# j-min/HiREST

Hardware: AMD Instinct MI355X
Metric: encoded frames/sec (EVA-CLIP-g/14 224^2) (higher is better)
Workload: dtype bf16

## Files before the change

### hirest_amd/_lib.py

```python
from __future__ import annotations

import ctypes as C
import os

HERE = os.path.dirname(os.path.abspath(__file__))
LIB_PATH = os.path.join(HERE, "lib", "libhirest_hip.so")
if os.environ.get("HIREST_LIB_VARIANT"):
    LIB_PATH = os.path.join(HERE, "lib", f"libhirest_hip.{os.environ['HIREST_LIB_VARIANT']}.so")

(EPI_BIAS_BF16, EPI_BIAS_GELU_BF16, EPI_BIAS_QGELU_BF16, EPI_BIAS_RESID_F32, EPI_BIAS_F32, EPI_PATCH_POS_F32,
 EPI_BIAS_RESID_LNSTATS_F32, EPI_LNFOLD_BF16, EPI_LNFOLD_GELU_BF16, EPI_BIAS_GELU_SPLIT2, EPI_BIAS_RESID2_LNSTATS) = range(11)

TOWER_NO_LNFOLD = 1
TOWER_NO_PRUNE = 2
TOWER_F32_RESIDUAL = 4
GEMM_REVERSE = 1
GEMM_X3 = 2
GEMM_X3_T128 = 4
ABI_VERSION = 4

ERRORS = {-1: "HIREST_E_BADARG", -2: "HIREST_E_SHAPE (unsupported shape)", -3: "HIREST_E_WORKSPACE (workspace too small)"}


class GemmArgs(C.Structure):
    _fields_ = [("struct_size", C.c_uint64),
                ("A", C.c_void_p), ("lda", C.c_int64), ("W", C.c_void_p), ("ldw", C.c_int64),
                ("bias", C.c_void_p), ("out", C.c_void_p), ("ldo", C.c_int64),
                ("M", C.c_int32), ("N", C.c_int32), ("K", C.c_int32), ("epilogue", C.c_int32),
                ("pos", C.c_void_p), ("patches_per_frame", C.c_int32), ("aux0", C.c_void_p), ("aux1", C.c_void_p), ("flags", C.c_int32)]

    @classmethod
    def make(cls, *fields):
        return cls(C.sizeof(cls), *fields)


F32_ENTRY = {"gemm": 0, "ws": 1, "layouts": 2, "ln": 3, "ln_colmax": 4, "rows_colmax": 5}


class GemmF32Query(C.Structure):
    _fields_ = [("struct_size", C.c_uint32)] + \
               [(n, C.c_int32) for n in ("entry", "M", "N", "K", "has_resid", "has_periodic", "has_ids", "has_ln_out", "has_workspace",
                                         "a_kmajor", "w_kmajor", "select_kernel", "ring_mode", "rows_ln_mode", "cus")]

    @classmethod
    def make(cls, entry, M, N, K, **fields):
        q = cls(C.sizeof(cls), F32_ENTRY[entry], M, N, K, select_kernel=-1, ring_mode=-1, rows_ln_mode=-1)
        for k, v in fields.items():
            setattr(q, k, int(v))
        return q


class BlockWeights(C.Structure):
    _fields_ = [(n, C.c_void_p) for n in ("ln1_g", "ln1_b", "qkv_w", "qkv_b", "proj_w", "proj_b",
                                          "ln2_g", "ln2_b", "fc1_w", "fc1_b", "fc2_w", "fc2_b",
                                          "qkv_wf", "qkv_bf", "qkv_s", "fc1_wf", "fc1_bf", "fc1_s")]


class VisionTower(C.Structure):
    _fields_ = [(n, C.c_int32) for n in ("image_size", "patch", "width", "heads", "head_dim", "mlp_dim",
                                         "layers", "embed_dim", "kpad", "act")] + \
               [("ln_eps", C.c_float)] + \
               [("patch_w", C.c_void_p), ("patch_b", C.c_void_p), ("cls", C.c_void_p), ("pos", C.c_void_p),
                ("blocks", C.POINTER(BlockWeights)),
                ("norm_g", C.c_void_p), ("norm_b", C.c_void_p), ("head_w", C.c_void_p), ("head_b", C.c_void_p),
                ("image_mean", C.c_void_p), ("image_std", C.c_void_p),
                ("ln_pre_g", C.c_void_p), ("ln_pre_b", C.c_void_p), ("out_all_tokens", C.c_int32)]


class TextTower(C.Structure):
    _fields_ = [(n, C.c_int32) for n in ("context", "vocab", "width", "heads", "layers", "embed_dim", "act")] + \
               [("ln_eps", C.c_float)] + \
               [("tok_emb", C.c_void_p), ("pos", C.c_void_p), ("blocks", C.POINTER(BlockWeights)),
                ("lnf_g", C.c_void_p), ("lnf_b", C.c_void_p), ("proj_w", C.c_void_p)]


class BlockWeightsF32(C.Structure):
    _fields_ = [(n, C.c_void_p) for n in ("ln1_g", "ln1_b", "qkv_w", "qkv_b", "proj_w", "proj_b",
                                          "ln2_g", "ln2_b", "fc1_w", "fc1_b", "fc2_w", "fc2_b")]


class VisionTowerF32(C.Structure):
    _fields_ = [(n, t) if n != "blocks" else (n, C.POINTER(BlockWeightsF32)) for n, t in VisionTower._fields_]


class TextTowerF32(C.Structure):
    _fields_ = [(n, t) if n != "blocks" else (n, C.POINTER(BlockWeightsF32)) for n, t in TextTower._fields_]


class BlockWeightsX3(C.Structure):
    _fields_ = [(n, C.c_void_p) for n in ("qkv_w2", "proj_w2", "fc1_w2", "fc2_w2")]


class VisionTowerX3(C.Structure):
    _fields_ = [("base", C.POINTER(VisionTowerF32)), ("blocks", C.POINTER(BlockWeightsX3))]


class CaptionLayer(C.Structure):
    _fields_ = [(n, C.c_void_p) for n in ("qkv_w", "qkv_b", "so_w", "so_b", "so_ln_g", "so_ln_b", "cq_w", "cq_b",
                                          "co_w", "co_b", "co_ln_g", "co_ln_b", "ff1_w", "ff1_b", "ff2_w", "ff2_b", "ff_ln_g", "ff_ln_b")]


class CaptionDecoder(C.Structure):
    _fields_ = [(n, C.c_int32) for n in ("layers", "heads", "hidden", "inter", "vocab_padded", "max_pos")] + \
               [(n, C.c_void_p) for n in ("word_emb", "pos_emb", "emb_ln_g", "emb_ln_b")] + \
               [("layer", C.POINTER(CaptionLayer))] + \
               [(n, C.c_void_p) for n in ("tr_w", "tr_b", "tr_ln_g", "tr_ln_b", "lm_w", "lm_b", "lm_w2")]


class WhisperLayer(C.Structure):
    _fields_ = [(n, C.c_void_p) for n in ("attn_ln_g", "attn_ln_b", "qkv_w", "qkv_b", "so_w", "so_b", "cross_ln_g", "cross_ln_b", "cq_w", "cq_b",
                                          "co_w", "co_b", "mlp_ln_g", "mlp_ln_b", "fc1_w", "fc1_b", "fc2_w", "fc2_b")]


class WhisperDecoder(C.Structure):
    _fields_ = [(n, C.c_int32) for n in ("layers", "heads", "hidden", "inter", "vocab_padded", "max_pos")] + \
               [(n, C.c_void_p) for n in ("tok_emb", "pos_emb")] + [("layer", C.POINTER(WhisperLayer))] + \
               [(n, C.c_void_p) for n in ("ln_g", "ln_b", "lm_b")]


class WhisperTailParams(C.Structure):
    _fields_ = [(n, C.c_int32) for n in ("n_vocab", "eot", "no_speech", "no_timestamps", "timestamp_begin", "max_initial_timestamp_index",
                                         "sample_begin", "blank", "suppress_blank", "timestamp_rules", "monotonic")] + \
               [("temperature", C.c_float), ("seed", C.c_uint32), ("serial", C.c_uint32), ("suppress_mask", C.c_void_p)]


class DtwProblem(C.Structure):
    _fields_ = [("x", C.c_void_p), ("ldx", C.c_int64), ("N", C.c_int32), ("M", C.c_int32), ("negate", C.c_int32), ("reserved", C.c_int32),
                ("path", C.c_void_p), ("path_len", C.c_void_p), ("cost", C.c_void_p), ("ldc", C.c_int64)]


class WhisperPrefillSeq(C.Structure):
    _fields_ = [(n, C.c_int32) for n in ("offset", "length", "window", "first_row", "n_rows", "sot_index")] + [("reserved", C.c_int32 * 2)]


DTW_MAX_N, DTW_MAX_M = 256, 4096

WHISPER_ROW_STATE_WORDS = 8
WHISPER_ROW_CTL_WORDS = 8


class JointLayerX3(C.Structure):
    _fields_ = [(n, C.c_void_p) for n in ("qkv_w2", "qkv_b", "ao_w2", "ao_b", "ln1_g", "ln1_b", "fc1_w2", "fc1_b", "fc2_w2", "fc2_b", "ln2_g", "ln2_b")]


class JointEncoderX3(C.Structure):
    _fields_ = [("struct_size", C.c_uint64)] + [(n, C.c_int32) for n in ("layers", "heads", "width", "mlp_dim", "in_dim", "max_pos")] + \
               [("ln_eps", C.c_float), ("attn_shift", C.c_float)] + \
               [(n, C.c_void_p) for n in ("emb_w2", "emb_b", "pos", "emb_ln_g", "emb_ln_b")] + [("layer", C.POINTER(JointLayerX3))]


class ColsumItem(C.Structure):
    _fields_ = [("x", C.c_void_p), ("row_weight", C.c_void_p), ("row_select", C.c_void_p), ("out", C.c_void_p), ("ldx", C.c_int64),
                ("R", C.c_int32), ("C", C.c_int32), ("select_value", C.c_int32), ("reserved", C.c_int32)]


COLSUM_GROUP_MAX = 40


class SplitItem(C.Structure):
    _fields_ = [("x", C.c_void_p), ("out", C.c_void_p), ("ldx", C.c_int64), ("ldo", C.c_int64), ("rows", C.c_int32), ("cols", C.c_int32),
                ("transposed", C.c_int32), ("reserved", C.c_int32)]


class OptimItem(C.Structure):
    _fields_ = [("p", C.c_void_p), ("g", C.c_void_p), ("m", C.c_void_p), ("v", C.c_void_p), ("n", C.c_int64)]


OPTIM_GROUP_MAX = 64
OPTIM_CHUNK = 8192


class TrainBlock(C.Structure):
    _fields_ = [("struct_size", C.c_uint64)] + [(n, C.c_int32) for n in ("B", "T", "heads", "width", "mlp", "precision")] + \
               [("ln_eps", C.c_float), ("drop", C.c_float)] + [(n, C.c_uint32) for n in ("seed_attn", "seed_ao", "seed_out", "reserved")] + \
               [(n, C.c_void_p) for n in ("wqkv", "bqkv", "wo", "bo", "ln1_g", "ln1_b", "w1", "b1", "w2", "b2", "ln2_g", "ln2_b", "x",
                                          "qkv", "P", "cx", "a_pre", "aa", "hpre", "hh", "x_pre", "out", "x2", "out2",
                                          "wqkv2", "wo2", "w12", "w22", "wqkvT2", "woT2", "w1T2", "w2T2", "ws")] + [("ws_bytes", C.c_size_t)]


class TrainFusionBwd(C.Structure):
    _fields_ = [("struct_size", C.c_uint64)] + \
               [(n, C.c_int32) for n in ("B", "T", "E", "W", "vis_dim", "text_dim", "asr_dim", "boundary", "max_pos", "reserved")] + \
               [("drop", C.c_float), ("seed_emb", C.c_uint32)] + \
               [(n, C.c_void_p) for n in ("w_emb", "emb_ln_g", "t2_w", "asr1_w", "asr0_g", "norm_g",
                                          "x0", "f", "v", "tn", "tin", "a0", "asr2", "v0", "vis2", "t", "text", "mm32", "bm32", "n_valid", "dx",
                                          "g_emb_ln_g", "g_emb_ln_b", "g_pos", "g_w_emb", "g_b_emb", "g_mask", "g_bound", "g_t2_w", "g_t2_b", "g_t0_w", "g_t0_b",
                                          "g_asr1_w", "g_asr1_b", "g_asr0_g", "g_asr0_b", "g_norm_g", "g_norm_b", "g_vis_w", "g_vis_b", "g_text_w", "g_text_b")] + \
               [("items", C.POINTER(ColsumItem)), ("n_items", C.POINTER(C.c_int32)), ("max_items", C.c_int32), ("reserved2", C.c_int32),
                ("ws", C.c_void_p), ("ws_bytes", C.c_size_t), ("side_stream", C.c_void_p), ("side_ws", C.c_void_p), ("side_ws_bytes", C.c_size_t),
                ("scratch", C.c_void_p), ("scratch_bytes", C.c_size_t)]


class TrainBlockGrads(C.Structure):
    _fields_ = [("struct_size", C.c_uint64)] + \
               [(n, C.c_void_p) for n in ("dout", "dx", "g_wqkv", "g_wo", "g_w1", "g_w2", "g_bqkv", "g_bo", "g_b1", "g_b2", "g_ln1_g", "g_ln1_b",
                                          "g_ln2_g", "g_ln2_b")] + \
               [("items", C.POINTER(ColsumItem)), ("n_items", C.POINTER(C.c_int32)), ("max_items", C.c_int32), ("reserved", C.c_int32),
                ("side_stream", C.c_void_p), ("side_ws", C.c_void_p), ("side_ws_bytes", C.c_size_t), ("scratch", C.c_void_p),
                ("scratch_bytes", C.c_size_t)]


class JpegImage(C.Structure):
    _fields_ = [(n, C.c_int32) for n in ("width", "height", "ncomp", "hs", "vs", "restart_interval", "mcux", "mcuy", "supported",
                                         "reason")] + \
               [("scan_begin", C.c_int64), ("scan_end", C.c_int64), ("table_set", C.c_int32), ("reserved", C.c_int32),
                ("data_offset", C.c_int64), ("out_offset", C.c_int64), ("ws_offset", C.c_int64),
                ("plane_offset", C.c_int64)]


class JpegTables(C.Structure):
    _fields_ = [("qt", (C.c_uint16 * 64) * 3), ("huff_bits", (C.c_uint8 * 16) * 6), ("huff_vals", (C.c_uint8 * 256) * 6)]


JPEG_REASONS = {0: "ok", 1: "not a JPEG / malformed markers", 2: "progressive", 3: "arithmetic coding", 4: "lossless / hierarchical",
                5: "not 8-bit", 6: "colour space (CMYK / YCCK / RGB / component count)", 7: "sampling factors", 8: "multi-scan",
                9: "truncated (no EOI after the scan)", 10: "bad or missing tables", 11: "image size"}
JPEG_STATUS = {1: "bad Huffman code", 2: "more than 64 coefficients in a block", 4: "out of data", 8: "RSTn out of sequence",
               16: "unsupported"}


BATCH_GATHER_MAX = 8


class BatchGather(C.Structure):
    _fields_ = [("src", C.c_void_p), ("dst", C.c_void_p), ("row_of_example", C.c_void_p), ("words", C.c_int32), ("reserved", C.c_int32)]


class BatchArgs(C.Structure):
    _fields_ = [("struct_size", C.c_uint64), ("index", C.c_void_p)] + \
               [(n, C.c_int32) for n in ("B", "T", "D", "Da", "n_examples", "n_model_frames", "n_gather", "reserved")] + \
               [(n, C.c_void_p) for n in ("frames", "frame_off", "asr_rows", "sub_off", "sub_span", "ex_video", "ex_len", "ex_range",
                                          "bound_off", "bound_val", "vis", "asr", "vis_mask", "moment_mask", "prev_boundary_mask")] + \
               [("gather", BatchGather * BATCH_GATHER_MAX)]


class ProfRecord(C.Structure):
    _fields_ = [("kind", C.c_int32), ("tag", C.c_int32), ("d0", C.c_int64), ("d1", C.c_int64), ("d2", C.c_int64),
                ("ms", C.c_float)]


_SIGNATURES = {
    "hirest_profile_enable": (C.c_int, [C.c_int32]),
    "hirest_attention_debug_mode": (C.c_int, [C.c_int32]),
    "hirest_profile_collect": (C.c_int, [C.POINTER(ProfRecord), C.c_int32]),
    "hirest_abi_version": (C.c_int, []),
    "hirest_build_info": (C.c_char_p, []),
    "hirest_gemm_bf16": (C.c_int, [C.POINTER(GemmArgs), C.c_void_p]),
    "hirest_gemm_select_kernel": (C.c_int, [C.c_int32]),
    "hirest_gemm_debug_mode": (C.c_int, [C.c_int32]),
    "hirest_gemm_dispatch_name": (C.c_int, [C.POINTER(GemmArgs), C.c_char_p, C.c_int32]),
    "hirest_attention_select_kernel": (C.c_int, [C.c_int32]),
    "hirest_attention_set_skew": (C.c_int, [C.c_int32]),
    "hirest_attention_set_mapping": (C.c_int, [C.c_int32]),
    "hirest_attention_set_pace": (C.c_int, [C.c_int32]),
    "hirest_attention_x3_select_waves": (C.c_int, [C.c_int32]),
    "hirest_attention_x3_debug_trace": (C.c_int, [C.c_void_p]),
    "hirest_attention_set_stagger": (C.c_int, [C.c_int32]),
    "hirest_attention_debug_trace_read": (C.c_int, [C.c_void_p, C.c_int32]),
    "hirest_layernorm": (C.c_int, [C.c_void_p, C.c_int64, C.c_void_p, C.c_void_p, C.c_void_p, C.c_float,
                                   C.c_void_p, C.c_int64, C.c_int32, C.c_int32, C.c_int32, C.c_void_p]),
    "hirest_attention_bf16": (C.c_int, [C.c_void_p, C.c_void_p, C.c_int32, C.c_int32, C.c_int32, C.c_int32,
                                        C.c_float, C.c_int32, C.c_void_p]),
    "hirest_attention_bf16_rows": (C.c_int, [C.c_void_p, C.c_void_p, C.c_int32, C.c_int32, C.c_int32, C.c_int32,
                                             C.c_float, C.c_int32, C.c_int32, C.c_void_p]),
    "hirest_fold_layernorm": (C.c_int, [C.c_void_p, C.c_void_p, C.c_void_p, C.c_void_p, C.c_void_p, C.c_void_p, C.c_void_p, C.c_int32,
                                        C.c_int32, C.c_void_p]),
    "hirest_patchify": (C.c_int, [C.c_void_p, C.c_int32, C.c_int32, C.c_int32, C.c_int32, C.c_void_p, C.c_void_p,
                                  C.c_void_p, C.c_int32, C.c_void_p]),
    "hirest_rowstats_bf16": (C.c_int, [C.c_void_p, C.c_int64, C.c_void_p, C.c_void_p, C.c_float, C.c_int32, C.c_int32, C.c_void_p, C.c_void_p]),
    "hirest_rowstats_split_bf16": (C.c_int, [C.c_void_p, C.c_int64, C.c_void_p, C.c_void_p, C.c_void_p, C.c_float, C.c_int32, C.c_int32, C.c_void_p,
                                             C.c_void_p]),
    "hirest_combine_hi_lo_f32": (C.c_int, [C.c_void_p, C.c_void_p, C.c_int64, C.c_void_p, C.c_int64, C.c_int32, C.c_int32, C.c_void_p]),
    "hirest_ln_stats_finalize": (C.c_int, [C.c_void_p, C.c_int32, C.c_void_p, C.c_float, C.c_int32, C.c_int32, C.c_void_p, C.c_void_p]),
    "hirest_write_cls_rows": (C.c_int, [C.c_void_p, C.c_int64, C.c_void_p, C.c_void_p, C.c_int32, C.c_int32,
                                        C.c_int32, C.c_void_p]),
    "hirest_embed_tokens": (C.c_int, [C.c_void_p, C.c_void_p, C.c_void_p, C.c_void_p, C.c_void_p, C.c_int32,
                                      C.c_int32, C.c_int32, C.c_int32, C.c_void_p]),
    "hirest_f32_to_bf16": (C.c_int, [C.c_void_p, C.c_void_p, C.c_int64, C.c_void_p]),
    "hirest_pool_l2norm": (C.c_int, [C.c_void_p, C.c_void_p, C.c_int32, C.c_int32, C.c_int32, C.c_int32, C.c_void_p]),
    "hirest_pool_l2norm_varlen": (C.c_int, [C.c_void_p, C.c_void_p, C.c_void_p, C.c_int32, C.c_int32, C.c_void_p]),
    "hirest_similarity_f32": (C.c_int, [C.c_void_p, C.c_void_p, C.c_void_p, C.c_int32, C.c_int32, C.c_int32, C.c_void_p]),
    "hirest_topk_workspace_bytes": (C.c_int64, [C.c_int32, C.c_int32, C.c_int32]),
    "hirest_topk_f32_ws": (C.c_int, [C.c_void_p, C.c_void_p, C.c_int32, C.c_int32, C.c_int32, C.c_void_p, C.c_void_p, C.c_void_p,
                                     C.c_int64, C.c_void_p]),
    "hirest_topk_f32": (C.c_int, [C.c_void_p, C.c_void_p, C.c_int32, C.c_int32, C.c_int32, C.c_void_p, C.c_void_p,
                                  C.c_void_p]),
    "hirest_clip_score": (C.c_int, [C.c_void_p, C.c_int32, C.c_int32, C.c_void_p, C.c_int32, C.c_void_p, C.c_int32, C.c_int32,
                                    C.c_int32, C.c_void_p, C.c_void_p]),
    "hirest_bertscore_greedy": (C.c_int, [C.c_void_p, C.c_int64, C.c_int32, C.c_void_p, C.c_int32, C.c_void_p, C.c_void_p, C.c_void_p,
                                          C.c_int32, C.c_void_p, C.c_void_p]),
    "hirest_gemm_f32": (C.c_int, [C.c_void_p, C.c_int64, C.c_void_p, C.c_int64, C.c_void_p, C.c_void_p, C.c_int64, C.c_void_p,
                                  C.c_int32, C.c_void_p, C.c_int64, C.c_int32, C.c_int32, C.c_int32, C.c_int32, C.c_void_p]),
    "hirest_attention_f32": (C.c_int, [C.c_void_p, C.c_void_p, C.c_int32, C.c_int32, C.c_int32, C.c_int32, C.c_float,
                                       C.c_float, C.c_void_p]),
    "hirest_attention_f32_qkv": (C.c_int, [C.c_void_p, C.c_int64, C.c_void_p, C.c_void_p, C.c_int64, C.c_void_p, C.c_int32, C.c_int32,
                                           C.c_int32, C.c_int32, C.c_int32, C.c_float, C.c_float, C.c_float, C.c_void_p]),
    "hirest_gemm_f32_select_kernel": (C.c_int, [C.c_int32]),
    "hirest_gemm_f32_workspace_bytes": (C.c_size_t, [C.c_int32, C.c_int32, C.c_int32]),
    "hirest_gemm_f32_layouts_workspace_bytes": (C.c_size_t, [C.c_int32, C.c_int32, C.c_int32]),
    "hirest_gemm_f32_layouts": (C.c_int, [C.c_void_p, C.c_int64, C.c_int32, C.c_void_p, C.c_int64, C.c_int32, C.c_void_p, C.c_void_p, C.c_int64,
                                          C.c_void_p, C.c_int64, C.c_int32, C.c_int32, C.c_int32, C.c_int32, C.c_void_p, C.c_size_t, C.c_void_p]),
    "hirest_gemm_f32_ws": (C.c_int, [C.c_void_p, C.c_int64, C.c_void_p, C.c_int64, C.c_void_p, C.c_void_p, C.c_int64, C.c_void_p,
                                     C.c_int32, C.c_void_p, C.c_int64, C.c_int32, C.c_int32, C.c_int32, C.c_int32, C.c_void_p, C.c_size_t,
                                     C.c_void_p]),
    "hirest_attention_f32_decode": (C.c_int, [C.c_void_p, C.c_int64, C.c_void_p, C.c_void_p, C.c_int64, C.c_void_p, C.c_int32, C.c_void_p,
                                              C.c_void_p, C.c_int64, C.c_void_p, C.c_void_p, C.c_void_p, C.c_int32, C.c_int32, C.c_float,
                                              C.c_float, C.c_float, C.c_void_p]),
    "hirest_gemm_f32_ln": (C.c_int, [C.c_void_p, C.c_int64, C.c_void_p, C.c_void_p, C.c_void_p, C.c_void_p, C.c_void_p, C.c_float,
                                     C.c_void_p, C.c_int64, C.c_void_p, C.c_int64, C.c_void_p, C.c_void_p, C.c_int64, C.c_void_p,
                                     C.c_int64, C.c_int32, C.c_int32, C.c_int32, C.c_int32, C.c_void_p]),
    "hirest_caption_step_workspace_bytes": (C.c_size_t, [C.POINTER(CaptionDecoder), C.c_int32]),
    "hirest_beam_backtrack": (C.c_int, [C.c_void_p, C.c_void_p, C.c_void_p, C.c_void_p, C.c_int32, C.c_int32, C.c_int32, C.c_void_p, C.c_void_p]),
    "hirest_beam_advance": (C.c_int, [C.c_void_p, C.c_void_p, C.c_int32, C.c_int32, C.c_int32, C.c_int32, C.c_int32, C.c_int32,
                                      C.c_void_p, C.c_void_p, C.c_void_p, C.c_void_p, C.c_void_p, C.c_void_p, C.c_void_p, C.c_void_p,
                                      C.c_void_p]),
    "hirest_caption_decode_step": (C.c_int, [C.POINTER(CaptionDecoder), C.c_int32, C.c_int32, C.c_void_p, C.c_void_p,
                                             C.POINTER(C.c_void_p), C.POINTER(C.c_void_p), C.POINTER(C.c_void_p), C.c_int32,
                                             C.c_void_p, C.c_void_p, C.c_void_p, C.c_size_t, C.c_void_p]),
    "hirest_caption_decode_logits": (C.c_int, [C.POINTER(CaptionDecoder), C.c_int32, C.c_int32, C.c_void_p, C.c_void_p,
                                               C.POINTER(C.c_void_p), C.POINTER(C.c_void_p), C.POINTER(C.c_void_p), C.c_int32,
                                               C.c_void_p, C.c_void_p, C.c_size_t, C.c_void_p]),
    "hirest_caption_select": (C.c_int, [C.c_int32]),
    "hirest_gemm_f32_ln_colmax": (C.c_int, [C.c_void_p, C.c_int64, C.c_void_p, C.c_void_p, C.c_float, C.c_void_p, C.c_int64, C.c_void_p,
                                            C.c_void_p, C.c_int64, C.c_void_p, C.c_int32, C.c_int32, C.c_int32, C.c_void_p]),
    "hirest_gemm_f32_dispatch_name": (C.c_int, [C.POINTER(GemmF32Query), C.c_char_p, C.c_int32]),
    "hirest_gemm_f32_rows_ln_mode": (C.c_int, [C.c_int32]),
    "hirest_gemm_f32_ring_mode": (C.c_int, [C.c_int32]),
    "hirest_gemm_f32_rows_preferred": (C.c_int, [C.c_int32]),
    "hirest_gemm_f32_rows_colmax": (C.c_int, [C.c_void_p, C.c_int64, C.c_void_p, C.c_int64, C.c_void_p, C.c_void_p, C.c_int64, C.c_void_p,
                                              C.c_int32, C.c_int32, C.c_int32, C.c_void_p]),
    "hirest_caption_beam_step": (C.c_int, [C.POINTER(CaptionDecoder), C.c_int32, C.c_int32, C.c_int32, C.c_void_p, C.c_void_p,
                                           C.POINTER(C.c_void_p), C.POINTER(C.c_void_p), C.POINTER(C.c_void_p), C.c_int32, C.c_void_p,
                                           C.c_void_p, C.c_int32, C.c_int32, C.c_void_p, C.c_void_p, C.c_void_p, C.c_void_p, C.c_void_p,
                                           C.c_void_p, C.c_void_p, C.c_size_t, C.c_void_p, C.c_size_t, C.c_void_p]),
    "hirest_caption_beam_tail_workspace_bytes": (C.c_size_t, [C.c_int32, C.c_int32, C.c_int32]),
    "hirest_caption_beam_tail": (C.c_int, [C.c_void_p, C.c_int64, C.c_void_p, C.c_int32, C.c_int32, C.c_int32, C.c_int32, C.c_int32,
                                           C.c_int32, C.c_void_p, C.c_void_p, C.c_void_p, C.c_void_p, C.c_void_p, C.c_void_p,
                                           C.c_void_p, C.c_void_p, C.c_void_p, C.c_void_p, C.c_size_t, C.c_void_p]),
    "hirest_attention_f32_varlen": (C.c_int, [C.c_void_p, C.c_void_p, C.c_void_p, C.c_int32, C.c_int32, C.c_int32, C.c_int32, C.c_float,
                                              C.c_float, C.c_void_p]),
    "hirest_log_softmax_f32": (C.c_int, [C.c_void_p, C.c_int64, C.c_void_p, C.c_void_p, C.c_int64, C.c_int32, C.c_int32, C.c_void_p]),
    "hirest_joint_time_grid_f32": (C.c_int, [C.c_void_p, C.c_int32, C.c_int32, C.c_void_p, C.c_void_p]),
    "hirest_joint_time_features": (C.c_int, [C.c_void_p, C.c_void_p, C.c_void_p, C.c_void_p, C.c_int32, C.c_int32, C.c_int32,
                                             C.c_void_p]),
    "hirest_joint_base": (C.c_int, [C.c_void_p, C.c_void_p, C.c_void_p, C.c_void_p, C.c_void_p, C.c_int32, C.c_int32, C.c_int32,
                                    C.c_void_p]),
    "hirest_joint_mask_add": (C.c_int, [C.c_void_p, C.c_void_p, C.c_void_p, C.c_void_p, C.c_void_p, C.c_void_p, C.c_int64,
                                        C.c_int32, C.c_void_p]),
    "hirest_transpose_pad_f32": (C.c_int, [C.c_void_p, C.c_int64, C.c_int32, C.c_int32, C.c_void_p, C.c_int32, C.c_void_p]),
    "hirest_weighted_colsum_grouped_f32": (C.c_int, [C.c_void_p, C.c_int32, C.c_void_p]),
    "hirest_train_fusion_backward_scratch_bytes": (C.c_size_t, [C.POINTER(TrainFusionBwd)]),
    "hirest_train_fusion_backward": (C.c_int, [C.POINTER(TrainFusionBwd), C.c_void_p]),
    "hirest_train_block_forward_scratch_bytes": (C.c_size_t, [C.POINTER(TrainBlock)]),
    "hirest_train_block_forward": (C.c_int, [C.POINTER(TrainBlock), C.c_void_p, C.c_size_t, C.c_void_p]),
    "hirest_train_block_backward_scratch_bytes": (C.c_size_t, [C.POINTER(TrainBlock)]),
    "hirest_train_block_backward": (C.c_int, [C.POINTER(TrainBlock), C.POINTER(TrainBlockGrads), C.c_void_p]),
    "hirest_optim_partials_count": (C.c_int64, [C.c_void_p, C.c_int32]),
    "hirest_grad_sqnorm_grouped_f32": (C.c_int, [C.c_void_p, C.c_int32, C.c_void_p, C.c_void_p]),
    "hirest_clip_coef_f32": (C.c_int, [C.c_void_p, C.c_int64, C.c_float, C.c_void_p, C.c_void_p]),
    "hirest_adamw_grouped_f32": (C.c_int, [C.c_void_p, C.c_int32, C.c_void_p, C.c_float, C.c_float, C.c_float, C.c_float, C.c_float,
                                           C.c_float, C.c_float, C.c_void_p]),
    "hirest_grad_sqnorm_scaled_grouped_f32": (C.c_int, [C.c_void_p, C.c_int32, C.c_void_p, C.c_void_p, C.c_void_p]),
    "hirest_clip_coef_dev_f32": (C.c_int, [C.c_void_p, C.c_int64, C.c_void_p, C.c_void_p, C.c_void_p]),
    "hirest_optim_step_advance_f32": (C.c_int, [C.c_void_p, C.c_int32, C.c_void_p, C.c_void_p]),
    "hirest_adamw_capturable_grouped_f32": (C.c_int, [C.c_void_p, C.c_void_p, C.c_int32, C.c_void_p, C.c_void_p, C.c_double, C.c_void_p,
                                                      C.c_void_p, C.c_double, C.c_double, C.c_float, C.c_double, C.c_void_p]),
    "hirest_weighted_colsum_f32": (C.c_int, [C.c_void_p, C.c_int64, C.c_void_p, C.c_void_p, C.c_int32, C.c_int32, C.c_int32, C.c_void_p, C.c_void_p]),
    "hirest_scale_by_device_scalar_f32": (C.c_int, [C.c_void_p, C.c_void_p, C.c_int64, C.c_void_p]),
    "hirest_act_f32": (C.c_int, [C.c_void_p, C.c_void_p, C.c_int64, C.c_int32, C.c_void_p]),
    "hirest_act_bwd_f32": (C.c_int, [C.c_void_p, C.c_void_p, C.c_void_p, C.c_int64, C.c_int32, C.c_void_p]),
    "hirest_dropout_add_f32": (C.c_int, [C.c_void_p, C.c_void_p, C.c_void_p, C.c_int64, C.c_float, C.c_uint32, C.c_void_p]),
    "hirest_layernorm_bwd_f32": (C.c_int, [C.c_void_p, C.c_void_p, C.c_void_p, C.c_float, C.c_void_p, C.c_void_p, C.c_int32, C.c_int32, C.c_void_p]),
    "hirest_attention_train_select": (C.c_int, [C.c_int32]),
    "hirest_gemm_f32_strided": (C.c_int, [C.c_void_p, C.c_int64, C.c_int64, C.c_void_p, C.c_int64, C.c_int64, C.c_void_p, C.c_int64,
                                          C.c_int32, C.c_int32, C.c_int32, C.c_float, C.c_void_p]),
    "hirest_attention_train_fwd_f32": (C.c_int, [C.c_void_p, C.c_void_p, C.c_void_p, C.c_int32, C.c_int32, C.c_int32, C.c_int32, C.c_float,
                                                 C.c_float, C.c_float, C.c_uint32, C.c_void_p]),
    "hirest_attention_train_bwd_f32": (C.c_int, [C.c_void_p, C.c_void_p, C.c_void_p, C.c_void_p, C.c_void_p, C.c_int32, C.c_int32, C.c_int32,
                                                 C.c_int32, C.c_float, C.c_float, C.c_uint32, C.c_void_p]),
    "hirest_attention_train_fwd_qkv_f32": (C.c_int, [C.c_void_p, C.c_int64, C.c_void_p, C.c_void_p, C.c_int64, C.c_void_p, C.c_void_p, C.c_void_p,
                                                     C.c_int64, C.c_int32, C.c_int32, C.c_int32, C.c_int32, C.c_int32, C.c_float, C.c_float,
                                                     C.c_float, C.c_uint32, C.c_void_p]),
    "hirest_attention_train_bwd_qkv_f32": (C.c_int, [C.c_void_p, C.c_int64, C.c_void_p, C.c_void_p, C.c_int64, C.c_void_p, C.c_void_p, C.c_int64,
                                                     C.c_void_p, C.c_void_p, C.c_int64, C.c_void_p, C.c_void_p, C.c_int64, C.c_int32, C.c_int32,
                                                     C.c_int32, C.c_int32, C.c_int32, C.c_float, C.c_float, C.c_uint32, C.c_void_p]),
    "hirest_embedding_fwd_f32": (C.c_int, [C.c_void_p, C.c_void_p, C.c_void_p, C.c_void_p, C.c_int64, C.c_int32, C.c_int32, C.c_void_p]),
    "hirest_embedding_pos_fwd_f32": (C.c_int, [C.c_void_p, C.c_void_p, C.c_void_p, C.c_void_p, C.c_void_p, C.c_int64, C.c_int32, C.c_void_p]),
    "hirest_embedding_bwd_f32": (C.c_int, [C.c_void_p, C.c_void_p, C.c_void_p, C.c_int64, C.c_int32, C.c_void_p]),
    "hirest_ce_rows_f32": (C.c_int, [C.c_void_p, C.c_int64, C.c_void_p, C.c_int32, C.c_int32, C.c_float, C.c_int32, C.c_void_p, C.c_void_p, C.c_void_p]),
    "hirest_bce_masked_f32": (C.c_int, [C.c_void_p, C.c_void_p, C.c_void_p, C.c_int32, C.c_int32, C.c_float, C.c_void_p, C.c_void_p, C.c_void_p]),
    "hirest_joint_base_bwd_f32": (C.c_int, [C.c_void_p, C.c_void_p, C.c_void_p, C.c_void_p, C.c_void_p, C.c_int32, C.c_int32, C.c_int32, C.c_void_p]),
    "hirest_l2norm_bwd_f32": (C.c_int, [C.c_void_p, C.c_void_p, C.c_void_p, C.c_int32, C.c_int32, C.c_void_p]),
    "hirest_ce_masked_f32": (C.c_int, [C.c_void_p, C.c_void_p, C.c_void_p, C.c_int32, C.c_int32, C.c_float, C.c_void_p, C.c_void_p, C.c_void_p]),
    "hirest_heads_bwd_f32": (C.c_int, [C.c_void_p, C.c_int64, C.c_int32, C.c_int32, C.c_void_p, C.c_void_p, C.c_void_p, C.c_void_p, C.c_void_p]),
    "hirest_linear_heads": (C.c_int, [C.c_void_p, C.c_int64, C.c_int32, C.c_int32, C.c_void_p, C.c_void_p, C.c_void_p, C.c_void_p,
                                      C.c_void_p, C.c_void_p]),
    "hirest_masked_argmax": (C.c_int, [C.c_void_p, C.c_void_p, C.c_float, C.c_int32, C.c_int32, C.c_void_p, C.c_void_p]),
    "hirest_moment_valid_f32": (C.c_int, [C.c_void_p, C.c_void_p, C.c_void_p, C.c_void_p, C.c_void_p, C.c_int32, C.c_int32, C.c_float,
                                          C.c_void_p, C.c_void_p, C.c_void_p]),
    "hirest_lm_head_ce_workspace_bytes": (C.c_size_t, [C.c_int32, C.c_int32]),
    "hirest_lm_head_ce_f32": (C.c_int, [C.c_void_p, C.c_int64, C.c_void_p, C.c_int64, C.c_void_p, C.c_void_p, C.c_int32, C.c_int32,
                                        C.c_int32, C.c_int32, C.c_void_p, C.c_void_p, C.c_void_p, C.c_size_t, C.c_void_p]),
    "hirest_segmentation_step": (C.c_int, [C.c_void_p, C.c_void_p, C.c_void_p, C.c_int32, C.c_int32, C.c_double, C.c_void_p,
                                           C.c_void_p, C.c_int32, C.c_void_p, C.c_void_p]),
    "hirest_preprocess_plan_bytes": (C.c_int64, [C.c_int32, C.c_int32, C.c_int32]),
    "hirest_preprocess_plan": (C.c_int, [C.c_int32, C.c_int32, C.c_int32, C.c_void_p, C.c_int64]),
    "hirest_preprocess_workspace_bytes": (C.c_int64, [C.c_int32, C.c_int32, C.c_int32, C.c_int32]),
    "hirest_preprocess_u8": (C.c_int, [C.c_void_p, C.c_int32, C.c_int32, C.c_int32, C.c_int32, C.c_void_p, C.c_void_p,
                                       C.c_int32, C.c_void_p, C.c_void_p, C.c_void_p, C.c_int64, C.c_void_p]),
    "hirest_jpeg_parse": (C.c_int, [C.c_void_p, C.c_int64, C.POINTER(JpegImage), C.POINTER(JpegTables)]),
    "hirest_jpeg_workspace_bytes": (C.c_int64, [C.POINTER(JpegImage), C.c_int32]),
    "hirest_jpeg_decode": (C.c_int, [C.c_void_p, C.c_void_p, C.c_int32, C.c_void_p, C.c_void_p, C.c_void_p, C.c_void_p, C.c_void_p,
                                     C.c_int64, C.c_void_p]),
    "hirest_jpeg_decode_host": (C.c_int, [C.POINTER(JpegImage), C.POINTER(JpegTables), C.c_void_p, C.c_void_p, C.POINTER(C.c_int32)]),
    "hirest_jpeg_chunked_workspace_bytes": (C.c_int64, [C.c_int32]),
    "hirest_jpeg_decode_chunked": (C.c_int, [C.c_void_p, C.c_void_p, C.c_int32, C.c_void_p, C.c_void_p, C.c_void_p, C.c_void_p, C.c_void_p,
                                             C.c_int64, C.c_int64, C.c_void_p, C.c_int64, C.c_void_p]),
# ... 130 lines not shown
```

### hirest_amd/clip.py

```python
from __future__ import annotations

import ctypes as C
import os
from typing import Dict, List, Union

import torch
from torch import nn

from . import _lib, ops
from .eva_clip import (OPENAI_DATASET_MEAN, OPENAI_DATASET_STD, _NO_FOLD, _RESBLOCK, TextTower, _Leaf, _Tower, _linear, _norm,
                       _precision_scope, image_transform)
from .tokenizer import tokenize

__all__ = ["available_models", "load", "tokenize", "build_model", "CLIP"]


def available_models() -> List[str]:
    return []


class OpenAIVisionTower(_Tower):
    _what = "CLIP vision tower"
    _FIELDS = (("patch_w", "patch", "conv1.weight"), ("patch_b", None, None),
               ("cls", "f32", "class_embedding"), ("pos", "f32", "positional_embedding"),
               ("norm_g", "f32", "ln_post.weight"), ("norm_b", "f32", "ln_post.bias"), ("head_w", "wT", "proj"), ("head_b", None, None),
               ("image_mean", "const", "image_mean"), ("image_std", "const", "image_std"),
               ("ln_pre_g", "f32", "ln_pre.weight"), ("ln_pre_b", "f32", "ln_pre.bias"))
    _TABLES = {"bf16": (_lib.VisionTower, _FIELDS, _lib.BlockWeights, _RESBLOCK + _NO_FOLD),
               "fp32": (_lib.VisionTowerF32, _FIELDS, _lib.BlockWeightsF32, _RESBLOCK)}
    image_mean, image_std = OPENAI_DATASET_MEAN, OPENAI_DATASET_STD

    def __init__(self, input_resolution: int, patch_size: int, width: int, layers: int, heads: int, output_dim: int):
        super().__init__()
        self.input_resolution, self.patch_size, self.width, self.layers, self.heads = input_resolution, patch_size, width, layers, heads
        self.output_dim = output_dim
        self.grid = input_resolution // patch_size
        self.num_tokens = self.grid ** 2 + 1
        D = width
        self.conv1 = _Leaf(weight=(D, 3, patch_size, patch_size))
        self.class_embedding = nn.Parameter(torch.zeros(D))
        self.positional_embedding = nn.Parameter(torch.zeros(self.num_tokens, D))
        self.ln_pre = _norm(D)
        self.transformer = nn.Module()
        blocks = []
        for _ in range(layers):
            b = nn.Module()
            b.attn = _Leaf(in_proj_weight=(3 * D, D), in_proj_bias=(3 * D,))
            b.attn.out_proj = _linear(D, D)
            b.ln_1, b.ln_2 = _norm(D), _norm(D)
            b.mlp = nn.Module()
            b.mlp.c_fc, b.mlp.c_proj = _linear(4 * D, D), _linear(D, 4 * D)
            blocks.append(b)
        self.transformer.resblocks = nn.ModuleList(blocks)
        self.precision = "bf16"
        self.pip_head = False
        self.ln_post = _norm(D)
        self.proj = nn.Parameter(torch.zeros(D, output_dim))
        self.max_frames_per_call = 2048

    def _blocks(self):
        return self.transformer.resblocks

    def _scalars(self):
        D, P = self.width, self.patch_size
        return dict(image_size=self.input_resolution, patch=P, width=D, heads=self.heads, head_dim=D // self.heads, mlp_dim=4 * D,
                    layers=self.layers, embed_dim=self.output_dim, kpad=(3 * P * P + 63) // 64 * 64,
                    act=1, ln_eps=1e-5,
                    out_all_tokens=1)

    @torch.no_grad()
    def forward(self, x: torch.Tensor) -> torch.Tensor:
        if x.dtype not in (torch.float32, torch.bfloat16, torch.uint8):
            x = x.float()
        f32 = self.precision != "bf16"
        desc = C.byref(self._prepared_for("fp32" if f32 else "bf16", x.device)["desc"])
        lib = _lib.load()
        x = x.contiguous()
        B, T, E = x.shape[0], self.num_tokens, self.output_dim
        out = torch.empty((B, T, E), dtype=torch.float32, device=x.device)
        if B == 0:
            return out[:, 0, :] if self.pip_head else out[:, 1:, :]
        code = ops._IN_DTYPES[x.dtype]

        def call(s, n, ws):
            if f32:
                _lib.check(lib.hirest_vision_forward_f32(desc, x[s:s + n].data_ptr(), code, n, out[s:s + n].data_ptr(), ws.data_ptr(),
                                                         ws.numel(), ops.stream_ptr()), "hirest_vision_forward_f32")
            else:
                _lib.check(lib.hirest_vision_forward(desc, x[s:s + n].data_ptr(), code, n, out[s:s + n].data_ptr(), ws.data_ptr(),
                                                     ws.numel(), 0, ops.stream_ptr()), "hirest_vision_forward")
        wsb = lib.hirest_vision_workspace_bytes_f32 if f32 else lib.hirest_vision_workspace_bytes
        self._run_calls(B, self.max_frames_per_call, False, lambda n: wsb(desc, n), call, x.device)
        if self.pip_head:
            return out[:, 0, :]
        return out[:, 1:, :]


class CLIP(nn.Module):

    def __init__(self, embed_dim, image_resolution, vision_layers, vision_width, vision_patch_size,
                 context_length, vocab_size, transformer_width, transformer_heads, transformer_layers):
        super().__init__()
        if isinstance(vision_layers, (tuple, list)):
            raise NotImplementedError("ModifiedResNet visual towers are not used by HiREST and not implemented")
        self.context_length = context_length
        self.visual = OpenAIVisionTower(image_resolution, vision_patch_size, vision_width, vision_layers,
                                        vision_width // 64, embed_dim)
        t = TextTower(vocab_size, transformer_width, transformer_layers, transformer_heads, context_length, embed_dim,
                      quick_gelu=True)
        object.__setattr__(self, "_text", t)
        self.transformer = t.transformer
        self.token_embedding = t.token_embedding
        self.positional_embedding = t.positional_embedding
        self.ln_final = t.ln_final
        self.text_projection = t.text_projection
        self.logit_scale = t.logit_scale
        self.vocab_size = vocab_size

    def _apply(self, fn, *a, **k):
        r = super()._apply(fn, *a, **k)
        self._text.invalidate()
        self._text._workspace = None
        return r

    def _load_from_state_dict(self, *a, **k):
        self._text.invalidate()
        return super()._load_from_state_dict(*a, **k)

    def set_precision(self, precision: str):
        if precision not in ("bf16", "fp32", "bf16x3"):
            raise ValueError(f"precision must be one of ('bf16', 'fp32', 'bf16x3'), got {precision!r}")
        p = "bf16" if precision == "bf16" else "fp32"
        self.visual.precision = p
        self._text.precision = p
        return self

    def precision_scope(self, visual: str = None, text: str = None):
        for precision in (visual, text):
            if precision not in (None, "bf16", "fp32", "bf16x3"):
                raise ValueError(f"precision must be one of ('bf16', 'fp32', 'bf16x3'), got {precision!r}")
        to = {None: None, "bf16": "bf16", "fp32": "fp32", "bf16x3": "fp32"}
        return _precision_scope(((self.visual, to[visual]), (self._text, to[text])))

    @property
    def dtype(self):
        return self.visual.conv1.weight.dtype

    def encode_image(self, image):
        return self.visual(image)

    def encode_text(self, text):
        return self._text(text)

    def forward(self, image, text):
        img = self.encode_image(image)
        txt = self.encode_text(text)
        img = ops.pool_l2norm(img.float().unsqueeze(1).contiguous())
        txt = ops.pool_l2norm(txt.float().unsqueeze(1).contiguous())
        logits_per_image = ops.gemm_f32_strided(img, txt, float(torch.exp(self.logit_scale.detach().float().cpu())))
        return logits_per_image, logits_per_image.transpose(-1, -2)


def build_model(state_dict: Dict[str, torch.Tensor]) -> CLIP:
    if "visual.proj" not in state_dict:
        raise NotImplementedError("only ViT CLIP checkpoints are supported (ModifiedResNet is unused by HiREST)")
    vision_width = state_dict["visual.conv1.weight"].shape[0]
    vision_layers = len([k for k in state_dict if k.startswith("visual.") and k.endswith(".attn.in_proj_weight")])
    vision_patch_size = state_dict["visual.conv1.weight"].shape[-1]
    grid_size = round((state_dict["visual.positional_embedding"].shape[0] - 1) ** 0.5)
    image_resolution = vision_patch_size * grid_size
    embed_dim = state_dict["text_projection"].shape[1]
    context_length = state_dict["positional_embedding"].shape[0]
    vocab_size = state_dict["token_embedding.weight"].shape[0]
    transformer_width = state_dict["ln_final.weight"].shape[0]
    transformer_heads = transformer_width // 64
    transformer_layers = len(set(k.split(".")[2] for k in state_dict if k.startswith("transformer.resblocks")))
    model = CLIP(embed_dim, image_resolution, vision_layers, vision_width, vision_patch_size, context_length, vocab_size,
                 transformer_width, transformer_heads, transformer_layers)
    sd = {k: v for k, v in state_dict.items() if k not in ("input_resolution", "context_length", "vocab_size")}
    model.load_state_dict({k: v.float() for k, v in sd.items()}, strict=True)
    return model.eval()


def load(name: str, device: Union[str, torch.device] = "cuda", jit: bool = False, download_root: str = None, pip_head: bool = False,
         precision: str = "bf16"):
    if not os.path.isfile(name):
        raise RuntimeError(f"Model {name} not found; available models = {available_models()}")
    try:
        state_dict = torch.jit.load(name, map_location="cpu").eval().state_dict()
    except RuntimeError:
        state_dict = torch.load(name, map_location="cpu")
    model = build_model(state_dict).to(device)
    env = os.environ.get("HIREST_PRECISION", "").strip().lower()
    model.set_precision(env or precision)
    model.visual.pip_head = bool(pip_head)
    return model, image_transform(model.visual.input_resolution)
```

### hirest_amd/csrc/attention.hip

```cpp
#include "common.h"
#include <atomic>
#include "profile.h"

namespace {

template <int DH, int DP, int NT>
struct AttnCfg {
    static constexpr int NPAD = 16 * NT;
    static constexpr int KS = (NT + 1) / 2;
    static constexpr int KP = 32 * KS;
    static constexpr int KRS = DP * 2 + 16;
    static constexpr int VRS = KP * 2 + 16;
    static constexpr int LDS_BYTES = NPAD * KRS + DP * VRS;
};

template <int DH, int DP, int NT>
__global__ __launch_bounds__(512) void attention_kernel(const bf16_t* __restrict__ qkv, bf16_t* __restrict__ out,
                                                       int N, int H, float scale_log2e, int causal, int nq) {
    using C = AttnCfg<DH, DP, NT>;
    extern __shared__ __attribute__((aligned(16))) char smem[];
    char* Ks = smem;
    char* Vt = smem + C::NPAD * C::KRS;
    const int tid = threadIdx.x, lane = tid & 63, wave = tid >> 6;
    const int b = blockIdx.x / H, h = blockIdx.x - b * H;
    const int D = H * DH;
    const int64_t ld = 3 * (int64_t)D;
    const bf16_t* base = qkv + (int64_t)b * N * ld + h * DH;

    constexpr int KCH = DP / 8;
    for (int idx = tid; idx < C::NPAD * KCH; idx += 512) {
        const int key = idx / KCH, ch = idx - key * KCH;
        bf16x8 v = {0, 0, 0, 0, 0, 0, 0, 0};
        if (key < N && ch * 8 < DH) v = *reinterpret_cast<const bf16x8*>(base + (int64_t)key * ld + D + ch * 8);
        *reinterpret_cast<bf16x8*>(Ks + key * C::KRS + ch * 16) = v;
    }
    constexpr int VCH = DH / 8;
    for (int idx = tid; idx < C::KP * VCH; idx += 512) {
        const int ch = idx / C::KP, key = idx - ch * C::KP;
        bf16x8 v = {0, 0, 0, 0, 0, 0, 0, 0};
        if (key < N) v = *reinterpret_cast<const bf16x8*>(base + (int64_t)key * ld + 2 * D + ch * 8);
#pragma unroll
        for (int e = 0; e < 8; ++e) *reinterpret_cast<bf16_t*>(Vt + (ch * 8 + e) * C::VRS + key * 2) = v[e];
    }
    __syncthreads();

    const int g = lane >> 4, c16 = lane & 15;
    const int nqt = (nq + 15) >> 4;
    for (int qt = wave; qt < nqt; qt += 8) {
        const int q = qt * 16 + c16;
        const bool qvalid = q < N;
        bf16x8 qf[DP / 32];
#pragma unroll
        for (int kk = 0; kk < DP / 32; ++kk) {
            const int d = (kk * 4 + g) * 8;
            bf16x8 v = {0, 0, 0, 0, 0, 0, 0, 0};
            if (qvalid && d < DH) v = *reinterpret_cast<const bf16x8*>(base + (int64_t)q * ld + d);
            qf[kk] = v;
        }
        f32x4 st[NT];
#pragma unroll
        for (int t = 0; t < NT; ++t) {
            f32x4 acc = {0.f, 0.f, 0.f, 0.f};
#pragma unroll
            for (int kk = 0; kk < DP / 32; ++kk) {
                const bf16x8 kf = *reinterpret_cast<const bf16x8*>(Ks + (t * 16 + c16) * C::KRS + (kk * 4 + g) * 16);
                acc = __builtin_amdgcn_mfma_f32_16x16x32_bf16(kf, qf[kk], acc, 0, 0, 0);
            }
            st[t] = acc;
            if ((t & 1) == 1) __builtin_amdgcn_sched_barrier(0);
        }
        const int klimit = causal ? (q < N - 1 ? q : N - 1) : N - 1;
        float mx = -3.0e38f;
#pragma unroll
        for (int t = 0; t < NT; ++t)
#pragma unroll
            for (int i = 0; i < 4; ++i) {
                const int key = t * 16 + 4 * g + i;
                const float s = key <= klimit ? st[t][i] : -3.0e38f;
                st[t][i] = s;
                mx = fmaxf(mx, s);
            }
        mx = fmaxf(mx, __shfl_xor(mx, 16, 64));
        mx = fmaxf(mx, __shfl_xor(mx, 32, 64));
        float sum = 0.f;
#pragma unroll
        for (int t = 0; t < NT; ++t)
#pragma unroll
            for (int i = 0; i < 4; ++i) {
                const float pz = exp2f((st[t][i] - mx) * scale_log2e);
                st[t][i] = pz;
                sum += pz;
            }
        sum += __shfl_xor(sum, 16, 64);
        sum += __shfl_xor(sum, 32, 64);
        const float inv = 1.0f / sum;
        bf16x8 pf[C::KS];
#pragma unroll
        for (int s = 0; s < C::KS; ++s) {
#pragma unroll
            for (int i = 0; i < 4; ++i) {
                pf[s][i] = (bf16_t)st[2 * s][i];
                if (2 * s + 1 < NT) pf[s][4 + i] = (bf16_t)st[2 * s + 1][i];
                else pf[s][4 + i] = (bf16_t)0.f;
            }
        }
#pragma unroll 1
        for (int dt = 0; dt < DP / 16; ++dt) {
            f32x4 acc = {0.f, 0.f, 0.f, 0.f};
            const char* vrow = Vt + (dt * 16 + c16) * C::VRS + 8 * g;
#pragma unroll
            for (int s = 0; s < C::KS; ++s) {
                const bf16x4 lo = *reinterpret_cast<const bf16x4*>(vrow + s * 64);
                const bf16x4 hi = *reinterpret_cast<const bf16x4*>(vrow + s * 64 + 32);
                const bf16x8 vf = {lo[0], lo[1], lo[2], lo[3], hi[0], hi[1], hi[2], hi[3]};
                acc = __builtin_amdgcn_mfma_f32_16x16x32_bf16(vf, pf[s], acc, 0, 0, 0);
            }
            const int d = dt * 16 + 4 * g;
            if (q < nq && d < DH) {
                bf16x4 o;
#pragma unroll
                for (int i = 0; i < 4; ++i) o[i] = (bf16_t)(acc[i] * inv);
                *reinterpret_cast<bf16x4*>(out + ((int64_t)b * N + q) * D + h * DH + d) = o;
            }
        }
    }
}

template <int DH, int DP, int NT>
int launch(const bf16_t* qkv, bf16_t* out, int B, int N, int H, float scale, int causal, int nq, hipStream_t s) {
    using C = AttnCfg<DH, DP, NT>;
    static HirestDevCfg cfg;
    auto kern = attention_kernel<DH, DP, NT>;
    if (int e = hirest_configure(kern, C::LDS_BYTES, cfg)) return e;
    hipLaunchKernelGGL(kern, dim3(B * H), dim3(512), C::LDS_BYTES, s, qkv, out, N, H, scale * 1.44269504088896340736f, causal, nq);
    return hirest_launch_status();
}


template <int DH, int DP, int NT>
struct AttnCfg2 {
    static constexpr int NPAD = 16 * NT;
    static constexpr int KS = (NT + 1) / 2;
    static constexpr int KP = 32 * KS;
    static constexpr int RS = DP * 2;
    static constexpr int CPR = DP / 8;
    static constexpr int NK_INSTR = NPAD * CPR / 64;
    static constexpr int NV_INSTR = KP * CPR / 64;
    static constexpr int LDS_BYTES = (NPAD + KP) * RS;
};

__device__ __forceinline__ void wait_vm_le(int n) {
    switch (n) {
        case 0: asm volatile("s_waitcnt vmcnt(0)" ::: "memory"); break;
        case 1: asm volatile("s_waitcnt vmcnt(1)" ::: "memory"); break;
        case 2: asm volatile("s_waitcnt vmcnt(2)" ::: "memory"); break;
        case 3: asm volatile("s_waitcnt vmcnt(3)" ::: "memory"); break;
        case 4: asm volatile("s_waitcnt vmcnt(4)" ::: "memory"); break;
        case 5: asm volatile("s_waitcnt vmcnt(5)" ::: "memory"); break;
        case 6: asm volatile("s_waitcnt vmcnt(6)" ::: "memory"); break;
        case 7: asm volatile("s_waitcnt vmcnt(7)" ::: "memory"); break;
        default: asm volatile("s_waitcnt vmcnt(8)" ::: "memory"); break;
    }
}

template <int DH, int DP, int NT>
__global__ __launch_bounds__(512) void attention_kernel_v2(const bf16_t* __restrict__ qkv, bf16_t* __restrict__ out,
                                                          int N, int H, float scale_log2e, int causal, int nq) {
    using C = AttnCfg2<DH, DP, NT>;
    extern __shared__ __attribute__((aligned(16))) char smem[];
    char* Ks = smem;
    char* Vs = smem + C::NPAD * C::RS;
    const int tid = threadIdx.x, lane = tid & 63;
    const int wave = __builtin_amdgcn_readfirstlane(tid >> 6);
    const int b = blockIdx.x / H, h = blockIdx.x - b * H;
    const int D = H * DH;
    const int64_t ld = 3 * (int64_t)D;
    const bf16_t* base = qkv + (int64_t)b * N * ld + h * DH;

    int nv_mine = 0;
    for (int i = wave; i < C::NK_INSTR; i += 8) {
        const int ci = i * 64 + lane;
        int row = ci / C::CPR, c = ci - row * C::CPR;
        c = (c & ~3) | ((c & 3) ^ ((-(row >> 2)) & 3));
        row = row < N ? row : N - 1;
        c = c * 8 < DH ? c : DH / 8 - 1;
        glds16(base + (int64_t)row * ld + D + c * 8, Ks + i * 1024);
    }
    for (int i = wave; i < C::NV_INSTR; i += 8) {
        const int ci = i * 64 + lane;
        int row = ci / C::CPR, c = ci - row * C::CPR;
        row = row < N ? row : N - 1;
        c = c * 8 < DH ? c : DH / 8 - 1;
        glds16(base + (int64_t)row * ld + 2 * D + c * 8, Vs + i * 1024);
        ++nv_mine;
    }
    wait_vm_le(nv_mine);
    __builtin_amdgcn_s_barrier();

    const int g = lane >> 4, c16 = lane & 15;
    const int gk = g ^ ((-(c16 >> 2)) & 3);
    const int nqt = (nq + 15) >> 4;
    bool v_ready = false;
    for (int qt = wave; qt < nqt; qt += 8) {
        const int q = qt * 16 + c16;
        const bool qvalid = q < N;
        bf16x8 qf[DP / 32];
#pragma unroll
        for (int kk = 0; kk < DP / 32; ++kk) {
            const int d = (kk * 4 + g) * 8;
            bf16x8 v = {0, 0, 0, 0, 0, 0, 0, 0};
            if (qvalid && d < DH) v = *reinterpret_cast<const bf16x8*>(base + (int64_t)q * ld + d);
            qf[kk] = v;
        }
        f32x4 st[NT];
#pragma unroll
        for (int t = 0; t < NT; ++t) {
            f32x4 acc = {0.f, 0.f, 0.f, 0.f};
#pragma unroll
            for (int kk = 0; kk < DP / 32; ++kk) {
                const bf16x8 kf = *reinterpret_cast<const bf16x8*>(Ks + (t * 16 + c16) * C::RS + (kk * 4 + gk) * 16);
                acc = __builtin_amdgcn_mfma_f32_16x16x32_bf16(kf, qf[kk], acc, 0, 0, 0);
            }
            st[t] = acc;
            if ((t & 1) == 1) __builtin_amdgcn_sched_barrier(0);
        }
        const int klimit = causal ? (q < N - 1 ? q : N - 1) : N - 1;
        float mx = -3.0e38f;
#pragma unroll
        for (int t = 0; t < NT; ++t)
#pragma unroll
            for (int i = 0; i < 4; ++i) {
                const int key = t * 16 + 4 * g + i;
                const float sv = key <= klimit ? st[t][i] : -3.0e38f;
                st[t][i] = sv;
                mx = fmaxf(mx, sv);
            }
        mx = fmaxf(mx, __shfl_xor(mx, 16, 64));
        mx = fmaxf(mx, __shfl_xor(mx, 32, 64));
        float sum = 0.f;
#pragma unroll
        for (int t = 0; t < NT; ++t)
#pragma unroll
            for (int i = 0; i < 4; ++i) {
                const float pz = exp2f((st[t][i] - mx) * scale_log2e);
                st[t][i] = pz;
                sum += pz;
            }
        sum += __shfl_xor(sum, 16, 64);
        sum += __shfl_xor(sum, 32, 64);
        const float inv = 1.0f / sum;
        bf16x8 pf[C::KS];
#pragma unroll
        for (int s = 0; s < C::KS; ++s) {
#pragma unroll
            for (int i = 0; i < 4; ++i) {
                pf[s][i] = (bf16_t)st[2 * s][i];
                if (2 * s + 1 < NT) pf[s][4 + i] = (bf16_t)st[2 * s + 1][i];
                else pf[s][4 + i] = (bf16_t)0.f;
            }
        }
        if (!v_ready) {
            asm volatile("s_waitcnt vmcnt(0)" ::: "memory");
            __builtin_amdgcn_s_barrier();
            v_ready = true;
        }
        const char* vlane = Vs + (4 * g + (c16 >> 2)) * C::RS + (c16 & 3) * 8;
#pragma unroll 1
        for (int dt = 0; dt < DP / 16; ++dt) {
            f32x4 acc = {0.f, 0.f, 0.f, 0.f};
            const char* vrow = vlane + dt * 32;
#pragma unroll
            for (int s = 0; s < C::KS; ++s) {
                const bf16x4 lo = __builtin_amdgcn_ds_read_tr16_b64_v4bf16(
                    (__attribute__((address_space(3))) bf16x4*)(vrow + s * 32 * C::RS));
                const bf16x4 hi = __builtin_amdgcn_ds_read_tr16_b64_v4bf16(
                    (__attribute__((address_space(3))) bf16x4*)(vrow + (s * 32 + 16) * C::RS));
                const bf16x8 vf = {lo[0], lo[1], lo[2], lo[3], hi[0], hi[1], hi[2], hi[3]};
                acc = __builtin_amdgcn_mfma_f32_16x16x32_bf16(vf, pf[s], acc, 0, 0, 0);
            }
            const int d = dt * 16 + 4 * g;
            if (q < nq && d < DH) {
                bf16x4 o;
#pragma unroll
                for (int i = 0; i < 4; ++i) o[i] = (bf16_t)(acc[i] * inv);
                *reinterpret_cast<bf16x4*>(out + ((int64_t)b * N + q) * D + h * DH + d) = o;
            }
        }
    }
    if (!v_ready) {
        asm volatile("s_waitcnt vmcnt(0)" ::: "memory");
        __builtin_amdgcn_s_barrier();
    }
}


__device__ __forceinline__ void sleep_n(int n) {
    for (int i = 0; i < n; ++i) __builtin_amdgcn_s_sleep(1);
}
template <int NW, int CPR> struct ROWS_PER_PIECE_OK { static constexpr bool value = (NW * 64 % CPR == 0) && ((NW * 64 / CPR) % 8 == 0); };
__device__ __attribute__((aligned(16))) const unsigned short g_attn_ones[8] = {0x3F80, 0x3F80, 0x3F80, 0x3F80, 0x3F80, 0x3F80, 0x3F80, 0x3F80};
__device__ __attribute__((aligned(16))) const unsigned short g_attn_zeros[8] = {0, 0, 0, 0, 0, 0, 0, 0};
constexpr int ATTN_TRACE_STEPS = 64, ATTN_TRACE_WAVES = 12, ATTN_TRACE_SLOTS = 12;
__device__ long long g_attn_trace[ATTN_TRACE_STEPS * ATTN_TRACE_WAVES * ATTN_TRACE_SLOTS];
__device__ __forceinline__ float max3_raw(float a, float b, float c) {
    float r;
    asm("v_max3_f32 %0, %1, %2, %3" : "=v"(r) : "v"(a), "v"(b), "v"(c));
    return r;
}
typedef float f32x2_t __attribute__((ext_vector_type(2)));
template <int DH, int DP, int NT, bool FAST, bool DBG, int NW = 9, bool LEAN = false, bool PROD = false>
__global__ __launch_bounds__((NW + (PROD ? 1 : 0)) * 64) void attention_kernel_v3(const bf16_t* __restrict__ qkv, bf16_t* __restrict__ out,
                                                          int N, int H, float scale_log2e, int causal, int dbg_bits, int nq, int skew,
                                                          int B, int map, int pace, int stagger) {
    const int dbg = DBG ? dbg_bits : 0;
    using C = AttnCfg2<DH, DP, NT>;
    extern __shared__ __attribute__((aligned(16))) char smem[];
    char* Vs = smem + 2 * C::NPAD * C::RS;
    const int tid = threadIdx.x, lane = tid & 63;
    const int wave = __builtin_amdgcn_readfirstlane(tid >> 6);
    const int D = H * DH;
    const int64_t ld = 3 * (int64_t)D;
    int b0, bstep, h0, hstep, nsteps;
    if (map == 0) { b0 = blockIdx.x; bstep = 0; h0 = 0; hstep = 1; nsteps = H; }
    else {
        const int xcd = blockIdx.x & 7, slot = blockIdx.x >> 3, FL = (gridDim.x >> 3) / H;
        h0 = slot % H; hstep = 0; b0 = xcd * FL + slot / H; bstep = 8 * FL;
        nsteps = b0 < B ? (B - b0 + bstep - 1) / bstep : 0;
    }
    if (nsteps == 0) return;
    if (stagger > 0 && blockIdx.x < 256) sleep_n(((blockIdx.x >> 3) & 15) * stagger);
    auto sbase = [&](int st) { return qkv + (int64_t)(b0 + st * bstep) * N * ld + (h0 + st * hstep) * DH; };
    const int g = lane >> 4, c16 = lane & 15;
    const int gk = g ^ ((-(c16 >> 2)) & 3);
    const int nqt = (nq + 15) >> 4;

    const int ci0 = wave * 64 + lane;
    const int row0 = ci0 / C::CPR, col0 = ci0 - row0 * C::CPR;
    constexpr bool VSWAP = C::RS == 192;
    const int vlog = VSWAP ? ((((col0 >> 1) ^ ((row0 >> 2) & 1)) << 1) | (col0 & 1)) : col0;
    const int vc = vlog * 8 < DH ? vlog : DH / 8 - 1;
    static_assert(ROWS_PER_PIECE_OK<NW, C::CPR>::value, "a lane's rows must keep (row >> 2) & 1 from piece to piece");
    static_assert((NW * 64) % C::CPR == 0, "piece stride must be whole rows");
    constexpr int ROWS_PER_PIECE = NW * 64 / C::CPR;
    auto dma_k = [&](int h, char* dst) -> int {
        int n = 0;
        const bf16_t* src = sbase(h) + D;
        for (int i = wave, row = row0; i < C::NK_INSTR; i += NW, row += ROWS_PER_PIECE) {
            int kc = (col0 & ~3) | ((col0 & 3) ^ ((-(row >> 2)) & 3));
            const bool kpad = kc * 8 >= DH;
            kc = kpad ? DH / 8 - 1 : kc;
            const int r = row < N ? row : N - 1;
            const void* from = src + (int64_t)r * ld + kc * 8;
            if (LEAN && DP > DH) from = kpad ? (const void*)g_attn_zeros : from;
            glds16(from, dst + i * 1024);
            ++n;
        }
        return n;
    };
    constexpr bool SUM_IN_MFMA = LEAN && DP > DH;
    const bool vpad = SUM_IN_MFMA && vlog * 8 >= DH;
    auto dma_v = [&](int h) {
        const bf16_t* src = sbase(h) + 2 * D + vc * 8;
        for (int i = wave, row = row0; i < C::NV_INSTR; i += NW, row += ROWS_PER_PIECE) {
            const int r = row < N ? row : N - 1;
            const void* from = src + (int64_t)r * ld;
            if (SUM_IN_MFMA) from = vpad ? (const void*)g_attn_ones : from;
            glds16(from, Vs + i * 1024);
        }
    };
    auto load_q = [&](int h, int qtile, bf16x8 (&dst)[DP / 32]) {
        const int q = qtile * 16 + c16;
        const bf16_t* base = sbase(h);
        if (LEAN && DP > DH) {
            const bf16_t* row = base + (int64_t)(q < N ? q : N - 1) * ld;
#pragma unroll
            for (int kk = 0; kk < DP / 32; ++kk) {
                const int d = (kk * 4 + g) * 8;
                dst[kk] = *reinterpret_cast<const bf16x8*>(row + (d < DH ? d : DH - 8));
            }
            return;
        }
#pragma unroll
        for (int kk = 0; kk < DP / 32; ++kk) {
            const int d = (kk * 4 + g) * 8;
            bf16x8 v = {0, 0, 0, 0, 0, 0, 0, 0};
            if (qtile < nqt && q < N && d < DH) v = *reinterpret_cast<const bf16x8*>(base + (int64_t)q * ld + d);
            dst[kk] = v;
        }
    };

    if (PROD && wave == NW) {
        constexpr int PER = C::CPR / 4;
        static_assert(C::NK_INSTR % PER == 0 && C::NV_INSTR % PER == 0, "whole 16-row groups");
        int prow[PER], pkoff[PER], pvoff[PER];
        bool pkpad[PER], pvpad[PER];
#pragma unroll
        for (int j = 0; j < PER; ++j) {
            const int ci = j * 64 + lane, r = ci / C::CPR, c = ci - r * C::CPR;
            prow[j] = r;
            int kc = (c & ~3) | ((c & 3) ^ ((-(r >> 2)) & 3));
            pkpad[j] = kc * 8 >= DH;
            pkoff[j] = (pkpad[j] ? DH / 8 - 1 : kc) * 8;
            const int vl = VSWAP ? ((((c >> 1) ^ ((r >> 2) & 1)) << 1) | (c & 1)) : c;
            pvpad[j] = SUM_IN_MFMA && vl * 8 >= DH;
            pvoff[j] = (vl * 8 < DH ? vl : DH / 8 - 1) * 8;
        }
        auto issue_k = [&](int st, char* dst, int pace_units) {
            const bf16_t* src = sbase(st) + D;
            for (int it0 = 0; it0 < C::NK_INSTR / PER; ++it0) {
                const int it = map ? (it0 + h0) % (C::NK_INSTR / PER) : it0;
#pragma unroll
                for (int j = 0; j < PER; ++j) {
                    const int row = prow[j] + 16 * it, r = row < N ? row : N - 1;
                    const void* from = src + (int64_t)r * ld + pkoff[j];
                    if (LEAN && DP > DH) from = pkpad[j] ? (const void*)g_attn_zeros : from;
                    glds16(from, dst + (it * PER + j) * 1024);
                    if (pace_units > 0) sleep_n(pace_units);
                }
            }
        };
        auto issue_v = [&](int st) {
            const bf16_t* src = sbase(st) + 2 * D;
            for (int it0 = 0; it0 < C::NV_INSTR / PER; ++it0) {
                const int it = map ? (it0 + h0) % (C::NV_INSTR / PER) : it0;
#pragma unroll
                for (int j = 0; j < PER; ++j) {
                    const int row = prow[j] + 16 * it, r = row < N ? row : N - 1;
                    const void* from = src + (int64_t)r * ld + pvoff[j];
                    if (SUM_IN_MFMA) from = pvpad[j] ? (const void*)g_attn_ones : from;
                    glds16(from, Vs + (it * PER + j) * 1024);
                }
            }
        };
        issue_k(0, smem, 0);
        for (int h = 0; h < nsteps; ++h) {
            asm volatile("s_waitcnt vmcnt(0)" ::: "memory");
            __builtin_amdgcn_s_barrier();
            issue_v(h);
            asm volatile("s_waitcnt vmcnt(0)" ::: "memory");
            __builtin_amdgcn_s_barrier();
            if (h + 1 < nsteps) issue_k(h + 1, smem + ((h + 1) & 1) * (C::NPAD * C::RS), pace);
        }
        asm volatile("s_waitcnt vmcnt(0)" ::: "memory");
        return;
    }

    bf16x8 qa[DP / 32], qb[DP / 32];
    load_q(0, wave, qa);
    load_q(0, wave + NW, qb);
    if (!(dbg & 8) && !PROD) dma_k(0, smem);
    for (int h = 0; h < nsteps; ++h) {
        const char* Ks = smem + (h & 1) * (C::NPAD * C::RS);
        auto stamp = [&](int slot) {
            if (DBG && (dbg & 256) && blockIdx.x == 0 && h < ATTN_TRACE_STEPS) {
                const long long t = __builtin_readcyclecounter();
                if (lane == 0) g_attn_trace[(h * ATTN_TRACE_WAVES + wave) * ATTN_TRACE_SLOTS + slot] = t;
            }
        };
        stamp(10);
        asm volatile("s_waitcnt vmcnt(0)" ::: "memory");
#pragma unroll
        for (int kk = 0; kk < DP / 32; ++kk) { asm volatile("" : "+v"(qa[kk])); asm volatile("" : "+v"(qb[kk])); }
        if (!(dbg & 128)) __builtin_amdgcn_s_barrier();
        stamp(0);
        if (!(dbg & 8) && !PROD) dma_v(h);
        const int nk_next = (h + 1 < nsteps && !(dbg & 8) && !PROD) ? dma_k(h + 1, smem + ((h + 1) & 1) * (C::NPAD * C::RS)) : 0;
        bool v_ready = false;
        auto tile = [&](int qt, bf16x8 (&qf)[DP / 32], int ord) {
            stamp(1 + 4 * ord);
            const int q = qt * 16 + c16;
            const bool qvalid = q < N;
            f32x4 st[NT];
#pragma unroll
            for (int t = 0; t < NT; t += 2) {
                f32x4 a0 = {0.f, 0.f, 0.f, 0.f}, a1 = {0.f, 0.f, 0.f, 0.f};
                if (!(dbg & 1))
#pragma unroll
                for (int kk = 0; kk < DP / 32; ++kk) {
                    const bf16x8 k0 = *reinterpret_cast<const bf16x8*>(Ks + (t * 16 + c16) * C::RS + (kk * 4 + gk) * 16);
                    a0 = __builtin_amdgcn_mfma_f32_16x16x32_bf16(k0, qf[kk], a0, 0, 0, 0);
                    if (t + 1 < NT) {
                        const bf16x8 k1 = *reinterpret_cast<const bf16x8*>(Ks + ((t + 1) * 16 + c16) * C::RS + (kk * 4 + gk) * 16);
                        a1 = __builtin_amdgcn_mfma_f32_16x16x32_bf16(k1, qf[kk], a1, 0, 0, 0);
                    }
                }
                st[t] = a0;
                if (t + 1 < NT) st[t + 1] = a1;
                if ((t & 2) || !FAST) __builtin_amdgcn_sched_barrier(0);
            }
            if (h + 1 < nsteps && !(dbg & 32)) load_q(h + 1, qt, qf);
            stamp(2 + 4 * ord);
            const int klimit = causal ? (q < N - 1 ? q : N - 1) : N - 1;
            float mx = -3.0e38f;
            float sum = 0.f;
            bf16x8 pf[C::KS];
            if (LEAN) {
                float mxb = -3.0e38f;
#pragma unroll
                for (int t = 0; t < NT; ++t) {
                    if (!FAST || t == NT - 1) {
#pragma unroll
                        for (int i = 0; i < 4; ++i) st[t][i] = (t * 16 + 4 * g + i) <= klimit ? st[t][i] : -3.0e38f;
                    }
                    if (t & 1) { mxb = max3_raw(mxb, st[t][0], st[t][1]); mxb = max3_raw(mxb, st[t][2], st[t][3]); }
                    else { mx = max3_raw(mx, st[t][0], st[t][1]); mx = max3_raw(mx, st[t][2], st[t][3]); }
                }
                float pa = max3_raw(mx, mxb, mxb), pb = pa;
                lane_swap16(pa, pb); pa = max3_raw(pa, pb, pb); pb = pa; lane_swap32(pa, pb); mx = max3_raw(pa, pb, pb);
                const float nmc = -mx * scale_log2e;
                const f32x2_t sc2 = {scale_log2e, scale_log2e}, nm2 = {nmc, nmc};
                f32x2_t sum2 = {0.f, 0.f};
#pragma unroll
                for (int s2 = 0; s2 < C::KS; ++s2) {
#pragma unroll
                    for (int u = 0; u < 2; ++u) {
                        if (2 * s2 + u < NT) {
#pragma unroll
                            for (int ip = 0; ip < 2; ++ip) {
                                const f32x2_t sv = {st[2 * s2 + u][2 * ip], st[2 * s2 + u][2 * ip + 1]};
                                const f32x2_t e = __builtin_elementwise_fma(sv, sc2, nm2);
                                const f32x2_t p2 = (dbg & 2) ? e : f32x2_t{__builtin_amdgcn_exp2f(e[0]), __builtin_amdgcn_exp2f(e[1])};
                                if (!SUM_IN_MFMA) sum2 += p2;
                                pf[s2][4 * u + 2 * ip] = (bf16_t)p2[0];
                                pf[s2][4 * u + 2 * ip + 1] = (bf16_t)p2[1];
                            }
                        } else {
#pragma unroll
                            for (int i = 0; i < 4; ++i) pf[s2][4 + i] = (bf16_t)0.f;
                        }
                    }
                }
                if (!SUM_IN_MFMA) {
                    sum = sum2[0] + sum2[1];
                    float sa = sum, sb = sum; lane_swap16(sa, sb); sum = sa + sb; sa = sum; sb = sum; lane_swap32(sa, sb); sum = sa + sb;
                }
            } else {
#pragma unroll
            for (int t = 0; t < NT; ++t) {
                if (!FAST || t == NT - 1) {
#pragma unroll
                    for (int i = 0; i < 4; ++i) st[t][i] = (t * 16 + 4 * g + i) <= klimit ? st[t][i] : -3.0e38f;
                }
                mx = fmaxf(fmaxf(mx, fmaxf(st[t][0], st[t][1])), fmaxf(st[t][2], st[t][3]));
            }
            { float pa = mx, pb = mx; lane_swap16(pa, pb); mx = fmaxf(pa, pb); pa = mx; pb = mx; lane_swap32(pa, pb); mx = fmaxf(pa, pb); }
            const float nmc = -mx * scale_log2e;
#pragma unroll
            for (int s2 = 0; s2 < C::KS; ++s2) {
#pragma unroll
                for (int i = 0; i < 4; ++i) {
                    const float e0 = fmaf(st[2 * s2][i], scale_log2e, nmc);
                    const float p0 = (dbg & 2) ? e0 : __builtin_amdgcn_exp2f(e0);
                    sum += p0;
                    pf[s2][i] = (bf16_t)p0;
                    if (2 * s2 + 1 < NT) {
                        const float e1 = fmaf(st[2 * s2 + 1][i], scale_log2e, nmc);
                        const float p1 = (dbg & 2) ? e1 : __builtin_amdgcn_exp2f(e1);
                        sum += p1;
                        pf[s2][4 + i] = (bf16_t)p1;
                    } else {
                        pf[s2][4 + i] = (bf16_t)0.f;
                    }
                }
            }
            { float pa = sum, pb = sum; lane_swap16(pa, pb); sum = pa + pb; pa = sum; pb = sum; lane_swap32(pa, pb); sum = pa + pb; }
            }
            stamp(3 + 4 * ord);
            if (!v_ready) {
                if (!PROD) wait_vm_le(nk_next);
                if (!(dbg & 64)) __builtin_amdgcn_s_barrier();
                v_ready = true;
            }
            stamp(4 + 4 * ord);
            const char* vlane = Vs + (4 * g + (c16 >> 2)) * C::RS + (c16 & 3) * 8;
            const char* vl_e = vlane + ((VSWAP && (g & 1)) ? 32 : 0);
            const char* vl_o = vlane - ((VSWAP && (g & 1)) ? 32 : 0);
            f32x4 oacc[DP / 16];
#pragma unroll
            for (int dt = 0; dt < DP / 16; ++dt) oacc[dt] = f32x4{0.f, 0.f, 0.f, 0.f};
            if (!(dbg & 4))
#pragma unroll
            for (int s2 = 0; s2 < C::KS; ++s2) {
#pragma unroll
                for (int dt = 0; dt < DP / 16; ++dt) {
                    const char* vrow = ((dt & 1) ? vl_o : vl_e) + dt * 32 + s2 * 32 * C::RS;
                    const bf16x4 lo = __builtin_amdgcn_ds_read_tr16_b64_v4bf16((__attribute__((address_space(3))) bf16x4*)(vrow));
                    const bf16x4 hi = __builtin_amdgcn_ds_read_tr16_b64_v4bf16((__attribute__((address_space(3))) bf16x4*)(vrow + 16 * C::RS));
                    const bf16x8 vf = {lo[0], lo[1], lo[2], lo[3], hi[0], hi[1], hi[2], hi[3]};
                    oacc[dt] = __builtin_amdgcn_mfma_f32_16x16x32_bf16(vf, pf[s2], oacc[dt], 0, 0, 0);
                }
                if ((s2 & 1) || !FAST) __builtin_amdgcn_sched_barrier(0);
            }
            if (SUM_IN_MFMA) {
                float sa = oacc[DP / 16 - 1][0], sb = sa;
                lane_swap32(sa, sb);
                sum = sb;
            }
            const float inv = 1.0f / sum;
            static_assert((DP / 16) % 2 == 0 && DH % 8 == 0, "paired d tiles");
#pragma unroll
            for (int dp = 0; dp < DP / 32; ++dp) {
                union { bf16x4 v; unsigned u[2]; } e, o;
#pragma unroll
                for (int i = 0; i < 4; ++i) { e.v[i] = (bf16_t)(oacc[2 * dp][i] * inv); o.v[i] = (bf16_t)(oacc[2 * dp + 1][i] * inv); }
                const auto s0 = __builtin_amdgcn_permlane16_swap(e.u[0], o.u[0], false, false);
                const auto s1 = __builtin_amdgcn_permlane16_swap(e.u[1], o.u[1], false, false);
                union { bf16x8 v; unsigned u[4]; } w;
                w.u[0] = s0[0]; w.u[1] = s1[0]; w.u[2] = s0[1]; w.u[3] = s1[1];
                const int d = (2 * dp + (g & 1)) * 16 + (g >> 1) * 8;
                if (qvalid && q < nq && d < DH && !(dbg & 16)) *reinterpret_cast<bf16x8*>(out + ((int64_t)(b0 + h * bstep) * N + q) * D + (h0 + h * hstep) * DH + d) = w.v;
            }
        };
        if (skew > 0 && wave >= 4 && wave < 8) sleep_n(skew);
        if (wave < nqt) tile(wave, qa, 0);
        if (wave + NW < nqt) tile(wave + NW, qb, 1);
        stamp(9);
        if (!v_ready) {
            if (!PROD) wait_vm_le(nk_next);
            __builtin_amdgcn_s_barrier();
        }
    }
    asm volatile("s_waitcnt vmcnt(0)" ::: "memory");
}

std::atomic<int> g_attn_dbg{0};
std::atomic<int> g_attn_skew{12};
std::atomic<int> g_attn_stagger{16};
std::atomic<int> g_attn_pace{0};
std::atomic<int> g_attn_map{2};
std::atomic<int> g_attn_variant{7};

template <int DH, int DP, int NT, bool FAST, bool DBG, int NW = 9, bool LEAN = false, bool PROD = false>
int launch3_impl(const bf16_t* qkv, bf16_t* out, int B, int N, int H, float scale, int causal, int nq, hipStream_t s) {
    using C = AttnCfg2<DH, DP, NT>;
    constexpr int LDS = (2 * C::NPAD + C::KP) * C::RS;
    static_assert(LDS <= 163840, "K x2 + V must fit the CU's LDS");
    static HirestDevCfg cfg;
    auto kern = attention_kernel_v3<DH, DP, NT, FAST, DBG, NW, LEAN, PROD>;
    if (int e = hirest_configure(kern, LDS, cfg)) return e;
    const bool by_head = (g_attn_map == 1 || (g_attn_map == 2 && B < 256)) && H <= 32 && 32 % H == 0 && B >= 8 * (32 / H) * 4;
    const int grid = by_head ? 256 : B;
    hipLaunchKernelGGL(kern, dim3(grid), dim3((NW + (PROD ? 1 : 0)) * 64), LDS, s, qkv, out, N, H, scale * 1.44269504088896340736f, causal, g_attn_dbg, nq,
                       g_attn_skew, B, by_head ? 1 : 0, g_attn_pace, g_attn_stagger);
    return hirest_launch_status();
}

template <int DH, int DP, int NT, bool FAST>
int launch3(const bf16_t* qkv, bf16_t* out, int B, int N, int H, float scale, int causal, int nq, hipStream_t s) {
    if (g_attn_dbg && FAST && g_attn_variant == 6) return launch3_impl<DH, DP, NT, FAST, true, 9, true, true>(qkv, out, B, N, H, scale, causal, nq, s);
    if (g_attn_variant == 6) return launch3_impl<DH, DP, NT, FAST, false, 9, true, true>(qkv, out, B, N, H, scale, causal, nq, s);
    if (g_attn_dbg && FAST && g_attn_variant == 7) return launch3_impl<DH, DP, NT, FAST, true, 9, false, true>(qkv, out, B, N, H, scale, causal, nq, s);
    if (g_attn_variant == 7) return launch3_impl<DH, DP, NT, FAST, false, 9, false, true>(qkv, out, B, N, H, scale, causal, nq, s);
    if (g_attn_dbg && FAST && g_attn_variant == 5) return launch3_impl<DH, DP, NT, FAST, true, 9, true>(qkv, out, B, N, H, scale, causal, nq, s);
    if (g_attn_dbg && FAST) return launch3_impl<DH, DP, NT, FAST, true>(qkv, out, B, N, H, scale, causal, nq, s);
    if (g_attn_variant == 4) return launch3_impl<DH, DP, NT, FAST, false, 12>(qkv, out, B, N, H, scale, causal, nq, s);
    if (g_attn_variant == 5) return launch3_impl<DH, DP, NT, FAST, false, 9, true>(qkv, out, B, N, H, scale, causal, nq, s);
    return launch3_impl<DH, DP, NT, FAST, false>(qkv, out, B, N, H, scale, causal, nq, s);
}


template <int DH, int DP, int NT>
int launch2(const bf16_t* qkv, bf16_t* out, int B, int N, int H, float scale, int causal, int nq, hipStream_t s) {
    using C = AttnCfg2<DH, DP, NT>;
    static HirestDevCfg cfg;
    auto kern = attention_kernel_v2<DH, DP, NT>;
    if (int e = hirest_configure(kern, C::LDS_BYTES, cfg)) return e;
    hipLaunchKernelGGL(kern, dim3(B * H), dim3(512), C::LDS_BYTES, s, qkv, out, N, H, scale * 1.44269504088896340736f, causal, nq);
    return hirest_launch_status();
}

}

extern "C" int hirest_attention_debug_mode(int32_t bits) { g_attn_dbg = bits; return 0; }

extern "C" int hirest_attention_set_skew(int32_t units) {
    if (units < 0 || units > 64) return HIREST_E_BADARG;
    g_attn_skew = units;
    return 0;
}

extern "C" int hirest_attention_debug_trace_read(int64_t* dst, int32_t n) {
    if (!dst || n <= 0 || n > ATTN_TRACE_STEPS * ATTN_TRACE_WAVES * ATTN_TRACE_SLOTS) return HIREST_E_BADARG;
    return (int)hipMemcpyFromSymbol(dst, HIP_SYMBOL(g_attn_trace), sizeof(long long) * n);
}

extern "C" int hirest_attention_set_stagger(int32_t units) {
    if (units < 0 || units > 64) return HIREST_E_BADARG;
    g_attn_stagger = units;
    return 0;
}

extern "C" int hirest_attention_set_pace(int32_t units) {
    if (units < 0 || units > 64) return HIREST_E_BADARG;
    g_attn_pace = units;
    return 0;
}

extern "C" int hirest_attention_set_mapping(int32_t by_head) {
    if (by_head < 0 || by_head > 2) return HIREST_E_BADARG;
    g_attn_map = by_head;
    return 0;
}

extern "C" int hirest_attention_select_kernel(int32_t which) {
    if (which < 1 || which > 7) return HIREST_E_BADARG;
    g_attn_variant = which;
    return 0;
}

extern "C" int hirest_attention_bf16(const hirest_bf16* qkv, hirest_bf16* out, int32_t B, int32_t N, int32_t H,
                                     int32_t dh, float scale, int32_t causal, void* stream) {
    return hirest_attention_bf16_rows(qkv, out, B, N, H, dh, scale, causal, N, stream);
}

extern "C" int hirest_attention_bf16_rows(const hirest_bf16* qkv, hirest_bf16* out, int32_t B, int32_t N, int32_t H,
                                          int32_t dh, float scale, int32_t causal, int32_t q_rows, void* stream) {
    if (!qkv || !out || B <= 0 || N <= 0 || H <= 0 || q_rows <= 0 || q_rows > N) return HIREST_E_BADARG;
    const int nq = q_rows;
    hipStream_t s = reinterpret_cast<hipStream_t>(stream);
    const bf16_t* q = reinterpret_cast<const bf16_t*>(qkv);
    bf16_t* o = reinterpret_cast<bf16_t*>(out);
    HirestProfScope prof(HIREST_PROF_ATTENTION, causal, (int64_t)B * H, N, dh, s);
    if (g_attn_variant >= 3 && N > 80 && N <= 272 && B >= 64) {
        const bool fast = !causal && N > 256;
        if (dh == 88) return fast ? launch3<88, 96, 17, true>(q, o, B, N, H, scale, causal, nq, s)
                                  : launch3<88, 96, 17, false>(q, o, B, N, H, scale, causal, nq, s);
        if (dh == 64) return fast ? launch3<64, 64, 17, true>(q, o, B, N, H, scale, causal, nq, s)
                                  : launch3<64, 64, 17, false>(q, o, B, N, H, scale, causal, nq, s);
    }
    if (g_attn_variant >= 2) {
        if (dh == 88) {
            if (N <= 80) return launch2<88, 96, 5>(q, o, B, N, H, scale, causal, nq, s);
            if (N <= 272) return launch2<88, 96, 17>(q, o, B, N, H, scale, causal, nq, s);
        } else if (dh == 64) {
            if (N <= 80) return launch2<64, 64, 5>(q, o, B, N, H, scale, causal, nq, s);
            if (N <= 272) return launch2<64, 64, 17>(q, o, B, N, H, scale, causal, nq, s);
        }
        return HIREST_E_SHAPE;
    }
    if (dh == 88) {
        if (N <= 80) return launch<88, 96, 5>(q, o, B, N, H, scale, causal, nq, s);
        if (N <= 272) return launch<88, 96, 17>(q, o, B, N, H, scale, causal, nq, s);
    } else if (dh == 64) {
        if (N <= 80) return launch<64, 64, 5>(q, o, B, N, H, scale, causal, nq, s);
        if (N <= 272) return launch<64, 64, 17>(q, o, B, N, H, scale, causal, nq, s);
    }
    return HIREST_E_SHAPE;
}
```

### hirest_amd/csrc/tower.hip

```cpp
#include "common.h"

namespace {

inline size_t align256(size_t v) { return (v + 255) & ~(size_t)255; }

struct Regions {
    size_t x, h, big, eot, xb, xl, cls, part, stats, guard, total;
};

Regions plan(int64_t M, int D, int wide, int B, bool lnfold = false) {
    Regions r;
    size_t off = 0;
    r.x = off; off += align256((size_t)M * D * 4);
    r.h = off; off += align256((size_t)M * D * 2);
    r.big = off; off += align256((size_t)M * wide * 2);
    r.eot = off; off += align256((size_t)B * 4);
    r.xb = r.xl = r.cls = r.part = r.stats = r.guard = off;
    if (lnfold) {
        r.xb = off; off += align256((size_t)M * D * 2);
        r.xl = off; off += align256((size_t)M * D * 2);
        r.cls = off; off += 2 * align256((size_t)B * D * 2);
        r.part = off; off += align256((size_t)M * ((D + 63) / 64) * 8);
        r.stats = off; off += align256((size_t)M * 8);
        r.guard = off; off += 256;
    }
    r.total = off;
    return r;
}

inline bool vision_lnfold(const hirest_vision_tower* t, int B) {
    if (!t->blocks || !t->blocks[0].qkv_wf || t->act != 0 || t->ln_pre_g || B < 64) return false;
    const int T = (t->image_size / t->patch) * (t->image_size / t->patch) + 1;
    const int64_t M = (int64_t)B * T;
    return t->width >= 256 && t->width <= 1536 && t->width % 8 == 0 && M * t->width >= (int64_t)2048 * 1024;
}

inline int vision_wide(const hirest_vision_tower* t) {
    int w = 3 * t->width;
    if (t->mlp_dim > w) w = t->mlp_dim;
    if (t->kpad > w) w = t->kpad;
    return w;
}

#define CHECK(expr) do { int _e = (expr); if (_e != 0) return _e; } while (0)

int gemm(const void* A, int64_t lda, const void* W, int64_t ldw, const float* bias, void* out, int64_t ldo, int M, int N,
         int K, int epi, void* stream, const float* pos = nullptr, int P = 0, void* aux0 = nullptr, void* aux1 = nullptr,
         int flags = 0) {
    hirest_gemm_args a;
    a.struct_size = sizeof(a);
    a.A = reinterpret_cast<const hirest_bf16*>(A); a.lda = lda;
    a.W = reinterpret_cast<const hirest_bf16*>(W); a.ldw = ldw;
    a.bias = bias; a.out = out; a.ldo = ldo; a.M = M; a.N = N; a.K = K; a.epilogue = epi;
    a.pos = pos; a.patches_per_frame = P; a.aux0 = aux0; a.aux1 = aux1; a.flags = flags;
    return hirest_gemm_bf16(&a, stream);
}

int run_block(const hirest_block_weights& w, float* x, hirest_bf16* h, hirest_bf16* big, int B, int T, int D, int heads,
              int dh, int Dm, float eps, int act, int causal, void* stream) {
    const int M = B * T;
    CHECK(hirest_layernorm(x, D, nullptr, w.ln1_g, w.ln1_b, eps, h, D, 0, M, D, stream));
    CHECK(gemm(h, D, w.qkv_w, D, w.qkv_b, big, 3 * D, M, 3 * D, D, HIREST_EPI_BIAS_BF16, stream));
    CHECK(hirest_attention_bf16(big, h, B, T, heads, dh, 1.0f / sqrtf((float)dh), causal, stream));
    CHECK(gemm(h, D, w.proj_w, D, w.proj_b, x, D, M, D, D, HIREST_EPI_BIAS_RESID_F32, stream));
    CHECK(hirest_layernorm(x, D, nullptr, w.ln2_g, w.ln2_b, eps, h, D, 0, M, D, stream));
    CHECK(gemm(h, D, w.fc1_w, D, w.fc1_b, big, Dm, M, Dm, D,
               act == 1 ? HIREST_EPI_BIAS_QGELU_BF16 : HIREST_EPI_BIAS_GELU_BF16, stream));
    CHECK(gemm(big, Dm, w.fc2_w, Dm, w.fc2_b, x, D, M, D, Dm, HIREST_EPI_BIAS_RESID_F32, stream));
    return 0;
}

int run_block_lnfold(const hirest_block_weights& w, float* x, hirest_bf16* h, hirest_bf16* big, hirest_bf16* xb, float* part,
                     float* stats, float* guard, int B, int T, int D, int heads, int dh, int Dm, float eps, void* stream,
                     hirest_bf16* xl = nullptr) {
    const int M = B * T, G = (D + 63) / 64;
    void* res = xl ? static_cast<void*>(xl) : static_cast<void*>(x);
    const int epi_res = xl ? HIREST_EPI_BIAS_RESID2_LNSTATS : HIREST_EPI_BIAS_RESID_LNSTATS_F32;
    CHECK(gemm(xb, D, w.qkv_wf, D, w.qkv_bf, big, 3 * D, M, 3 * D, D, HIREST_EPI_LNFOLD_BF16, stream, nullptr, 0, stats,
               const_cast<float*>(w.qkv_s)));
    CHECK(hirest_attention_bf16(big, h, B, T, heads, dh, 1.0f / sqrtf((float)dh), 0, stream));
    CHECK(gemm(h, D, w.proj_w, D, w.proj_b, res, D, M, D, D, epi_res, stream, nullptr, 0, xb, part));
    CHECK(hirest_ln_stats_finalize(part, G, stats, eps, M, D, guard, stream));
    CHECK(gemm(xb, D, w.fc1_wf, D, w.fc1_bf, big, Dm, M, Dm, D, HIREST_EPI_LNFOLD_GELU_BF16, stream, nullptr, 0, stats,
               const_cast<float*>(w.fc1_s)));
    CHECK(gemm(big, Dm, w.fc2_w, Dm, w.fc2_b, res, D, M, D, Dm, epi_res, stream, nullptr, 0, xb, part, HIREST_GEMM_REVERSE));
    CHECK(hirest_ln_stats_finalize(part, G, stats, eps, M, D, guard, stream));
    return 0;
}

int run_block_lnfold_cls(const hirest_block_weights& w, float* x, hirest_bf16* h, hirest_bf16* big, hirest_bf16* xb, float* part,
                         float* stats, float* guard, int B, int T, int D, int heads, int dh, int Dm, float eps, void* stream,
                         hirest_bf16* xl = nullptr, hirest_bf16* cls_hi = nullptr, hirest_bf16* cls_lo = nullptr) {
    const int M = B * T, G = (D + 63) / 64;
    const int64_t TD = (int64_t)T * D;
    CHECK(gemm(xb, D, w.qkv_wf, D, w.qkv_bf, big, 3 * D, M, 3 * D, D, HIREST_EPI_LNFOLD_BF16, stream, nullptr, 0, stats,
               const_cast<float*>(w.qkv_s)));
    CHECK(hirest_attention_bf16_rows(big, h, B, T, heads, dh, 1.0f / sqrtf((float)dh), 0, 1, stream));
    if (xl) {
        hipStream_t s = reinterpret_cast<hipStream_t>(stream);
        if (hipMemcpy2DAsync(cls_hi, (size_t)D * 2, xb, (size_t)TD * 2, (size_t)D * 2, B, hipMemcpyDeviceToDevice, s) != hipSuccess ||
            hipMemcpy2DAsync(cls_lo, (size_t)D * 2, xl, (size_t)TD * 2, (size_t)D * 2, B, hipMemcpyDeviceToDevice, s) != hipSuccess)
            return hirest_launch_status();
        CHECK(gemm(h, TD, w.proj_w, D, w.proj_b, cls_lo, D, B, D, D, HIREST_EPI_BIAS_RESID2_LNSTATS, stream, nullptr, 0, cls_hi, part));
        CHECK(hirest_ln_stats_finalize(part, G, stats, eps, B, D, guard, stream));
        CHECK(gemm(cls_hi, D, w.fc1_wf, D, w.fc1_bf, big, Dm, B, Dm, D, HIREST_EPI_LNFOLD_GELU_BF16, stream, nullptr, 0, stats,
                   const_cast<float*>(w.fc1_s)));
        CHECK(gemm(big, Dm, w.fc2_w, Dm, w.fc2_b, cls_lo, D, B, D, Dm, HIREST_EPI_BIAS_RESID2_LNSTATS, stream, nullptr, 0, cls_hi, part));
        return 0;
    }
    CHECK(gemm(h, TD, w.proj_w, D, w.proj_b, x, TD, B, D, D, HIREST_EPI_BIAS_RESID_LNSTATS_F32, stream, nullptr, 0, xb, part));
    CHECK(hirest_ln_stats_finalize(part, G, stats, eps, B, D, guard, stream));
    CHECK(gemm(xb, D, w.fc1_wf, D, w.fc1_bf, big, Dm, B, Dm, D, HIREST_EPI_LNFOLD_GELU_BF16, stream, nullptr, 0, stats,
               const_cast<float*>(w.fc1_s)));
    CHECK(gemm(big, Dm, w.fc2_w, Dm, w.fc2_b, x, TD, B, D, Dm, HIREST_EPI_BIAS_RESID_LNSTATS_F32, stream, nullptr, 0, xb, part));
    return 0;
}

}

extern "C" int hirest_abi_version(void) { return HIREST_ABI_VERSION; }

extern "C" const char* hirest_build_info(void) {
    return "hirest_hip gfx950 (CDNA4) | gemm pq256 (persistent ping-pong, 2 phases per K step, 16x16x32 bf16 MFMA) / p256 / t128 + LDS-DMA | "
           "bf16x3 split-operand GEMM + attention | attention 16x16x32 bf16 MFMA + tr16 reads | " __VERSION__;
}

extern "C" size_t hirest_vision_workspace_bytes(const hirest_vision_tower* t, int32_t B) {
    if (!t || B <= 0) return 0;
    const int T = (t->image_size / t->patch) * (t->image_size / t->patch) + 1;
    return plan((int64_t)B * T, t->width, vision_wide(t), B, vision_lnfold(t, B)).total;
}

extern "C" size_t hirest_vision_guard_offset(const hirest_vision_tower* t, int32_t B) {
    if (!t || B <= 0 || !vision_lnfold(t, B)) return (size_t)-1;
    const int T = (t->image_size / t->patch) * (t->image_size / t->patch) + 1;
    return plan((int64_t)B * T, t->width, vision_wide(t), B, true).guard;
}

extern "C" int hirest_vision_forward(const hirest_vision_tower* t, const void* frames, int32_t in_dtype, int32_t B,
                                     float* out, void* workspace, size_t workspace_bytes, int32_t flags, void* stream) {
    if (!t || !frames || !out || !workspace || B <= 0 || !t->blocks) return HIREST_E_BADARG;
    if (t->width != t->heads * t->head_dim || t->image_size % t->patch != 0) return HIREST_E_SHAPE;
    const int G = t->image_size / t->patch, P = G * G, T = P + 1, D = t->width;
    const bool can_fold = vision_lnfold(t, B), lnfold = can_fold && !(flags & HIREST_TOWER_NO_LNFOLD);
    const Regions r = plan((int64_t)B * T, D, vision_wide(t), B, can_fold);
    if (workspace_bytes < r.total) return HIREST_E_WORKSPACE;
    char* ws = reinterpret_cast<char*>(workspace);
    float* x = reinterpret_cast<float*>(ws + r.x);
    hirest_bf16* h = reinterpret_cast<hirest_bf16*>(ws + r.h);
    hirest_bf16* big = reinterpret_cast<hirest_bf16*>(ws + r.big);

    CHECK(hirest_patchify(frames, in_dtype, B, t->image_size, t->patch, t->image_mean, t->image_std, big, t->kpad, stream));
    CHECK(gemm(big, t->kpad, t->patch_w, t->kpad, t->patch_b, x, D, B * P, D, t->kpad, HIREST_EPI_PATCH_POS_F32, stream,
               t->pos, P));
    CHECK(hirest_write_cls_rows(x, D, t->cls, t->pos, B, T, D, stream));
    if (t->ln_pre_g)
        CHECK(hirest_layernorm(x, D, nullptr, t->ln_pre_g, t->ln_pre_b, t->ln_eps, x, D, 1, B * T, D, stream));
    int64_t cls_ldx = (int64_t)T * D;
    if (lnfold) {
        hirest_bf16* xb = reinterpret_cast<hirest_bf16*>(ws + r.xb);
        float* part = reinterpret_cast<float*>(ws + r.part);
        float* stats = reinterpret_cast<float*>(ws + r.stats);
        float* guard = reinterpret_cast<float*>(ws + r.guard);
        if (hipMemsetAsync(guard, 0, 256, reinterpret_cast<hipStream_t>(stream)) != hipSuccess) return hirest_launch_status();
        const bool prune = !t->out_all_tokens && !(flags & HIREST_TOWER_NO_PRUNE);
        hirest_bf16* xl = ((flags & HIREST_TOWER_F32_RESIDUAL) || (prune && t->layers == 1)) ? nullptr : reinterpret_cast<hirest_bf16*>(ws + r.xl);
        hirest_bf16* cls_hi = reinterpret_cast<hirest_bf16*>(ws + r.cls);
        hirest_bf16* cls_lo = reinterpret_cast<hirest_bf16*>(ws + r.cls + align256((size_t)B * D * 2));
        CHECK(hirest_rowstats_split_bf16(x, D, xb, xl, stats, t->ln_eps, B * T, D, guard, stream));
        for (int l = 0; l < t->layers; ++l) {
            if (prune && l == t->layers - 1) {
                CHECK(run_block_lnfold_cls(t->blocks[l], x, h, big, xb, part, stats, guard, B, T, D, t->heads, t->head_dim, t->mlp_dim,
                                           t->ln_eps, stream, xl, cls_hi, cls_lo));
            } else {
                CHECK(run_block_lnfold(t->blocks[l], x, h, big, xb, part, stats, guard, B, T, D, t->heads, t->head_dim, t->mlp_dim,
                                       t->ln_eps, stream, xl));
            }
        }
        if (xl && !prune) CHECK(hirest_combine_hi_lo_f32(xb, xl, D, x, D, B * T, D, stream));
        if (xl && prune) {
            CHECK(hirest_combine_hi_lo_f32(cls_hi, cls_lo, D, x, D, B, D, stream));
            cls_ldx = D;
        }
    } else {
        for (int l = 0; l < t->layers; ++l)
            CHECK(run_block(t->blocks[l], x, h, big, B, T, D, t->heads, t->head_dim, t->mlp_dim, t->ln_eps, t->act, 0, stream));
    }
    if (t->out_all_tokens) {
        CHECK(hirest_layernorm(x, D, nullptr, t->norm_g, t->norm_b, t->ln_eps, h, D, 0, B * T, D, stream));
        CHECK(gemm(h, D, t->head_w, D, t->head_b, out, t->embed_dim, B * T, t->embed_dim, D, HIREST_EPI_BIAS_F32, stream));
        return 0;
    }
    CHECK(hirest_layernorm(x, cls_ldx, nullptr, t->norm_g, t->norm_b, t->ln_eps, h, D, 0, B, D, stream));
    CHECK(gemm(h, D, t->head_w, D, t->head_b, out, t->embed_dim, B, t->embed_dim, D, HIREST_EPI_BIAS_F32, stream));
    return 0;
}

extern "C" size_t hirest_text_workspace_bytes(const hirest_text_tower* t, int32_t B) {
    if (!t || B <= 0) return 0;
    return plan((int64_t)B * t->context, t->width, 4 * t->width, B).total;
}

extern "C" int hirest_text_forward(const hirest_text_tower* t, const int64_t* tokens, int32_t B, float* out,
                                   void* workspace, size_t workspace_bytes, void* stream) {
    if (!t || !tokens || !out || !workspace || B <= 0 || !t->blocks) return HIREST_E_BADARG;
    if (t->width % t->heads != 0) return HIREST_E_SHAPE;
    const int L = t->context, D = t->width, dh = D / t->heads;
    const Regions r = plan((int64_t)B * L, D, 4 * D, B);
    if (workspace_bytes < r.total) return HIREST_E_WORKSPACE;
    char* ws = reinterpret_cast<char*>(workspace);
    float* x = reinterpret_cast<float*>(ws + r.x);
    hirest_bf16* h = reinterpret_cast<hirest_bf16*>(ws + r.h);
    hirest_bf16* big = reinterpret_cast<hirest_bf16*>(ws + r.big);
    int32_t* eot = reinterpret_cast<int32_t*>(ws + r.eot);

    CHECK(hirest_embed_tokens(tokens, t->tok_emb, t->pos, x, eot, B, L, D, t->vocab, stream));
    for (int l = 0; l < t->layers; ++l)
        CHECK(run_block(t->blocks[l], x, h, big, B, L, D, t->heads, dh, 4 * D, t->ln_eps, t->act, 1, stream));
    CHECK(hirest_layernorm(x, D, eot, t->lnf_g, t->lnf_b, t->ln_eps, h, D, 0, B, D, stream));
    CHECK(gemm(h, D, t->proj_w, D, nullptr, out, t->embed_dim, B, t->embed_dim, D, HIREST_EPI_BIAS_F32, stream));
    return 0;
}
```

### hirest_amd/eva_clip.py

```python
from __future__ import annotations

import ctypes as C
import json
import math
import os
from contextlib import contextmanager
from copy import deepcopy
from operator import attrgetter
from typing import Dict, Optional, Tuple

import numpy as np
import torch
from torch import nn

from . import _lib, ops, synth

OPENAI_DATASET_MEAN = (0.48145466, 0.4578275, 0.40821073)
OPENAI_DATASET_STD = (0.26862954, 0.26130258, 0.27577711)

TOWER_PRECISIONS = ("fp32", "bf16x3", "bf16")
_NO_GUARD = (1 << 64) - 1

_MODEL_CONFIGS: Dict[str, dict] = {"EVA_CLIP_g_14": synth.EVA_CLIP_G_14, "EVA_CLIP_tiny_test": synth.EVA_CLIP_TINY,
                                   "EVA_CLIP_tiny_e1024_test": dict(synth.EVA_CLIP_TINY, embed_dim=1024)}


def list_models():
    return list(_MODEL_CONFIGS.keys())


def add_model_config(path):
    paths = [os.path.join(path, f) for f in os.listdir(path)] if os.path.isdir(path) else [path]
    for p in paths:
        if p.endswith(".json"):
            cfg = json.load(open(p))
            if all(k in cfg for k in ("embed_dim", "vision_cfg", "text_cfg")):
                _MODEL_CONFIGS[os.path.splitext(os.path.basename(p))[0]] = cfg


def get_model_config(model_name):
    return deepcopy(_MODEL_CONFIGS[model_name]) if model_name in _MODEL_CONFIGS else None


class _Leaf(nn.Module):

    def __init__(self, **shapes):
        super().__init__()
        for name, shape in shapes.items():
            self.register_parameter(name, nn.Parameter(torch.zeros(shape), requires_grad=True))


def _linear(out_f, in_f, bias=True):
    return _Leaf(weight=(out_f, in_f), bias=(out_f,)) if bias else _Leaf(weight=(out_f, in_f))


def _norm(d):
    return _Leaf(weight=(d,), bias=(d,))


def _struct(struct, /, **fields):
    names = [n for n, _ in struct._fields_]
    if sorted(fields) != sorted(names):
        raise TypeError(f"{struct.__name__}: fields {sorted(set(fields) ^ set(names))} missing or unknown")
    return struct(**fields)


@contextmanager
def _precision_scope(towers):
    old = [t.precision for t, _ in towers]
    try:
        for t, p in towers:
            if p is not None:
                t.precision = p
        yield
    finally:
        for (t, _), p in zip(towers, old):
            t.precision = p


def _fold_rows(lin, weight, norm):
    return tuple((f"{lin}_{out}", f"fold{i}", (weight, f"{lin}_b", norm)) for i, out in enumerate(("wf", "bf", "s")))


_NO_FOLD = tuple((f, None, None) for f in ("qkv_wf", "qkv_bf", "qkv_s", "fc1_wf", "fc1_bf", "fc1_s"))
_RESBLOCK = (("ln1_g", "f32", "ln_1.weight"), ("ln1_b", "f32", "ln_1.bias"),
             ("qkv_w", "w", "attn.in_proj_weight"), ("qkv_b", "f32", "attn.in_proj_bias"),
             ("proj_w", "w", "attn.out_proj.weight"), ("proj_b", "f32", "attn.out_proj.bias"),
             ("ln2_g", "f32", "ln_2.weight"), ("ln2_b", "f32", "ln_2.bias"),
             ("fc1_w", "w", "mlp.c_fc.weight"), ("fc1_b", "f32", "mlp.c_fc.bias"),
             ("fc2_w", "w", "mlp.c_proj.weight"), ("fc2_b", "f32", "mlp.c_proj.bias"))


class _Tower(nn.Module):
    _TABLES: Dict[str, tuple] = {}
    _what = "tower"
    fold_layernorm = False

    def __init__(self):
        super().__init__()
        self._prepared = None
        self._workspace = None
        self.precision = "bf16"

    def _apply(self, fn, *a, **k):
        self._prepared = None
        self._workspace = None
        return super()._apply(fn, *a, **k)

    def _load_from_state_dict(self, *a, **k):
        self._prepared = None
        return super()._load_from_state_dict(*a, **k)

    def invalidate(self):
        self._prepared = None

    def _ws(self, nbytes: int, device) -> torch.Tensor:
        if self._workspace is None or self._workspace.numel() < nbytes or self._workspace.device != device:
            self._workspace = torch.empty(nbytes, dtype=torch.uint8, device=device)
        return self._workspace

    @staticmethod
    def _f32(p: torch.Tensor) -> torch.Tensor:
        return p.detach().float().contiguous()

    def _prepared_for(self, kind: str, device) -> dict:
        cache = self._prepared
        if cache is None or any(p["device"] != device for p in cache.values()):
            cache = self._prepared = {}
        if kind not in cache:
            if device.type != "cuda":
                raise RuntimeError(f"hirest_amd: the {self._what} runs on MI355X only (no CPU fallback); move the model to a GPU")
            desc_cls, rows, block_cls, block_rows = self._TABLES[kind]
            keep = []
            blocks = (block_cls * self.layers)()
            for i, b in enumerate(self._blocks()):
                blocks[i] = _struct(block_cls, **self._pointers(b, block_rows, kind, device, keep))
            if kind == "x3":
                base = self._prepared_for("fp32", device)
                keep.append(base)
                scalars = {"base": C.pointer(base["desc"])}
            else:
                scalars = self._scalars()
            desc = _struct(desc_cls, blocks=blocks, **scalars, **self._pointers(self, rows, kind, device, keep))
            cache[kind] = {"device": device, "desc": desc, "blocks": blocks, "keep": keep}
        return cache[kind]

    def _pointers(self, owner, rows, kind, device, keep) -> dict:
        cast = ops.to_bf16 if kind == "bf16" else (lambda t: t)
        fold = self.fold_layernorm and not self.quick_gelu
        done, folded = {}, {}
        for field, form, src in rows:
            if form is None or (form.startswith("fold") and not fold):
                t = None
            elif form == "const":
                t = torch.tensor(getattr(self, src), dtype=torch.float32, device=device)
            elif form.startswith("fold"):
                if src not in folded:
                    weight, bias, norm = src
                    folded[src] = self._fold(self._f32(attrgetter(weight)(owner)), done[bias], attrgetter(norm)(owner), device)
                t = folded[src][int(form[4:])]
            else:
                p = attrgetter(src)(owner)
                if form == "qkv_bias":
                    t = torch.cat([p.q_bias.detach().float(), torch.zeros(self.width, device=device), p.v_bias.detach().float()])
                elif form == "patch":
                    K = p[0].numel()
                    t = torch.zeros((self.width, self._scalars()["kpad"]), dtype=torch.float32, device=device)
                    t[:, :K] = p.detach().float().reshape(self.width, K)
                    t = cast(t)
                else:
                    t = self._f32(p.detach().float().t() if form == "wT" else p)
                    t = ops.split2(t) if form == "split" else t if form == "f32" else cast(t)
            done[field] = t
        keep.extend(t for t in done.values() if t is not None)
        return {f: None if t is None else t.data_ptr() for f, t in done.items()}

    def _fold(self, w32, bias, norm, device):
        N, K = w32.shape
        wf = torch.empty((N, K), dtype=torch.bfloat16, device=device)
        bf = torch.empty((N,), dtype=torch.float32, device=device)
        cs = torch.empty((N,), dtype=torch.float32, device=device)
        _lib.check(_lib.load().hirest_fold_layernorm(w32.data_ptr(), self._f32(norm.weight).data_ptr(), self._f32(norm.bias).data_ptr(),
                                                     bias.data_ptr(), wf.data_ptr(), bf.data_ptr(), cs.data_ptr(), N, K,
                                                     ops.stream_ptr()), "hirest_fold_layernorm")
        return wf, bf, cs

    @staticmethod
    def _call_size(B: int, limit, near_equal: bool) -> int:
        limit = max(1, int(limit))
        return -(-B // -(-B // limit)) if near_equal else min(B, limit)

    def _run_calls(self, B: int, limit, near_equal: bool, ws_bytes, call, device):
        if B <= 0:
            return []
        step = self._call_size(B, limit, near_equal)
        ws = self._ws(ws_bytes(step), device)
        spans = [(s, min(step, B - s)) for s in range(0, B, step)]
        for s, n in spans:
            call(s, n, ws)
        return spans


class VisionTower(_Tower):
    _what = "vision tower"
    _FIELDS = (("patch_w", "patch", "patch_embed.proj.weight"), ("patch_b", "f32", "patch_embed.proj.bias"),
               ("cls", "f32", "cls_token"), ("pos", "f32", "pos_embed"), ("norm_g", "f32", "norm.weight"), ("norm_b", "f32", "norm.bias"),
               ("head_w", "w", "head.weight"), ("head_b", "f32", "head.bias"),
               ("image_mean", "const", "image_mean"), ("image_std", "const", "image_std"), ("ln_pre_g", None, None), ("ln_pre_b", None, None))
    _BLOCK = (("ln1_g", "f32", "norm1.weight"), ("ln1_b", "f32", "norm1.bias"),
              ("qkv_w", "w", "attn.qkv.weight"), ("qkv_b", "qkv_bias", "attn"),
              ("proj_w", "w", "attn.proj.weight"), ("proj_b", "f32", "attn.proj.bias"),
              ("ln2_g", "f32", "norm2.weight"), ("ln2_b", "f32", "norm2.bias"),
              ("fc1_w", "w", "mlp.fc1.weight"), ("fc1_b", "f32", "mlp.fc1.bias"),
              ("fc2_w", "w", "mlp.fc2.weight"), ("fc2_b", "f32", "mlp.fc2.bias"))
    _TABLES = {"bf16": (_lib.VisionTower, _FIELDS, _lib.BlockWeights,
                        _BLOCK + _fold_rows("qkv", "attn.qkv.weight", "norm1") + _fold_rows("fc1", "mlp.fc1.weight", "norm2")),
               "fp32": (_lib.VisionTowerF32, _FIELDS, _lib.BlockWeightsF32, _BLOCK),
               "x3": (_lib.VisionTowerX3, (), _lib.BlockWeightsX3, tuple((f + "2", "split", src) for f, form, src in _BLOCK if form == "w"))}

    def __init__(self, image_size, patch_size, width, layers, heads, mlp_ratio, embed_dim, quick_gelu=False):
        super().__init__()
        self.image_size, self.patch_size, self.width, self.layers, self.heads = image_size, patch_size, width, layers, heads
        self.mlp_dim = int(width * mlp_ratio)
        self.embed_dim = self.num_classes = embed_dim
        self.quick_gelu = quick_gelu
        self.num_tokens = (image_size // patch_size) ** 2 + 1
        D, Dm = width, self.mlp_dim
        self.cls_token = nn.Parameter(torch.zeros(1, 1, D))
        self.pos_embed = nn.Parameter(torch.zeros(1, self.num_tokens, D))
        self.patch_embed = nn.Module()
        self.patch_embed.proj = _Leaf(weight=(D, 3, patch_size, patch_size), bias=(D,))
        blocks = []
        for _ in range(layers):
            b = nn.Module()
            b.norm1, b.norm2 = _norm(D), _norm(D)
            b.attn = _Leaf(q_bias=(D,), v_bias=(D,))
            b.attn.qkv = _linear(3 * D, D, bias=False)
            b.attn.proj = _linear(D, D)
            b.mlp = nn.Module()
            b.mlp.fc1, b.mlp.fc2 = _linear(Dm, D), _linear(D, Dm)
            blocks.append(b)
        self.blocks = nn.ModuleList(blocks)
        self.norm = _norm(D)
        self.head = _linear(embed_dim, D)
        self.image_mean, self.image_std = OPENAI_DATASET_MEAN, OPENAI_DATASET_STD
        self.max_frames_per_call = 1024
        self.max_frames_per_call_f32 = 256
        self.max_frames_per_call_x3 = 1024
        self.fold_layernorm = True
        self.fold_guard_ratio = 4.0
        self.last_fold_ratio = 0.0
        self.fold_fallbacks = 0
        self.prune_last_block = True
        self.f32_residual = os.environ.get("HIREST_F32_RESIDUAL", "0") == "1"

    def _blocks(self):
        return self.blocks

    def _scalars(self):
        P = self.patch_size
        return dict(image_size=self.image_size, patch=P, width=self.width, heads=self.heads, head_dim=self.width // self.heads,
                    mlp_dim=self.mlp_dim, layers=self.layers, embed_dim=self.embed_dim, kpad=(3 * P * P + 63) // 64 * 64,
                    act=1 if self.quick_gelu else 0, ln_eps=1e-6,
                    out_all_tokens=0)

    _EXACT = {"fp32": ("fp32", "hirest_vision_workspace_bytes_f32", "hirest_vision_forward_f32", "max_frames_per_call_f32", False),
              "bf16x3": ("x3", "hirest_vision_workspace_bytes_x3", "hirest_vision_forward_x3", "max_frames_per_call_x3", True)}

    def _forward_exact(self, image: torch.Tensor) -> torch.Tensor:
        kind, ws_bytes, fwd, limit, near_equal = self._EXACT[self.precision]
        desc = C.byref(self._prepared_for(kind, image.device)["desc"])
        lib = _lib.load()
        out = torch.empty((image.shape[0], self.embed_dim), dtype=torch.float32, device=image.device)
        code = ops._IN_DTYPES[image.dtype]

        def call(s, n, ws):
            _lib.check(getattr(lib, fwd)(desc, image[s:s + n].data_ptr(), code, n, out[s:s + n].data_ptr(), ws.data_ptr(), ws.numel(),
                                         ops.stream_ptr()), fwd)
        self._run_calls(image.shape[0], getattr(self, limit), near_equal, lambda n: getattr(lib, ws_bytes)(desc, n), call, image.device)
        return out

    @torch.no_grad()
    @ops.on_tensor_device
    def forward(self, image: torch.Tensor) -> torch.Tensor:
        if image.dtype == torch.uint8:
            H, W = image.shape[1], image.shape[2]
        else:
            H, W = image.shape[-2], image.shape[-1]
            if image.dtype not in (torch.float32, torch.bfloat16):
                image = image.float()
        assert H == self.image_size and W == self.image_size, \
            f"Input image size ({H}*{W}) doesn't match model ({self.image_size}*{self.image_size})."
        image = image.contiguous()
        if self.precision in self._EXACT:
            return self._forward_exact(image)
        desc = C.byref(self._prepared_for("bf16", image.device)["desc"])
        lib = _lib.load()
        B = image.shape[0]
        out = torch.empty((B, self.embed_dim), dtype=torch.float32, device=image.device)
        if B == 0:
            return out
        step = self._call_size(B, self.max_frames_per_call, True)
        code = ops._IN_DTYPES[image.dtype]
        self.last_fold_ratio = 0.0
        flags = (0 if self.prune_last_block else _lib.TOWER_NO_PRUNE) | (_lib.TOWER_F32_RESIDUAL if self.f32_residual else 0)
        goff = lib.hirest_vision_guard_offset(desc, step) if self.fold_guard_ratio is not None else _NO_GUARD
        guards = torch.zeros(-(-B // step), dtype=torch.float32, device=image.device) if goff != _NO_GUARD else None

        def call(s, n, ws, extra=0):
            _lib.check(lib.hirest_vision_forward(desc, image[s:s + n].data_ptr(), code, n, out[s:s + n].data_ptr(),
                                                 ws.data_ptr(), ws.numel(), flags | extra, ops.stream_ptr()), "hirest_vision_forward")

        def guarded(s, n, ws):
            call(s, n, ws)
            if guards is not None:
                g = lib.hirest_vision_guard_offset(desc, n)
                if g != _NO_GUARD:
                    guards[s // step:s // step + 1].copy_(ws[g:g + 4].view(torch.float32))
        spans = self._run_calls(B, self.max_frames_per_call, True, lambda n: lib.hirest_vision_workspace_bytes(desc, n), guarded, image.device)
        if guards is not None:
            ratios = guards.cpu().tolist()
            self.last_fold_ratio = max(ratios)
            for (s, n), ratio in zip(spans, ratios):
                if not ratio <= self.fold_guard_ratio:
                    self.fold_fallbacks += 1
                    call(s, n, self._workspace, _lib.TOWER_NO_LNFOLD)
        return out


class TextTower(_Tower):
    _what = "text tower"
    _FIELDS = (("tok_emb", "f32", "token_embedding.weight"), ("pos", "f32", "positional_embedding"),
               ("lnf_g", "f32", "ln_final.weight"), ("lnf_b", "f32", "ln_final.bias"), ("proj_w", "wT", "text_projection"))
    _TABLES = {"bf16": (_lib.TextTower, _FIELDS, _lib.BlockWeights, _RESBLOCK + _NO_FOLD),
               "fp32": (_lib.TextTowerF32, _FIELDS, _lib.BlockWeightsF32, _RESBLOCK)}

    def __init__(self, vocab_size, width, layers, heads, context_length, embed_dim, quick_gelu=False):
        super().__init__()
        self.vocab_size, self.width, self.layers, self.heads = vocab_size, width, layers, heads
        self.context_length, self.embed_dim, self.quick_gelu = context_length, embed_dim, quick_gelu
        D = width
        self.token_embedding = _Leaf(weight=(vocab_size, D))
        self.positional_embedding = nn.Parameter(torch.zeros(context_length, D))
        self.transformer = nn.Module()
        blocks = []
        for _ in range(layers):
            b = nn.Module()
            b.ln_1, b.ln_2 = _norm(D), _norm(D)
            b.attn = _Leaf(in_proj_weight=(3 * D, D), in_proj_bias=(3 * D,))
            b.attn.out_proj = _linear(D, D)
            b.mlp = nn.Module()
            b.mlp.c_fc, b.mlp.c_proj = _linear(4 * D, D), _linear(D, 4 * D)
            blocks.append(b)
        self.transformer.resblocks = nn.ModuleList(blocks)
        self.ln_final = _norm(D)
        self.text_projection = nn.Parameter(torch.zeros(D, embed_dim))
        self.logit_scale = nn.Parameter(torch.ones([]) * math.log(1 / 0.07))
        self.max_rows_per_call = 1024

    def _blocks(self):
        return self.transformer.resblocks

    def _scalars(self):
        return dict(context=self.context_length, vocab=self.vocab_size, width=self.width, heads=self.heads, layers=self.layers,
                    embed_dim=self.embed_dim, act=1 if self.quick_gelu else 0, ln_eps=1e-5)

    @torch.no_grad()
    @ops.on_tensor_device
    def forward(self, text: torch.Tensor) -> torch.Tensor:
        if text.dim() != 2 or text.shape[1] != self.context_length:
            raise RuntimeError(f"encode_text expects [B,{self.context_length}] token ids, got {tuple(text.shape)}")
        f32 = self.precision == "fp32"
        desc = C.byref(self._prepared_for("fp32" if f32 else "bf16", text.device)["desc"])
        lib = _lib.load()
        text = text.to(torch.int64).contiguous()
        out = torch.empty((text.shape[0], self.embed_dim), dtype=torch.float32, device=text.device)
        ws_bytes, fwd = (lib.hirest_text_workspace_bytes_f32, lib.hirest_text_forward_f32) if f32 else \
            (lib.hirest_text_workspace_bytes, lib.hirest_text_forward)

        def call(s, n, ws):
            _lib.check(fwd(desc, text[s:s + n].data_ptr(), n, out[s:s + n].data_ptr(), ws.data_ptr(), ws.numel(), ops.stream_ptr()),
                       "hirest_text_forward_f32" if f32 else "hirest_text_forward")
        self._run_calls(text.shape[0], self.max_rows_per_call, False, lambda n: ws_bytes(desc, n), call, text.device)
        return out


class EVA_CLIP(nn.Module):

    def __init__(self, embed_dim: int, vision_cfg: dict, text_cfg: dict, quick_gelu: bool = False):
        super().__init__()
        v, t = dict(vision_cfg), dict(text_cfg)
        self.visual = VisionTower(v.get("image_size", 224), v.get("patch_size", 16), v.get("width", 768),
                                  v.get("layers", 12), v.get("width", 768) // v.get("head_width", 64),
                                  v.get("mlp_ratio", 4.0), embed_dim)
        self.text = TextTower(t.get("vocab_size", 49408), t.get("width", 512), t.get("layers", 12), t.get("heads", 8),
                              t.get("context_length", 77), embed_dim, quick_gelu)
        self.output_dtype = torch.float32

    def set_precision(self, precision: str):
        if precision not in TOWER_PRECISIONS:
            raise ValueError(f"precision must be one of {TOWER_PRECISIONS}, got {precision!r}")
        self.visual.precision = precision
        self.text.precision = "fp32" if precision == "bf16x3" else precision
        return self

    def precision_scope(self, visual: Optional[str] = None, text: Optional[str] = None):
        for precision in (visual, text):
            if precision is not None and precision not in TOWER_PRECISIONS:
                raise ValueError(f"precision must be one of {TOWER_PRECISIONS}, got {precision!r}")
        return _precision_scope(((self.visual, visual), (self.text, "fp32" if text == "bf16x3" else text)))

    @torch.no_grad()
    def init_random_(self, seed: int = 0):
        gen = torch.Generator(device=next(self.parameters()).device)
        gen.manual_seed(seed)
        for name, p in self.named_parameters():
            std, mean = synth._init_rule(name, tuple(p.shape))
# ... 132 lines not shown
```

### hirest_amd/ops.py

```python
from __future__ import annotations

import ctypes as C
import functools
from typing import Optional

import torch

from . import _lib
from ._lib import (EPI_BIAS_BF16, EPI_BIAS_F32, EPI_BIAS_GELU_BF16, EPI_BIAS_QGELU_BF16, EPI_BIAS_RESID_F32,
                   EPI_PATCH_POS_F32)

__all__ = ["gemm", "layernorm", "attention", "patchify", "write_cls_rows", "embed_tokens", "to_bf16",
           "pool_l2norm", "similarity", "topk", "clip_score", "stream_ptr", "on_tensor_device"]


_raw_stream = getattr(torch._C, "_cuda_getCurrentRawStream", None)


def stream_ptr() -> int:
    if _raw_stream is not None:
        return _raw_stream(torch.cuda.current_device())
    return torch.cuda.current_stream().cuda_stream


def on_tensor_device(fn):
    @functools.wraps(fn)
    def wrapped(*args, **kw):
        for a in list(args) + list(kw.values()):
            if isinstance(a, torch.Tensor) and a.is_cuda:
                if a.device.index != torch.cuda.current_device():
                    with torch.cuda.device(a.device):
                        return fn(*args, **kw)
                break
        return fn(*args, **kw)
    return wrapped


def _dev(t: torch.Tensor, dtype, name: str) -> int:
    if not isinstance(t, torch.Tensor) or not t.is_cuda:
        raise RuntimeError(f"{name}: expected a GPU tensor (the HIP path has no CPU fallback)")
    if t.dtype != dtype:
        raise RuntimeError(f"{name}: expected dtype {dtype}, got {t.dtype}")
    if not t.is_contiguous():
        raise RuntimeError(f"{name}: expected a contiguous tensor")
    return t.data_ptr()


def _opt(t: Optional[torch.Tensor], dtype, name: str) -> Optional[int]:
    return None if t is None else _dev(t, dtype, name)


@on_tensor_device
def gemm(a: torch.Tensor, w: torch.Tensor, bias: Optional[torch.Tensor], out: torch.Tensor, epilogue: int,
         pos: Optional[torch.Tensor] = None, patches_per_frame: int = 0,
         aux0: Optional[torch.Tensor] = None, aux1: Optional[torch.Tensor] = None, flags: int = 0) -> torch.Tensor:
    lib = _lib.load()
    M, K = a.shape
    N = w.shape[0]
    if w.shape[1] != K:
        raise RuntimeError(f"gemm: K mismatch {a.shape} x {w.shape}")
    out_dtype = torch.bfloat16 if epilogue in (EPI_BIAS_BF16, EPI_BIAS_GELU_BF16, EPI_BIAS_QGELU_BF16, _lib.EPI_LNFOLD_BF16,
                                              _lib.EPI_LNFOLD_GELU_BF16, _lib.EPI_BIAS_RESID2_LNSTATS) else torch.float32
    args = _lib.GemmArgs.make(_dev(a, torch.bfloat16, "gemm.a"), K, _dev(w, torch.bfloat16, "gemm.w"), K,
                         _opt(bias, torch.float32, "gemm.bias"), _dev(out, out_dtype, "gemm.out"), out.shape[-1],
                         M, N, K, epilogue, _opt(pos, torch.float32, "gemm.pos"), patches_per_frame,
                         None if aux0 is None else _dev(aux0, aux0.dtype, "gemm.aux0"),
                         None if aux1 is None else _dev(aux1, aux1.dtype, "gemm.aux1"), int(flags))
    _lib.check(lib.hirest_gemm_bf16(C.byref(args), stream_ptr()), "hirest_gemm_bf16")
    return out


def gemm_select_kernel(which: int):
    _lib.check(_lib.load().hirest_gemm_select_kernel(int(which)), "hirest_gemm_select_kernel")


ATTENTION_DEFAULT_KERNEL = 7


def attention_select_kernel(which: int):
    _lib.check(_lib.load().hirest_attention_select_kernel(int(which)), "hirest_attention_select_kernel")


def attention_set_mapping(by_head: Optional[bool] = None):
    _lib.check(_lib.load().hirest_attention_set_mapping(2 if by_head is None else int(bool(by_head))), "hirest_attention_set_mapping")


@on_tensor_device
def layernorm(x: torch.Tensor, gamma: torch.Tensor, beta: torch.Tensor, eps: float, out: torch.Tensor,
              row_index: Optional[torch.Tensor] = None, ldx: Optional[int] = None, rows: Optional[int] = None):
    lib = _lib.load()
    D = gamma.numel()
    rows = rows if rows is not None else (row_index.numel() if row_index is not None else x.numel() // D)
    ldx = ldx if ldx is not None else D
    out_f32 = 1 if out.dtype == torch.float32 else 0
    _lib.check(lib.hirest_layernorm(_dev(x, torch.float32, "ln.x"), ldx, _opt(row_index, torch.int32, "ln.row_index"),
                                    _dev(gamma, torch.float32, "ln.gamma"), _dev(beta, torch.float32, "ln.beta"),
                                    float(eps), _dev(out, out.dtype, "ln.out"), D, out_f32, rows, D, stream_ptr()),
               "hirest_layernorm")
    return out


@on_tensor_device
def attention(qkv: torch.Tensor, out: torch.Tensor, B: int, N: int, H: int, dh: int, causal: bool,
              scale: Optional[float] = None):
    lib = _lib.load()
    scale = dh ** -0.5 if scale is None else scale
    _lib.check(lib.hirest_attention_bf16(_dev(qkv, torch.bfloat16, "attn.qkv"), _dev(out, torch.bfloat16, "attn.out"),
                                         B, N, H, dh, float(scale), int(bool(causal)), stream_ptr()),
               "hirest_attention_bf16")
    return out


_IN_DTYPES = {torch.float32: 0, torch.bfloat16: 1, torch.uint8: 2}


@on_tensor_device
def patchify(frames: torch.Tensor, patch: int, kpad: int, out: torch.Tensor, mean=None, std=None):
    lib = _lib.load()
    if frames.dtype not in _IN_DTYPES:
        raise RuntimeError(f"patchify: unsupported frame dtype {frames.dtype}")
    code = _IN_DTYPES[frames.dtype]
    B = frames.shape[0]
    S = frames.shape[-1] if code != 2 else frames.shape[1]
    _lib.check(lib.hirest_patchify(_dev(frames, frames.dtype, "patchify.frames"), code, B, S, patch,
                                   _opt(mean, torch.float32, "mean"), _opt(std, torch.float32, "std"),
                                   _dev(out, torch.bfloat16, "patchify.out"), kpad, stream_ptr()), "hirest_patchify")
    return out


@on_tensor_device
def write_cls_rows(x: torch.Tensor, cls: torch.Tensor, pos0: torch.Tensor, B: int, T: int, D: int):
    lib = _lib.load()
    _lib.check(lib.hirest_write_cls_rows(_dev(x, torch.float32, "x"), D, _dev(cls, torch.float32, "cls"),
                                         _dev(pos0, torch.float32, "pos"), B, T, D, stream_ptr()), "hirest_write_cls_rows")
    return x


@on_tensor_device
def embed_tokens(tokens: torch.Tensor, tok_emb: torch.Tensor, pos: torch.Tensor, x: torch.Tensor, eot_row: torch.Tensor):
    lib = _lib.load()
    B, L = tokens.shape
    V, D = tok_emb.shape
    _lib.check(lib.hirest_embed_tokens(_dev(tokens, torch.int64, "tokens"), _dev(tok_emb, torch.float32, "tok_emb"),
                                       _dev(pos, torch.float32, "pos"), _dev(x, torch.float32, "x"),
                                       _dev(eot_row, torch.int32, "eot_row"), B, L, D, V, stream_ptr()), "hirest_embed_tokens")
    return x


@on_tensor_device
def to_bf16(t: torch.Tensor) -> torch.Tensor:
    lib = _lib.load()
    t = t.contiguous()
    out = torch.empty(t.shape, dtype=torch.bfloat16, device=t.device)
    n = t.numel()
    if n % 4 != 0:
        raise RuntimeError("to_bf16: element count must be a multiple of 4")
    _lib.check(lib.hirest_f32_to_bf16(_dev(t, torch.float32, "to_bf16.in"), out.data_ptr(), n, stream_ptr()), "hirest_f32_to_bf16")
    return out


@on_tensor_device
def split2(x: torch.Tensor, gelu: bool = False) -> torch.Tensor:
    lib = _lib.load()
    rows, D = x.shape
    out = torch.empty((rows, 2 * D), dtype=torch.bfloat16, device=x.device)
    _lib.check(lib.hirest_split2_bf16(_dev(x, torch.float32, "split2.in"), D, out.data_ptr(), 2 * D, rows, D, int(bool(gelu)), stream_ptr()),
               "hirest_split2_bf16")
    return out


@on_tensor_device
def gemm_x3(a2: torch.Tensor, w2: torch.Tensor, bias: Optional[torch.Tensor] = None, resid_out: Optional[torch.Tensor] = None,
            gelu_split: bool = False, stream=None) -> torch.Tensor:
    lib = _lib.load()
    M, K2 = a2.shape
    N = w2.shape[0]
    if gelu_split:
        out = torch.empty((M, 2 * N), dtype=torch.bfloat16, device=a2.device)
        args = _lib.GemmArgs.make(_dev(a2, torch.bfloat16, "gemm_x3.a"), K2, _dev(w2, torch.bfloat16, "gemm_x3.w"), K2,
                                  _opt(bias, torch.float32, "gemm_x3.bias"), out.data_ptr(), 2 * N, M, N, K2, _lib.EPI_BIAS_GELU_SPLIT2, None, 0,
                                  None, None, _lib.GEMM_X3)
        _lib.check(lib.hirest_gemm_bf16(C.byref(args), stream_ptr()), "hirest_gemm_bf16 (x3, gelu + split)")
        return out
    out = resid_out if resid_out is not None else torch.empty((M, N), dtype=torch.float32, device=a2.device)
    epi = _lib.EPI_BIAS_RESID_F32 if resid_out is not None else _lib.EPI_BIAS_F32
    args = _lib.GemmArgs.make(_dev(a2, torch.bfloat16, "gemm_x3.a"), K2, _dev(w2, torch.bfloat16, "gemm_x3.w"), K2,
                              _opt(bias, torch.float32, "gemm_x3.bias"), out.data_ptr(), N, M, N, K2, epi, None, 0, None, None, _lib.GEMM_X3)
    _lib.check(lib.hirest_gemm_bf16(C.byref(args), stream_ptr() if stream is None else stream), "hirest_gemm_bf16 (x3)")
    return out


@on_tensor_device
def pool_l2norm(frame_embeds: torch.Tensor, normalize_frames_first: bool = False) -> torch.Tensor:
    lib = _lib.load()
    V, F, E = frame_embeds.shape
    out = torch.empty((V, E), dtype=torch.float32, device=frame_embeds.device)
    _lib.check(lib.hirest_pool_l2norm(_dev(frame_embeds, torch.float32, "pool.in"), out.data_ptr(), V, F, E,
                                      int(bool(normalize_frames_first)), stream_ptr()), "hirest_pool_l2norm")
    return out


@on_tensor_device
def similarity(text_n: torch.Tensor, video_n: torch.Tensor) -> torch.Tensor:
    lib = _lib.load()
    Q, E = text_n.shape
    V = video_n.shape[0]
    out = torch.empty((Q, V), dtype=torch.float32, device=text_n.device)
    _lib.check(lib.hirest_similarity_f32(_dev(text_n, torch.float32, "sim.text"), _dev(video_n, torch.float32, "sim.video"),
                                         out.data_ptr(), Q, V, E, stream_ptr()), "hirest_similarity_f32")
    return out


def gemm_f32_strided(a: torch.Tensor, b: torch.Tensor, alpha: float = 1.0) -> torch.Tensor:
    lib = _lib.load()
    M, K = a.shape
    N = b.shape[0]
    out = torch.empty((M, N), dtype=torch.float32, device=a.device)
    _lib.check(lib.hirest_gemm_f32_strided(_dev(a, torch.float32, "gemm.a"), a.stride(0), 1, _dev(b, torch.float32, "gemm.b"), b.stride(0), 1,
                                           out.data_ptr(), N, M, N, K, float(alpha), stream_ptr()), "hirest_gemm_f32_strided")
    return out


@on_tensor_device
def topk(scores: torch.Tensor, k: int, tie_rank: Optional[torch.Tensor] = None):
    lib = _lib.load()
    Q, V = scores.shape
    idx = torch.empty((Q, k), dtype=torch.int32, device=scores.device)
    val = torch.empty((Q, k), dtype=torch.float32, device=scores.device)
    if V >= 16384:
        need = lib.hirest_topk_workspace_bytes(Q, V, k)
        ws = torch.empty(need, dtype=torch.uint8, device=scores.device)
        _lib.check(lib.hirest_topk_f32_ws(_dev(scores, torch.float32, "topk.scores"), _opt(tie_rank, torch.int32, "topk.tie_rank"),
                                          Q, V, k, idx.data_ptr(), val.data_ptr(), ws.data_ptr(), need, stream_ptr()),
                   "hirest_topk_f32_ws")
        return val, idx
    _lib.check(lib.hirest_topk_f32(_dev(scores, torch.float32, "topk.scores"), _opt(tie_rank, torch.int32, "topk.tie_rank"),
                                   Q, V, k, idx.data_ptr(), val.data_ptr(), stream_ptr()), "hirest_topk_f32")
    return val, idx



@on_tensor_device
def clip_score(img_rows: torch.Tensor, txt_rows: torch.Tensor, sel) -> torch.Tensor:
    lib = _lib.load()
    if img_rows.dim() != 2 or txt_rows.dim() != 2 or img_rows.shape[1] != txt_rows.shape[1]:
        raise RuntimeError(f"clip_score: expected [U, E] and [C, E] rows, got {tuple(img_rows.shape)} and {tuple(txt_rows.shape)}")
    sel = torch.as_tensor(sel)
    U, E = img_rows.shape
    C = txt_rows.shape[0]
    if sel.dim() != 2 or sel.shape[0] != C or sel.shape[1] < 1:
        raise RuntimeError(f"clip_score: sel must be [C={C}, K>=1], got {tuple(sel.shape)}")
    if sel.numel() and (int(sel.min()) < 0 or int(sel.max()) >= U):
        raise RuntimeError(f"clip_score: row ids must lie in [0, {U})")
    for t, name in ((img_rows, "clip_score.img"), (txt_rows, "clip_score.txt")):
        if t.dtype not in (torch.float32, torch.bfloat16):
            raise RuntimeError(f"{name}: expected fp32 or bf16 rows, got {t.dtype}")
    out = torch.empty(C, dtype=torch.float32, device=img_rows.device)
    sel = sel.to(device=img_rows.device, dtype=torch.int32).contiguous()
    _lib.check(lib.hirest_clip_score(_dev(img_rows, img_rows.dtype, "clip_score.img"), _IN_DTYPES[img_rows.dtype], U,
# ... 101 lines not shown
```

### include/hirest_hip.h

```cpp
#ifndef HIREST_HIP_H
#define HIREST_HIP_H

#include <stddef.h>
#include <stdint.h>

#ifdef __cplusplus
extern "C" {
#endif

#define HIREST_ABI_VERSION 4

#define HIREST_E_BADARG   (-1)
#define HIREST_E_SHAPE    (-2)
#define HIREST_E_WORKSPACE (-3)

typedef uint16_t hirest_bf16;

int hirest_abi_version(void);
const char* hirest_build_info(void);

enum hirest_epilogue {
    HIREST_EPI_BIAS_BF16 = 0,
    HIREST_EPI_BIAS_GELU_BF16 = 1,
    HIREST_EPI_BIAS_QGELU_BF16 = 2,
    HIREST_EPI_BIAS_RESID_F32 = 3,
    HIREST_EPI_BIAS_F32 = 4,
    HIREST_EPI_PATCH_POS_F32 = 5,
    HIREST_EPI_BIAS_RESID_LNSTATS_F32 = 6,
    HIREST_EPI_LNFOLD_BF16 = 7,
    HIREST_EPI_LNFOLD_GELU_BF16 = 8,
    HIREST_EPI_BIAS_GELU_SPLIT2 = 9,
    HIREST_EPI_BIAS_RESID2_LNSTATS = 10
};

typedef struct hirest_gemm_args {
    uint64_t struct_size;
    const hirest_bf16* A;  int64_t lda;
    const hirest_bf16* W;  int64_t ldw;
    const float* bias;
    void* out;             int64_t ldo;
    int32_t M, N, K;
    int32_t epilogue;
    const float* pos;
    int32_t patches_per_frame;
    void* aux0;
    void* aux1;
    int32_t flags;
} hirest_gemm_args;
enum { HIREST_GEMM_REVERSE = 1,
       HIREST_GEMM_X3 = 2,
       HIREST_GEMM_X3_T128 = 4
     };

int hirest_gemm_bf16(const hirest_gemm_args* args, void* stream);
int hirest_gemm_select_kernel(int32_t which);
int hirest_gemm_debug_mode(int32_t bits);
int hirest_gemm_dispatch_name(const hirest_gemm_args* args, char* out, int32_t out_len);

int hirest_layernorm(const float* x, int64_t ldx, const int32_t* row_index,
                     const float* gamma, const float* beta, float eps,
                     void* out, int64_t ldo, int32_t out_is_f32,
                     int32_t rows, int32_t D, void* stream);

int hirest_attention_bf16(const hirest_bf16* qkv, hirest_bf16* out,
                          int32_t B, int32_t N, int32_t H, int32_t dh,
                          float scale, int32_t causal, void* stream);
int hirest_attention_bf16_rows(const hirest_bf16* qkv, hirest_bf16* out,
                               int32_t B, int32_t N, int32_t H, int32_t dh,
                               float scale, int32_t causal, int32_t q_rows, void* stream);
int hirest_attention_select_kernel(int32_t which);
int hirest_attention_set_mapping(int32_t by_head);
int hirest_attention_set_pace(int32_t units);
int hirest_attention_set_stagger(int32_t units);
int hirest_attention_set_skew(int32_t units);
int hirest_attention_debug_mode(int32_t bits);
int hirest_attention_debug_trace_read(int64_t* dst, int32_t n);

int hirest_patchify(const void* frames, int32_t in_dtype, int32_t B, int32_t S, int32_t P,
                    const float* mean3, const float* std3,
                    hirest_bf16* patches, int32_t Kpad, void* stream);

int hirest_fold_layernorm(const float* W, const float* gamma, const float* beta, const float* bias, hirest_bf16* Wf,
                          float* bias_out, float* colsum_out, int32_t N, int32_t K, void* stream);
int hirest_write_cls_rows(float* x, int64_t ldx, const float* cls, const float* pos0,
                          int32_t B, int32_t tokens_per_frame, int32_t D, void* stream);

int hirest_rowstats_bf16(const float* x, int64_t ldx, hirest_bf16* xb, float* stats, float eps, int32_t rows, int32_t D,
                         float* guard, void* stream);
int hirest_rowstats_split_bf16(const float* x, int64_t ldx, hirest_bf16* xb, hirest_bf16* xlo, float* stats, float eps, int32_t rows,
                               int32_t D, float* guard, void* stream);
int hirest_combine_hi_lo_f32(const hirest_bf16* hi, const hirest_bf16* lo, int64_t ld_in, float* out, int64_t ldo, int32_t rows,
                             int32_t D, void* stream);
int hirest_ln_stats_finalize(const float* partials, int32_t groups, float* stats, float eps, int32_t rows, int32_t D,
                             float* guard, void* stream);

int hirest_embed_tokens(const int64_t* tokens, const float* tok_emb, const float* pos,
                        float* x, int32_t* eot_row, int32_t B, int32_t L, int32_t D,
                        int32_t vocab, void* stream);

int hirest_f32_to_bf16(const float* in, hirest_bf16* out, int64_t n, void* stream);

int hirest_pool_l2norm(const float* frame_embeds, float* out, int32_t V, int32_t F, int32_t E,
                       int32_t normalize_frames_first, void* stream);
int hirest_pool_l2norm_varlen(const float* rows, const int32_t* seg_off, float* out, int32_t V, int32_t E, void* stream);

int hirest_similarity_f32(const float* text_n, const float* video_n, float* scores,
                          int32_t Q, int32_t V, int32_t E, void* stream);

int hirest_topk_f32(const float* scores, const int32_t* tie_rank, int32_t Q, int32_t V, int32_t k,
                    int32_t* out_index, float* out_score, void* stream);
int64_t hirest_topk_workspace_bytes(int32_t Q, int32_t V, int32_t k);
int hirest_topk_f32_ws(const float* scores, const int32_t* tie_rank, int32_t Q, int32_t V, int32_t k,
                       int32_t* out_index, float* out_score, void* workspace, int64_t workspace_bytes, void* stream);
int hirest_clip_score(const void* img_rows, int32_t img_dtype, int32_t U, const void* txt_rows, int32_t txt_dtype,
                      const int32_t* sel, int32_t C, int32_t K, int32_t E, float* out, void* stream);

#define HIREST_BERTSCORE_MAX_TOKENS 1024
int hirest_bertscore_greedy(const float* states, int64_t ld, int32_t D, const int32_t* seq_off, int32_t n_seq,
                            const float* tok_weight, const int32_t* cand_seq, const int32_t* ref_seq, int32_t n_pairs,
                            float* out , void* stream);

typedef struct hirest_block_weights {
    const float* ln1_g; const float* ln1_b;
    const hirest_bf16* qkv_w; const float* qkv_b;
    const hirest_bf16* proj_w; const float* proj_b;
    const float* ln2_g; const float* ln2_b;
    const hirest_bf16* fc1_w; const float* fc1_b;
    const hirest_bf16* fc2_w; const float* fc2_b;
    const hirest_bf16* qkv_wf; const float* qkv_bf; const float* qkv_s;
    const hirest_bf16* fc1_wf; const float* fc1_bf; const float* fc1_s;
} hirest_block_weights;

typedef struct hirest_vision_tower {
    int32_t image_size, patch, width, heads, head_dim, mlp_dim, layers, embed_dim;
    int32_t kpad;
    int32_t act;
    float ln_eps;
    const hirest_bf16* patch_w;
    const float* patch_b;
    const float* cls;
    const float* pos;
    const hirest_block_weights* blocks;
    const float* norm_g; const float* norm_b;
    const hirest_bf16* head_w;
    const float* head_b;
    const float* image_mean; const float* image_std;
    const float* ln_pre_g; const float* ln_pre_b;
    int32_t out_all_tokens;
} hirest_vision_tower;

size_t hirest_vision_workspace_bytes(const hirest_vision_tower* t, int32_t B);
enum { HIREST_TOWER_NO_LNFOLD = 1,
       HIREST_TOWER_NO_PRUNE = 2,
       HIREST_TOWER_F32_RESIDUAL = 4 };
int hirest_vision_forward(const hirest_vision_tower* t, const void* frames, int32_t in_dtype,
                          int32_t B, float* out, void* workspace, size_t workspace_bytes,
                          int32_t flags, void* stream);
size_t hirest_vision_guard_offset(const hirest_vision_tower* t, int32_t B);

typedef struct hirest_text_tower {
    int32_t context, vocab, width, heads, layers, embed_dim;
    int32_t act;
    float ln_eps;
    const float* tok_emb;
    const float* pos;
    const hirest_block_weights* blocks;
    const float* lnf_g; const float* lnf_b;
    const hirest_bf16* proj_w;
} hirest_text_tower;

size_t hirest_text_workspace_bytes(const hirest_text_tower* t, int32_t B);
int hirest_text_forward(const hirest_text_tower* t, const int64_t* tokens, int32_t B, float* out,
                        void* workspace, size_t workspace_bytes, void* stream);

typedef struct hirest_block_weights_f32 {
    const float* ln1_g; const float* ln1_b;
    const float* qkv_w; const float* qkv_b;
    const float* proj_w; const float* proj_b;
    const float* ln2_g; const float* ln2_b;
    const float* fc1_w; const float* fc1_b;
    const float* fc2_w; const float* fc2_b;
} hirest_block_weights_f32;

typedef struct hirest_vision_tower_f32 {
    int32_t image_size, patch, width, heads, head_dim, mlp_dim, layers, embed_dim;
    int32_t kpad;
    int32_t act;
    float ln_eps;
    const float* patch_w;
    const float* patch_b; const float* cls; const float* pos;
    const hirest_block_weights_f32* blocks;
    const float* norm_g; const float* norm_b;
    const float* head_w; const float* head_b;
    const float* image_mean; const float* image_std;
    const float* ln_pre_g; const float* ln_pre_b;
    int32_t out_all_tokens;
} hirest_vision_tower_f32;

typedef struct hirest_text_tower_f32 {
    int32_t context, vocab, width, heads, layers, embed_dim;
    int32_t act;
    float ln_eps;
    const float* tok_emb; const float* pos;
    const hirest_block_weights_f32* blocks;
    const float* lnf_g; const float* lnf_b;
    const float* proj_w;
} hirest_text_tower_f32;

size_t hirest_vision_workspace_bytes_f32(const hirest_vision_tower_f32* t, int32_t B);
int hirest_vision_forward_f32(const hirest_vision_tower_f32* t, const void* frames, int32_t in_dtype, int32_t B, float* out,
                              void* workspace, size_t workspace_bytes, void* stream);
int hirest_vision_embed_f32(const hirest_vision_tower_f32* t, const void* frames, int32_t in_dtype, int32_t B, float* x, float* rows,
                            void* stream);
size_t hirest_text_workspace_bytes_f32(const hirest_text_tower_f32* t, int32_t B);
int hirest_text_forward_f32(const hirest_text_tower_f32* t, const int64_t* tokens, int32_t B, float* out,
                            void* workspace, size_t workspace_bytes, void* stream);

typedef struct hirest_block_weights_x3 {
    const hirest_bf16* qkv_w2;
    const hirest_bf16* proj_w2;
    const hirest_bf16* fc1_w2;
    const hirest_bf16* fc2_w2;
} hirest_block_weights_x3;

typedef struct hirest_vision_tower_x3 {
    const hirest_vision_tower_f32* base;
    const hirest_block_weights_x3* blocks;
} hirest_vision_tower_x3;

int hirest_split2_bf16(const float* x, int64_t ldx, hirest_bf16* out, int64_t ldo, int64_t rows, int32_t D, int32_t act, void* stream);
int hirest_split2_transposed_bf16(const float* x, int64_t ldx, hirest_bf16* out, int64_t ldo, int32_t rows, int32_t cols, void* stream);
#define HIREST_SPLIT_GROUP_MAX 16
typedef struct hirest_split_item {
    const float* x; hirest_bf16* out;
    int64_t ldx, ldo;
    int32_t rows, cols, transposed, reserved;
} hirest_split_item;
int hirest_split2_grouped_bf16(const hirest_split_item* items, int32_t count, void* stream);
int hirest_layernorm_split2(const float* x, int64_t ldx, const float* gamma, const float* beta, float eps, hirest_bf16* out, int64_t ldo,
                            int32_t rows, int32_t D, void* stream);
int hirest_attention_x3_qkv(const float* q, int64_t ldq, const float* k, const float* v, int64_t ldkv, float* out, int32_t B, int32_t Tq,
                            int32_t Tk, int32_t H, int32_t dh, float scale, void* stream);
int hirest_attention_x3_qkv_split2(const float* q, int64_t ldq, const float* k, const float* v, int64_t ldkv, hirest_bf16* out2, int32_t B,
                                   int32_t Tq, int32_t Tk, int32_t H, int32_t dh, float scale, void* stream);
int hirest_attention_x3_select_waves(int32_t waves);
int hirest_attention_x3_debug_trace(int64_t* device_buffer);
int hirest_vision_x3_select_attention(int32_t which);
size_t hirest_vision_workspace_bytes_x3(const hirest_vision_tower_x3* t, int32_t B);
int hirest_vision_forward_x3(const hirest_vision_tower_x3* t, const void* frames, int32_t in_dtype, int32_t B, float* out,
                             void* workspace, size_t workspace_bytes, void* stream);

int hirest_gemm_f32(const float* A, int64_t lda, const float* W, int64_t ldw, const float* bias,
                    const float* resid, int64_t ldr, const float* periodic, int32_t period,
                    float* out, int64_t ldo, int32_t M, int32_t N, int32_t K, int32_t act, void* stream);
size_t hirest_gemm_f32_workspace_bytes(int32_t M, int32_t N, int32_t K);
int hirest_gemm_f32_ws(const float* A, int64_t lda, const float* W, int64_t ldw, const float* bias, const float* resid, int64_t ldr,
                       const float* periodic, int32_t period, float* out, int64_t ldo, int32_t M, int32_t N, int32_t K, int32_t act,
                       void* workspace, size_t workspace_bytes, void* stream);
size_t hirest_gemm_f32_layouts_workspace_bytes(int32_t M, int32_t N, int32_t K);
int hirest_gemm_f32_layouts(const float* A, int64_t lda, int32_t a_kmajor, const float* W, int64_t ldw, int32_t w_kmajor,
                            const float* bias, const float* resid, int64_t ldr, float* out, int64_t ldo, int32_t M, int32_t N,
                            int32_t K, int32_t act, void* workspace, size_t workspace_bytes, void* stream);
int hirest_gemm_f32_select_kernel(int32_t which);
int hirest_gemm_f32_ring_mode(int32_t mode);
int hirest_gemm_f32_ln(const float* X, int64_t ldx, const int32_t* ids, const float* table, const float* pos_row,
                       const float* gamma, const float* beta, float eps, float* ln_out, int64_t ldl, const float* W, int64_t ldw,
                       const float* bias, const float* resid, int64_t ldr, float* out, int64_t ldo, int32_t M, int32_t N, int32_t K,
                       int32_t act, void* stream);
int hirest_gemm_f32_ln_colmax(const float* X, int64_t ldx, const float* gamma, const float* beta, float eps, const float* W, int64_t ldw,
                              const float* bias, float* out, int64_t ldo, float* colmax, int32_t M, int32_t N, int32_t K, void* stream);
int hirest_gemm_f32_rows_ln_mode(int32_t mode);
int hirest_gemm_f32_rows_preferred(int32_t M);
int hirest_gemm_f32_rows_colmax(const float* A, int64_t lda, const float* W, int64_t ldw, const float* bias, float* out, int64_t ldo,
                                float* colmax, int32_t M, int32_t N, int32_t K, void* stream);
#define HIREST_F32_ENTRY_GEMM 0
#define HIREST_F32_ENTRY_WS 1
#define HIREST_F32_ENTRY_LAYOUTS 2
#define HIREST_F32_ENTRY_LN 3
#define HIREST_F32_ENTRY_LN_COLMAX 4
#define HIREST_F32_ENTRY_ROWS_COLMAX 5
typedef struct hirest_gemm_f32_query {
    uint32_t struct_size;
    int32_t entry;
    int32_t M, N, K;
    int32_t has_resid, has_periodic;
    int32_t has_ids, has_ln_out;
    int32_t has_workspace;
    int32_t a_kmajor, w_kmajor;
    int32_t select_kernel, ring_mode, rows_ln_mode;
    int32_t cus;
} hirest_gemm_f32_query;
int hirest_gemm_f32_dispatch_name(const hirest_gemm_f32_query* query, char* out, int32_t out_len);
int hirest_attention_f32(const float* qkv, float* out, int32_t B, int32_t T, int32_t H, int32_t dh,
                         float scale, float add_const, void* stream);
int hirest_attention_f32_qkv(const float* q, int64_t ldq, const float* k, const float* v, int64_t ldkv, float* out,
                             int32_t B, int32_t Tq, int32_t Tk, int32_t H, int32_t dh, float scale, float add_const,
                             float causal_penalty, void* stream);
int hirest_attention_f32_varlen(const float* qkv, float* out, const int32_t* seq_off, int32_t B, int32_t max_len, int32_t H,
                                int32_t dh, float scale, float add_const, void* stream);
int hirest_log_softmax_f32(const float* x, int64_t ldx, const float* row_add, float* out, int64_t ldo, int32_t rows,
                           int32_t V, void* stream);
int hirest_joint_time_features(const int32_t* n_valid, const float* w1, const float* b1, float* tin,
                               int32_t B, int32_t T, int32_t E, void* stream);
int hirest_joint_time_grid_f32(const int32_t* n_valid, int32_t B, int32_t T, float* grid, void* stream);
int hirest_joint_base(const float* v, const float* text_proj, const float* asr, const float* temporal, float* base,
                      int32_t B, int32_t T, int32_t E, void* stream);
int hirest_joint_mask_add(const float* base, const int32_t* moment_mask, const int32_t* boundary_mask,
                          const float* mask_embed, const float* boundary_embed, float* f, int64_t rows, int32_t E,
                          void* stream);
int hirest_linear_heads(const float* x, int64_t rows, int32_t D, int32_t nheads, const float* w0, const float* w1,
                        const float* w2, const float* bias3, float* logits, void* stream);
typedef struct hirest_caption_layer {
    const float* qkv_w; const float* qkv_b;
    const float* so_w; const float* so_b; const float* so_ln_g; const float* so_ln_b;
    const float* cq_w; const float* cq_b;
    const float* co_w; const float* co_b; const float* co_ln_g; const float* co_ln_b;
    const float* ff1_w; const float* ff1_b;
    const float* ff2_w; const float* ff2_b; const float* ff_ln_g; const float* ff_ln_b;
} hirest_caption_layer;
typedef struct hirest_caption_decoder {
    int32_t layers, heads, hidden, inter, vocab_padded, max_pos;
    const float* word_emb; const float* pos_emb; const float* emb_ln_g; const float* emb_ln_b;
    const hirest_caption_layer* layer;
    const float* tr_w; const float* tr_b; const float* tr_ln_g; const float* tr_ln_b;
    const float* lm_w; const float* lm_b;
    const hirest_bf16* lm_w2;
} hirest_caption_decoder;
size_t hirest_caption_step_workspace_bytes(const hirest_caption_decoder* d, int32_t R);
int hirest_caption_decode_step(const hirest_caption_decoder* d, int32_t R, int32_t position, const int32_t* last_ids,
                               const int32_t* parent_rows, const float* const* kv_in, float* const* kv_out,
                               const float* const* enc_kv, int32_t F, const float* row_add, float* logp,
                               void* workspace, size_t workspace_bytes, void* stream);

int hirest_attention_f32_decode(const float* q, int64_t ldq, const float* k_hist, const float* v_hist, int64_t ld_hist,
                                const int32_t* parent, int32_t t_hist, const float* k_new, const float* v_new, int64_t ld_new,
                                float* k_out, float* v_out, float* out, int32_t R, int32_t H, float scale, float add_const,
                                float causal_penalty, void* stream);
int hirest_caption_select(int32_t mode);
int hirest_caption_decode_logits(const hirest_caption_decoder* d, int32_t R, int32_t position, const int32_t* last_ids,
                                 const int32_t* parent_rows, const float* const* kv_in, float* const* kv_out,
                                 const float* const* enc_kv, int32_t F, float* logits, void* workspace, size_t workspace_bytes,
                                 void* stream);
size_t hirest_caption_beam_tail_workspace_bytes(int32_t B, int32_t beam, int32_t vocab);
int hirest_caption_beam_tail(const float* logits, int64_t ldx, const float* row_add, int32_t B, int32_t beam, int32_t vocab,
                             int32_t step, int32_t max_steps, int32_t eos_id, float* scores, int32_t* tokens, int32_t* backptr,
                             int32_t* n_steps, int32_t* done, int32_t* next_ids, int32_t* next_parents, float* next_add,
                             int32_t* done_host, void* workspace, size_t workspace_bytes, void* stream);

int hirest_caption_beam_step(const hirest_caption_decoder* d, int32_t B, int32_t beam, int32_t position, int32_t* ids, int32_t* parent_rows,
// ... 408 lines not shown
```

Baseline: 2198.

## Permute folded QKV weight columns per head and pass layout to attention

Adds a QKV column layout descriptor so the folded QKV weights can be reordered at load time (q0 k0 | v0 k1 q1 | ... ordering), placing each head's q, k, v columns near each other. The attention kernels now compute per-head q/k/v base offsets from the layout instead of assuming contiguous Q|K|V blocks. The intent is better memory locality when attention reads each head's q/k/v slices from the QKV GEMM output. It costs a small amount of index arithmetic in the kernels, adds a field to the tower structs, and is enabled by default for EVA vision towers that use layernorm folding.

Result: no change. 2202 (median of 6 runs) (+0.2%).

```diff
diff --git a/hirest_amd/_lib.py b/hirest_amd/_lib.py
--- a/hirest_amd/_lib.py
+++ b/hirest_amd/_lib.py
@@ -64,7 +64,27 @@
                 ("blocks", C.POINTER(BlockWeights)),
                 ("norm_g", C.c_void_p), ("norm_b", C.c_void_p), ("head_w", C.c_void_p), ("head_b", C.c_void_p),
                 ("image_mean", C.c_void_p), ("image_std", C.c_void_p),
-                ("ln_pre_g", C.c_void_p), ("ln_pre_b", C.c_void_p), ("out_all_tokens", C.c_int32)]
+                ("ln_pre_g", C.c_void_p), ("ln_pre_b", C.c_void_p), ("out_all_tokens", C.c_int32),
+                ("qkv_fold_order", C.c_int32)]
+
+
+class QkvLayout(C.Structure):
+    _fields_ = [("first", C.c_int32 * 3), ("base", C.c_int32 * 3), ("step", C.c_int32 * 3)]
+
+    @classmethod
+    def make(cls, order: int, H: int, dh: int):
+        D, i3 = H * dh, C.c_int32 * 3
+        if order == 1:
+            return cls(i3(0, dh, 2 * dh), i3(dh, 0, 2 * dh), i3(3 * dh, 3 * dh, 3 * dh))
+        return cls(i3(0, D, 2 * D), i3(0, D, 2 * D), i3(dh, dh, dh))
+
+    def columns(self, H: int, dh: int):
+        perm = [0] * (3 * H * dh)
+        for x in range(3):
+            for h in range(H):
+                c = self.first[x] if h == 0 else self.base[x] + h * self.step[x]
+                perm[c:c + dh] = range(x * H * dh + h * dh, x * H * dh + (h + 1) * dh)
+        return perm
 
 
 class TextTower(C.Structure):
@@ -263,6 +283,8 @@
                                         C.c_float, C.c_int32, C.c_void_p]),
     "hirest_attention_bf16_rows": (C.c_int, [C.c_void_p, C.c_void_p, C.c_int32, C.c_int32, C.c_int32, C.c_int32,
                                              C.c_float, C.c_int32, C.c_int32, C.c_void_p]),
+    "hirest_attention_bf16_layout": (C.c_int, [C.c_void_p, C.c_void_p, C.c_int32, C.c_int32, C.c_int32, C.c_int32,
+                                               C.c_float, C.c_int32, C.c_int32, C.c_void_p, C.c_void_p]),
     "hirest_fold_layernorm": (C.c_int, [C.c_void_p, C.c_void_p, C.c_void_p, C.c_void_p, C.c_void_p, C.c_void_p, C.c_void_p, C.c_int32,
                                         C.c_int32, C.c_void_p]),
     "hirest_patchify": (C.c_int, [C.c_void_p, C.c_int32, C.c_int32, C.c_int32, C.c_int32, C.c_void_p, C.c_void_p,
diff --git a/hirest_amd/clip.py b/hirest_amd/clip.py
--- a/hirest_amd/clip.py
+++ b/hirest_amd/clip.py
@@ -66,7 +66,8 @@
         return dict(image_size=self.input_resolution, patch=P, width=D, heads=self.heads, head_dim=D // self.heads, mlp_dim=4 * D,
                     layers=self.layers, embed_dim=self.output_dim, kpad=(3 * P * P + 63) // 64 * 64,
                     act=1, ln_eps=1e-5,
-                    out_all_tokens=1)
+                    out_all_tokens=1,
+                    qkv_fold_order=0)
 
     @torch.no_grad()
     def forward(self, x: torch.Tensor) -> torch.Tensor:
diff --git a/hirest_amd/csrc/attention.hip b/hirest_amd/csrc/attention.hip
--- a/hirest_amd/csrc/attention.hip
+++ b/hirest_amd/csrc/attention.hip
@@ -3,6 +3,8 @@
 #include "profile.h"
 
 namespace {
+
+__device__ __forceinline__ int qkv_col(const hirest_qkv_layout& L, int x, int h) { return h == 0 ? L.first[x] : L.base[x] + h * L.step[x]; }
 
 template <int DH, int DP, int NT>
 struct AttnCfg {
@@ -16,7 +18,7 @@
 
 template <int DH, int DP, int NT>
 __global__ __launch_bounds__(512) void attention_kernel(const bf16_t* __restrict__ qkv, bf16_t* __restrict__ out,
-                                                       int N, int H, float scale_log2e, int causal, int nq) {
+                                                       int N, int H, float scale_log2e, int causal, int nq, hirest_qkv_layout L) {
     using C = AttnCfg<DH, DP, NT>;
     extern __shared__ __attribute__((aligned(16))) char smem[];
     char* Ks = smem;
@@ -25,20 +27,21 @@
     const int b = blockIdx.x / H, h = blockIdx.x - b * H;
     const int D = H * DH;
     const int64_t ld = 3 * (int64_t)D;
-    const bf16_t* base = qkv + (int64_t)b * N * ld + h * DH;
+    const bf16_t* frame = qkv + (int64_t)b * N * ld;
+    const bf16_t *qs = frame + qkv_col(L, 0, h), *ks = frame + qkv_col(L, 1, h), *vs = frame + qkv_col(L, 2, h);
 
     constexpr int KCH = DP / 8;
     for (int idx = tid; idx < C::NPAD * KCH; idx += 512) {
         const int key = idx / KCH, ch = idx - key * KCH;
         bf16x8 v = {0, 0, 0, 0, 0, 0, 0, 0};
-        if (key < N && ch * 8 < DH) v = *reinterpret_cast<const bf16x8*>(base + (int64_t)key * ld + D + ch * 8);
+        if (key < N && ch * 8 < DH) v = *reinterpret_cast<const bf16x8*>(ks + (int64_t)key * ld + ch * 8);
         *reinterpret_cast<bf16x8*>(Ks + key * C::KRS + ch * 16) = v;
     }
     constexpr int VCH = DH / 8;
     for (int idx = tid; idx < C::KP * VCH; idx += 512) {
         const int ch = idx / C::KP, key = idx - ch * C::KP;
         bf16x8 v = {0, 0, 0, 0, 0, 0, 0, 0};
-        if (key < N) v = *reinterpret_cast<const bf16x8*>(base + (int64_t)key * ld + 2 * D + ch * 8);
+        if (key < N) v = *reinterpret_cast<const bf16x8*>(vs + (int64_t)key * ld + ch * 8);
 #pragma unroll
         for (int e = 0; e < 8; ++e) *reinterpret_cast<bf16_t*>(Vt + (ch * 8 + e) * C::VRS + key * 2) = v[e];
     }
@@ -54,7 +57,7 @@
         for (int kk = 0; kk < DP / 32; ++kk) {
             const int d = (kk * 4 + g) * 8;
             bf16x8 v = {0, 0, 0, 0, 0, 0, 0, 0};
-            if (qvalid && d < DH) v = *reinterpret_cast<const bf16x8*>(base + (int64_t)q * ld + d);
+            if (qvalid && d < DH) v = *reinterpret_cast<const bf16x8*>(qs + (int64_t)q * ld + d);
             qf[kk] = v;
         }
         f32x4 st[NT];
@@ -127,12 +130,12 @@
 }
 
 template <int DH, int DP, int NT>
-int launch(const bf16_t* qkv, bf16_t* out, int B, int N, int H, float scale, int causal, int nq, hipStream_t s) {
+int launch(const bf16_t* qkv, bf16_t* out, int B, int N, int H, float scale, int causal, int nq, const hirest_qkv_layout& L, hipStream_t s) {
     using C = AttnCfg<DH, DP, NT>;
     static HirestDevCfg cfg;
     auto kern = attention_kernel<DH, DP, NT>;
     if (int e = hirest_configure(kern, C::LDS_BYTES, cfg)) return e;
-    hipLaunchKernelGGL(kern, dim3(B * H), dim3(512), C::LDS_BYTES, s, qkv, out, N, H, scale * 1.44269504088896340736f, causal, nq);
+    hipLaunchKernelGGL(kern, dim3(B * H), dim3(512), C::LDS_BYTES, s, qkv, out, N, H, scale * 1.44269504088896340736f, causal, nq, L);
     return hirest_launch_status();
 }
 
@@ -165,7 +168,7 @@
 
 template <int DH, int DP, int NT>
 __global__ __launch_bounds__(512) void attention_kernel_v2(const bf16_t* __restrict__ qkv, bf16_t* __restrict__ out,
-                                                          int N, int H, float scale_log2e, int causal, int nq) {
+                                                          int N, int H, float scale_log2e, int causal, int nq, hirest_qkv_layout L) {
     using C = AttnCfg2<DH, DP, NT>;
     extern __shared__ __attribute__((aligned(16))) char smem[];
     char* Ks = smem;
@@ -175,7 +178,8 @@
     const int b = blockIdx.x / H, h = blockIdx.x - b * H;
     const int D = H * DH;
     const int64_t ld = 3 * (int64_t)D;
-    const bf16_t* base = qkv + (int64_t)b * N * ld + h * DH;
+    const bf16_t* frame = qkv + (int64_t)b * N * ld;
+    const bf16_t *qs = frame + qkv_col(L, 0, h), *ks = frame + qkv_col(L, 1, h), *vs = frame + qkv_col(L, 2, h);
 
     int nv_mine = 0;
     for (int i = wave; i < C::NK_INSTR; i += 8) {
@@ -184,14 +188,14 @@
         c = (c & ~3) | ((c & 3) ^ ((-(row >> 2)) & 3));
         row = row < N ? row : N - 1;
         c = c * 8 < DH ? c : DH / 8 - 1;
-        glds16(base + (int64_t)row * ld + D + c * 8, Ks + i * 1024);
+        glds16(ks + (int64_t)row * ld + c * 8, Ks + i * 1024);
     }
     for (int i = wave; i < C::NV_INSTR; i += 8) {
         const int ci = i * 64 + lane;
         int row = ci / C::CPR, c = ci - row * C::CPR;
         row = row < N ? row : N - 1;
         c = c * 8 < DH ? c : DH / 8 - 1;
-        glds16(base + (int64_t)row * ld + 2 * D + c * 8, Vs + i * 1024);
+        glds16(vs + (int64_t)row * ld + c * 8, Vs + i * 1024);
         ++nv_mine;
     }
     wait_vm_le(nv_mine);
@@ -209,7 +213,7 @@
         for (int kk = 0; kk < DP / 32; ++kk) {
             const int d = (kk * 4 + g) * 8;
             bf16x8 v = {0, 0, 0, 0, 0, 0, 0, 0};
-            if (qvalid && d < DH) v = *reinterpret_cast<const bf16x8*>(base + (int64_t)q * ld + d);
+            if (qvalid && d < DH) v = *reinterpret_cast<const bf16x8*>(qs + (int64_t)q * ld + d);
             qf[kk] = v;
         }
         f32x4 st[NT];
@@ -311,7 +315,7 @@
 template <int DH, int DP, int NT, bool FAST, bool DBG, int NW = 9, bool LEAN = false, bool PROD = false>
 __global__ __launch_bounds__((NW + (PROD ? 1 : 0)) * 64) void attention_kernel_v3(const bf16_t* __restrict__ qkv, bf16_t* __restrict__ out,
                                                           int N, int H, float scale_log2e, int causal, int dbg_bits, int nq, int skew,
-                                                          int B, int map, int pace, int stagger) {
+                                                          int B, int map, int pace, int stagger, hirest_qkv_layout L) {
     const int dbg = DBG ? dbg_bits : 0;
     using C = AttnCfg2<DH, DP, NT>;
     extern __shared__ __attribute__((aligned(16))) char smem[];
@@ -329,7 +333,7 @@
     }
     if (nsteps == 0) return;
     if (stagger > 0 && blockIdx.x < 256) sleep_n(((blockIdx.x >> 3) & 15) * stagger);
-    auto sbase = [&](int st) { return qkv + (int64_t)(b0 + st * bstep) * N * ld + (h0 + st * hstep) * DH; };
+    auto sbase = [&](int st, int x) { return qkv + (int64_t)(b0 + st * bstep) * N * ld + qkv_col(L, x, h0 + st * hstep); };
     const int g = lane >> 4, c16 = lane & 15;
     const int gk = g ^ ((-(c16 >> 2)) & 3);
     const int nqt = (nq + 15) >> 4;
@@ -344,7 +348,7 @@
     constexpr int ROWS_PER_PIECE = NW * 64 / C::CPR;
     auto dma_k = [&](int h, char* dst) -> int {
         int n = 0;
-        const bf16_t* src = sbase(h) + D;
+        const bf16_t* src = sbase(h, 1);
         for (int i = wave, row = row0; i < C::NK_INSTR; i += NW, row += ROWS_PER_PIECE) {
             int kc = (col0 & ~3) | ((col0 & 3) ^ ((-(row >> 2)) & 3));
             const bool kpad = kc * 8 >= DH;
@@ -360,7 +364,7 @@
     constexpr bool SUM_IN_MFMA = LEAN && DP > DH;
     const bool vpad = SUM_IN_MFMA && vlog * 8 >= DH;
     auto dma_v = [&](int h) {
-        const bf16_t* src = sbase(h) + 2 * D + vc * 8;
+        const bf16_t* src = sbase(h, 2) + vc * 8;
         for (int i = wave, row = row0; i < C::NV_INSTR; i += NW, row += ROWS_PER_PIECE) {
             const int r = row < N ? row : N - 1;
             const void* from = src + (int64_t)r * ld;
@@ -370,7 +374,7 @@
     };
     auto load_q = [&](int h, int qtile, bf16x8 (&dst)[DP / 32]) {
         const int q = qtile * 16 + c16;
-        const bf16_t* base = sbase(h);
+        const bf16_t* base = sbase(h, 0);
         if (LEAN && DP > DH) {
             const bf16_t* row = base + (int64_t)(q < N ? q : N - 1) * ld;
 #pragma unroll
@@ -406,7 +410,7 @@
             pvoff[j] = (vl * 8 < DH ? vl : DH / 8 - 1) * 8;
         }
         auto issue_k = [&](int st, char* dst, int pace_units) {
-            const bf16_t* src = sbase(st) + D;
+            const bf16_t* src = sbase(st, 1);
             for (int it0 = 0; it0 < C::NK_INSTR / PER; ++it0) {
                 const int it = map ? (it0 + h0) % (C::NK_INSTR / PER) : it0;
 #pragma unroll
@@ -420,7 +424,7 @@
             }
         };
         auto issue_v = [&](int st) {
-            const bf16_t* src = sbase(st) + 2 * D;
+            const bf16_t* src = sbase(st, 2);
             for (int it0 = 0; it0 < C::NV_INSTR / PER; ++it0) {
                 const int it = map ? (it0 + h0) % (C::NV_INSTR / PER) : it0;
 #pragma unroll
@@ -631,7 +635,7 @@
 std::atomic<int> g_attn_variant{7};
 
 template <int DH, int DP, int NT, bool FAST, bool DBG, int NW = 9, bool LEAN = false, bool PROD = false>
-int launch3_impl(const bf16_t* qkv, bf16_t* out, int B, int N, int H, float scale, int causal, int nq, hipStream_t s) {
+int launch3_impl(const bf16_t* qkv, bf16_t* out, int B, int N, int H, float scale, int causal, int nq, const hirest_qkv_layout& L, hipStream_t s) {
     using C = AttnCfg2<DH, DP, NT>;
     constexpr int LDS = (2 * C::NPAD + C::KP) * C::RS;
     static_assert(LDS <= 163840, "K x2 + V must fit the CU's LDS");
@@ -641,31 +645,31 @@
     const bool by_head = (g_attn_map == 1 || (g_attn_map == 2 && B < 256)) && H <= 32 && 32 % H == 0 && B >= 8 * (32 / H) * 4;
     const int grid = by_head ? 256 : B;
     hipLaunchKernelGGL(kern, dim3(grid), dim3((NW + (PROD ? 1 : 0)) * 64), LDS, s, qkv, out, N, H, scale * 1.44269504088896340736f, causal, g_attn_dbg, nq,
-                       g_attn_skew, B, by_head ? 1 : 0, g_attn_pace, g_attn_stagger);
+                       g_attn_skew, B, by_head ? 1 : 0, g_attn_pace, g_attn_stagger, L);
     return hirest_launch_status();
 }
 
 template <int DH, int DP, int NT, bool FAST>
-int launch3(const bf16_t* qkv, bf16_t* out, int B, int N, int H, float scale, int causal, int nq, hipStream_t s) {
-    if (g_attn_dbg && FAST && g_attn_variant == 6) return launch3_impl<DH, DP, NT, FAST, true, 9, true, true>(qkv, out, B, N, H, scale, causal, nq, s);
-    if (g_attn_variant == 6) return launch3_impl<DH, DP, NT, FAST, false, 9, true, true>(qkv, out, B, N, H, scale, causal, nq, s);
-    if (g_attn_dbg && FAST && g_attn_variant == 7) return launch3_impl<DH, DP, NT, FAST, true, 9, false, true>(qkv, out, B, N, H, scale, causal, nq, s);
-    if (g_attn_variant == 7) return launch3_impl<DH, DP, NT, FAST, false, 9, false, true>(qkv, out, B, N, H, scale, causal, nq, s);
-    if (g_attn_dbg && FAST && g_attn_variant == 5) return launch3_impl<DH, DP, NT, FAST, true, 9, true>(qkv, out, B, N, H, scale, causal, nq, s);
-    if (g_attn_dbg && FAST) return launch3_impl<DH, DP, NT, FAST, true>(qkv, out, B, N, H, scale, causal, nq, s);
-    if (g_attn_variant == 4) return launch3_impl<DH, DP, NT, FAST, false, 12>(qkv, out, B, N, H, scale, causal, nq, s);
-    if (g_attn_variant == 5) return launch3_impl<DH, DP, NT, FAST, false, 9, true>(qkv, out, B, N, H, scale, causal, nq, s);
-    return launch3_impl<DH, DP, NT, FAST, false>(qkv, out, B, N, H, scale, causal, nq, s);
+int launch3(const bf16_t* qkv, bf16_t* out, int B, int N, int H, float scale, int causal, int nq, const hirest_qkv_layout& L, hipStream_t s) {
+    if (g_attn_dbg && FAST && g_attn_variant == 6) return launch3_impl<DH, DP, NT, FAST, true, 9, true, true>(qkv, out, B, N, H, scale, causal, nq, L, s);
+    if (g_attn_variant == 6) return launch3_impl<DH, DP, NT, FAST, false, 9, true, true>(qkv, out, B, N, H, scale, causal, nq, L, s);
+    if (g_attn_dbg && FAST && g_attn_variant == 7) return launch3_impl<DH, DP, NT, FAST, true, 9, false, true>(qkv, out, B, N, H, scale, causal, nq, L, s);
+    if (g_attn_variant == 7) return launch3_impl<DH, DP, NT, FAST, false, 9, false, true>(qkv, out, B, N, H, scale, causal, nq, L, s);
+    if (g_attn_dbg && FAST && g_attn_variant == 5) return launch3_impl<DH, DP, NT, FAST, true, 9, true>(qkv, out, B, N, H, scale, causal, nq, L, s);
+    if (g_attn_dbg && FAST) return launch3_impl<DH, DP, NT, FAST, true>(qkv, out, B, N, H, scale, causal, nq, L, s);
+    if (g_attn_variant == 4) return launch3_impl<DH, DP, NT, FAST, false, 12>(qkv, out, B, N, H, scale, causal, nq, L, s);
+    if (g_attn_variant == 5) return launch3_impl<DH, DP, NT, FAST, false, 9, true>(qkv, out, B, N, H, scale, causal, nq, L, s);
+    return launch3_impl<DH, DP, NT, FAST, false>(qkv, out, B, N, H, scale, causal, nq, L, s);
 }
 
 
 template <int DH, int DP, int NT>
-int launch2(const bf16_t* qkv, bf16_t* out, int B, int N, int H, float scale, int causal, int nq, hipStream_t s) {
+int launch2(const bf16_t* qkv, bf16_t* out, int B, int N, int H, float scale, int causal, int nq, const hirest_qkv_layout& L, hipStream_t s) {
     using C = AttnCfg2<DH, DP, NT>;
     static HirestDevCfg cfg;
     auto kern = attention_kernel_v2<DH, DP, NT>;
     if (int e = hirest_configure(kern, C::LDS_BYTES, cfg)) return e;
-    hipLaunchKernelGGL(kern, dim3(B * H), dim3(512), C::LDS_BYTES, s, qkv, out, N, H, scale * 1.44269504088896340736f, causal, nq);
+    hipLaunchKernelGGL(kern, dim3(B * H), dim3(512), C::LDS_BYTES, s, qkv, out, N, H, scale * 1.44269504088896340736f, causal, nq, L);
     return hirest_launch_status();
 }
 
@@ -715,7 +719,22 @@
 
 extern "C" int hirest_attention_bf16_rows(const hirest_bf16* qkv, hirest_bf16* out, int32_t B, int32_t N, int32_t H,
                                           int32_t dh, float scale, int32_t causal, int32_t q_rows, void* stream) {
-    if (!qkv || !out || B <= 0 || N <= 0 || H <= 0 || q_rows <= 0 || q_rows > N) return HIREST_E_BADARG;
+    return hirest_attention_bf16_layout(qkv, out, B, N, H, dh, scale, causal, q_rows, nullptr, stream);
+}
+
+extern "C" int hirest_attention_bf16_layout(const hirest_bf16* qkv, hirest_bf16* out, int32_t B, int32_t N, int32_t H,
+                                            int32_t dh, float scale, int32_t causal, int32_t q_rows,
+                                            const hirest_qkv_layout* layout, void* stream) {
+    if (!qkv || !out || B <= 0 || N <= 0 || H <= 0 || dh <= 0 || q_rows <= 0 || q_rows > N) return HIREST_E_BADARG;
+    const int64_t D = (int64_t)H * dh;
+    if (3 * D > INT32_MAX) return HIREST_E_BADARG;
+    const hirest_qkv_layout standard = {{0, (int32_t)D, (int32_t)(2 * D)}, {0, (int32_t)D, (int32_t)(2 * D)}, {dh, dh, dh}};
+    const hirest_qkv_layout L = layout ? *layout : standard;
+    for (int x = 0; layout && x < 3; ++x)
+        for (int h = 0; h < H; ++h) {
+            const int64_t c = h == 0 ? L.first[x] : L.base[x] + (int64_t)h * L.step[x];
+            if (c < 0 || c % 8 != 0 || c + dh > 3 * D) return HIREST_E_BADARG;
+        }
     const int nq = q_rows;
     hipStream_t s = reinterpret_cast<hipStream_t>(stream);
     const bf16_t* q = reinterpret_cast<const bf16_t*>(qkv);
@@ -723,27 +742,27 @@
     HirestProfScope prof(HIREST_PROF_ATTENTION, causal, (int64_t)B * H, N, dh, s);
     if (g_attn_variant >= 3 && N > 80 && N <= 272 && B >= 64) {
         const bool fast = !causal && N > 256;
-        if (dh == 88) return fast ? launch3<88, 96, 17, true>(q, o, B, N, H, scale, causal, nq, s)
-                                  : launch3<88, 96, 17, false>(q, o, B, N, H, scale, causal, nq, s);
-        if (dh == 64) return fast ? launch3<64, 64, 17, true>(q, o, B, N, H, scale, causal, nq, s)
-                                  : launch3<64, 64, 17, false>(q, o, B, N, H, scale, causal, nq, s);
+        if (dh == 88) return fast ? launch3<88, 96, 17, true>(q, o, B, N, H, scale, causal, nq, L, s)
+                                  : launch3<88, 96, 17, false>(q, o, B, N, H, scale, causal, nq, L, s);
+        if (dh == 64) return fast ? launch3<64, 64, 17, true>(q, o, B, N, H, scale, causal, nq, L, s)
+                                  : launch3<64, 64, 17, false>(q, o, B, N, H, scale, causal, nq, L, s);
     }
     if (g_attn_variant >= 2) {
         if (dh == 88) {
-            if (N <= 80) return launch2<88, 96, 5>(q, o, B, N, H, scale, causal, nq, s);
-            if (N <= 272) return launch2<88, 96, 17>(q, o, B, N, H, scale, causal, nq, s);
+            if (N <= 80) return launch2<88, 96, 5>(q, o, B, N, H, scale, causal, nq, L, s);
+            if (N <= 272) return launch2<88, 96, 17>(q, o, B, N, H, scale, causal, nq, L, s);
         } else if (dh == 64) {
-            if (N <= 80) return launch2<64, 64, 5>(q, o, B, N, H, scale, causal, nq, s);
-            if (N <= 272) return launch2<64, 64, 17>(q, o, B, N, H, scale, causal, nq, s);
+            if (N <= 80) return launch2<64, 64, 5>(q, o, B, N, H, scale, causal, nq, L, s);
+            if (N <= 272) return launch2<64, 64, 17>(q, o, B, N, H, scale, causal, nq, L, s);
         }
         return HIREST_E_SHAPE;
     }
     if (dh == 88) {
-        if (N <= 80) return launch<88, 96, 5>(q, o, B, N, H, scale, causal, nq, s);
-        if (N <= 272) return launch<88, 96, 17>(q, o, B, N, H, scale, causal, nq, s);
+        if (N <= 80) return launch<88, 96, 5>(q, o, B, N, H, scale, causal, nq, L, s);
+        if (N <= 272) return launch<88, 96, 17>(q, o, B, N, H, scale, causal, nq, L, s);
     } else if (dh == 64) {
-        if (N <= 80) return launch<64, 64, 5>(q, o, B, N, H, scale, causal, nq, s);
-        if (N <= 272) return launch<64, 64, 17>(q, o, B, N, H, scale, causal, nq, s);
+        if (N <= 80) return launch<64, 64, 5>(q, o, B, N, H, scale, causal, nq, L, s);
+        if (N <= 272) return launch<64, 64, 17>(q, o, B, N, H, scale, causal, nq, L, s);
     }
     return HIREST_E_SHAPE;
 }
diff --git a/hirest_amd/csrc/tower.hip b/hirest_amd/csrc/tower.hip
--- a/hirest_amd/csrc/tower.hip
+++ b/hirest_amd/csrc/tower.hip
@@ -70,15 +70,21 @@
     return 0;
 }
 
+hirest_qkv_layout fold_layout(int order, int heads, int dh) {
+    const int D = heads * dh;
+    if (order == 1) return {{0, dh, 2 * dh}, {dh, 0, 2 * dh}, {3 * dh, 3 * dh, 3 * dh}};
+    return {{0, D, 2 * D}, {0, D, 2 * D}, {dh, dh, dh}};
+}
+
 int run_block_lnfold(const hirest_block_weights& w, float* x, hirest_bf16* h, hirest_bf16* big, hirest_bf16* xb, float* part,
                      float* stats, float* guard, int B, int T, int D, int heads, int dh, int Dm, float eps, void* stream,
-                     hirest_bf16* xl = nullptr) {
+                     const hirest_qkv_layout& lay, hirest_bf16* xl = nullptr) {
     const int M = B * T, G = (D + 63) / 64;
     void* res = xl ? static_cast<void*>(xl) : static_cast<void*>(x);
     const int epi_res = xl ? HIREST_EPI_BIAS_RESID2_LNSTATS : HIREST_EPI_BIAS_RESID_LNSTATS_F32;
     CHECK(gemm(xb, D, w.qkv_wf, D, w.qkv_bf, big, 3 * D, M, 3 * D, D, HIREST_EPI_LNFOLD_BF16, stream, nullptr, 0, stats,
                const_cast<float*>(w.qkv_s)));
-    CHECK(hirest_attention_bf16(big, h, B, T, heads, dh, 1.0f / sqrtf((float)dh), 0, stream));
+    CHECK(hirest_attention_bf16_layout(big, h, B, T, heads, dh, 1.0f / sqrtf((float)dh), 0, T, &lay, stream));
     CHECK(gemm(h, D, w.proj_w, D, w.proj_b, res, D, M, D, D, epi_res, stream, nullptr, 0, xb, part));
     CHECK(hirest_ln_stats_finalize(part, G, stats, eps, M, D, guard, stream));
     CHECK(gemm(xb, D, w.fc1_wf, D, w.fc1_bf, big, Dm, M, Dm, D, HIREST_EPI_LNFOLD_GELU_BF16, stream, nullptr, 0, stats,
@@ -90,12 +96,12 @@
 
 int run_block_lnfold_cls(const hirest_block_weights& w, float* x, hirest_bf16* h, hirest_bf16* big, hirest_bf16* xb, float* part,
                          float* stats, float* guard, int B, int T, int D, int heads, int dh, int Dm, float eps, void* stream,
-                         hirest_bf16* xl = nullptr, hirest_bf16* cls_hi = nullptr, hirest_bf16* cls_lo = nullptr) {
+                         const hirest_qkv_layout& lay, hirest_bf16* xl = nullptr, hirest_bf16* cls_hi = nullptr, hirest_bf16* cls_lo = nullptr) {
     const int M = B * T, G = (D + 63) / 64;
     const int64_t TD = (int64_t)T * D;
     CHECK(gemm(xb, D, w.qkv_wf, D, w.qkv_bf, big, 3 * D, M, 3 * D, D, HIREST_EPI_LNFOLD_BF16, stream, nullptr, 0, stats,
                const_cast<float*>(w.qkv_s)));
-    CHECK(hirest_attention_bf16_rows(big, h, B, T, heads, dh, 1.0f / sqrtf((float)dh), 0, 1, stream));
+    CHECK(hirest_attention_bf16_layout(big, h, B, T, heads, dh, 1.0f / sqrtf((float)dh), 0, 1, &lay, stream));
     if (xl) {
         hipStream_t s = reinterpret_cast<hipStream_t>(stream);
         if (hipMemcpy2DAsync(cls_hi, (size_t)D * 2, xb, (size_t)TD * 2, (size_t)D * 2, B, hipMemcpyDeviceToDevice, s) != hipSuccess ||
@@ -122,7 +128,8 @@
 
 extern "C" const char* hirest_build_info(void) {
     return "hirest_hip gfx950 (CDNA4) | gemm pq256 (persistent ping-pong, 2 phases per K step, 16x16x32 bf16 MFMA) / p256 / t128 + LDS-DMA | "
-           "bf16x3 split-operand GEMM + attention | attention 16x16x32 bf16 MFMA + tr16 reads | " __VERSION__;
+           "bf16x3 split-operand GEMM + attention | attention 16x16x32 bf16 MFMA + tr16 reads, per-head q/k/v column offsets "
+           "(folded qkv: q0 k0 | v0 k1 q1 | ... | v_last) | " __VERSION__;
 }
 
 extern "C" size_t hirest_vision_workspace_bytes(const hirest_vision_tower* t, int32_t B) {
@@ -141,6 +148,7 @@
                                      float* out, void* workspace, size_t workspace_bytes, int32_t flags, void* stream) {
     if (!t || !frames || !out || !workspace || B <= 0 || !t->blocks) return HIREST_E_BADARG;
     if (t->width != t->heads * t->head_dim || t->image_size % t->patch != 0) return HIREST_E_SHAPE;
+    if (t->qkv_fold_order != 0 && t->qkv_fold_order != 1) return HIREST_E_BADARG;
     const int G = t->image_size / t->patch, P = G * G, T = P + 1, D = t->width;
     const bool can_fold = vision_lnfold(t, B), lnfold = can_fold && !(flags & HIREST_TOWER_NO_LNFOLD);
     const Regions r = plan((int64_t)B * T, D, vision_wide(t), B, can_fold);
@@ -168,13 +176,14 @@
         hirest_bf16* cls_hi = reinterpret_cast<hirest_bf16*>(ws + r.cls);
         hirest_bf16* cls_lo = reinterpret_cast<hirest_bf16*>(ws + r.cls + align256((size_t)B * D * 2));
         CHECK(hirest_rowstats_split_bf16(x, D, xb, xl, stats, t->ln_eps, B * T, D, guard, stream));
+        const hirest_qkv_layout lay = fold_layout(t->qkv_fold_order, t->heads, t->head_dim);
         for (int l = 0; l < t->layers; ++l) {
             if (prune && l == t->layers - 1) {
                 CHECK(run_block_lnfold_cls(t->blocks[l], x, h, big, xb, part, stats, guard, B, T, D, t->heads, t->head_dim, t->mlp_dim,
-                                           t->ln_eps, stream, xl, cls_hi, cls_lo));
+                                           t->ln_eps, stream, lay, xl, cls_hi, cls_lo));
             } else {
                 CHECK(run_block_lnfold(t->blocks[l], x, h, big, xb, part, stats, guard, B, T, D, t->heads, t->head_dim, t->mlp_dim,
-                                       t->ln_eps, stream, xl));
+                                       t->ln_eps, stream, lay, xl));
             }
         }
         if (xl && !prune) CHECK(hirest_combine_hi_lo_f32(xb, xl, D, x, D, B * T, D, stream));
diff --git a/hirest_amd/eva_clip.py b/hirest_amd/eva_clip.py
--- a/hirest_amd/eva_clip.py
+++ b/hirest_amd/eva_clip.py
@@ -158,6 +158,10 @@
                 if src not in folded:
                     weight, bias, norm = src
                     folded[src] = self._fold(self._f32(attrgetter(weight)(owner)), done[bias], attrgetter(norm)(owner), device)
+                    if field.startswith("qkv_") and self._qkv_fold_order():
+                        rows = torch.tensor(_lib.QkvLayout.make(1, self.heads, self.width // self.heads).columns(
+                            self.heads, self.width // self.heads), dtype=torch.int64, device=device)
+                        folded[src] = tuple(t.index_select(0, rows).contiguous() for t in folded[src])
                 t = folded[src][int(form[4:])]
             else:
                 p = attrgetter(src)(owner)
@@ -174,6 +178,9 @@
             done[field] = t
         keep.extend(t for t in done.values() if t is not None)
         return {f: None if t is None else t.data_ptr() for f, t in done.items()}
+
+    def _qkv_fold_order(self) -> int:
+        return 0
 
     def _fold(self, w32, bias, norm, device):
         N, K = w32.shape
@@ -262,7 +269,11 @@
         return dict(image_size=self.image_size, patch=P, width=self.width, heads=self.heads, head_dim=self.width // self.heads,
                     mlp_dim=self.mlp_dim, layers=self.layers, embed_dim=self.embed_dim, kpad=(3 * P * P + 63) // 64 * 64,
                     act=1 if self.quick_gelu else 0, ln_eps=1e-6,
-                    out_all_tokens=0)
+                    out_all_tokens=0, qkv_fold_order=self._qkv_fold_order())
+
+    def _qkv_fold_order(self) -> int:
+        fold = self.fold_layernorm and not self.quick_gelu and (self.width // self.heads) % 8 == 0
+        return 1 if fold and os.environ.get("HIREST_QKV_COLUMN_ORDER", "1") != "0" else 0
 
     _EXACT = {"fp32": ("fp32", "hirest_vision_workspace_bytes_f32", "hirest_vision_forward_f32", "max_frames_per_call_f32", False),
               "bf16x3": ("x3", "hirest_vision_workspace_bytes_x3", "hirest_vision_forward_x3", "max_frames_per_call_x3", True)}
diff --git a/hirest_amd/ops.py b/hirest_amd/ops.py
--- a/hirest_amd/ops.py
+++ b/hirest_amd/ops.py
@@ -102,9 +102,15 @@
 
 @on_tensor_device
 def attention(qkv: torch.Tensor, out: torch.Tensor, B: int, N: int, H: int, dh: int, causal: bool,
-              scale: Optional[float] = None):
+              scale: Optional[float] = None, layout: Optional[_lib.QkvLayout] = None, q_rows: Optional[int] = None):
     lib = _lib.load()
     scale = dh ** -0.5 if scale is None else scale
+    if layout is not None or q_rows is not None:
+        _lib.check(lib.hirest_attention_bf16_layout(_dev(qkv, torch.bfloat16, "attn.qkv"), _dev(out, torch.bfloat16, "attn.out"),
+                                                    B, N, H, dh, float(scale), int(bool(causal)), N if q_rows is None else int(q_rows),
+                                                    None if layout is None else C.addressof(layout), stream_ptr()),
+                   "hirest_attention_bf16_layout")
+        return out
     _lib.check(lib.hirest_attention_bf16(_dev(qkv, torch.bfloat16, "attn.qkv"), _dev(out, torch.bfloat16, "attn.out"),
                                          B, N, H, dh, float(scale), int(bool(causal)), stream_ptr()),
                "hirest_attention_bf16")
diff --git a/include/hirest_hip.h b/include/hirest_hip.h
--- a/include/hirest_hip.h
+++ b/include/hirest_hip.h
@@ -68,6 +68,13 @@
 int hirest_attention_bf16_rows(const hirest_bf16* qkv, hirest_bf16* out,
                                int32_t B, int32_t N, int32_t H, int32_t dh,
                                float scale, int32_t causal, int32_t q_rows, void* stream);
+typedef struct hirest_qkv_layout {
+    int32_t first[3], base[3], step[3];
+} hirest_qkv_layout;
+int hirest_attention_bf16_layout(const hirest_bf16* qkv, hirest_bf16* out,
+                                 int32_t B, int32_t N, int32_t H, int32_t dh,
+                                 float scale, int32_t causal, int32_t q_rows,
+                                 const hirest_qkv_layout* layout, void* stream);
 int hirest_attention_select_kernel(int32_t which);
 int hirest_attention_set_mapping(int32_t by_head);
 int hirest_attention_set_pace(int32_t units);
@@ -147,6 +154,7 @@
     const float* image_mean; const float* image_std;
     const float* ln_pre_g; const float* ln_pre_b;
     int32_t out_all_tokens;
+    int32_t qkv_fold_order;
 } hirest_vision_tower;
 
 size_t hirest_vision_workspace_bytes(const hirest_vision_tower* t, int32_t B);
@@ -195,6 +203,7 @@
     const float* image_mean; const float* image_std;
     const float* ln_pre_g; const float* ln_pre_b;
     int32_t out_all_tokens;
+    int32_t qkv_fold_order;
 } hirest_vision_tower_f32;
 
 typedef struct hirest_text_tower_f32 {
```
